# GregoryFaust/yaha

Hardware: AMD Instinct MI355X
Metric: aligned reads/s (whole node), 1 000 bp reads, OQC mode hot path (higher is better)
Workload: dtype int16

## Files before the change

### yaha_amd/csrc/device/abi.hip

```cpp
#include "ctx.h"
#include <memory>

std::atomic<int> gCtxPerDevice[64];
std::mutex gRowsMu[64];
hipEvent_t gRowsEv[64][4];
bool gRowsEvValid[64][4];
unsigned long long gRowsSeq[64];
std::atomic<int> gActiveRuns[64];
const char *const kStageNames[T_N] = {"seed_lookup", "hit_sort", "fragments_regions", "chain", "align_dp", "layout", "align_p1_gapfill", "ext_rows", "ext_trace",
                                      "align_p3_score_split", "ext_rows_device_clock", "ext_rows_packed16"};
thread_local const ygpu_ctx *tlsPfFailed = nullptr;

int runTo(ygpu_ctx *ctx, int stage)
{
    int rc;
    HIPCHK(hipSetDevice(ctx->device));
    if (ctx->stageDone < 1) {
        rc = stageSeed(ctx); if (rc) return rc;
        EV0(T_FRAGS); rc = buildFrags(ctx);
        if (rc == YD_RESORT) { rc = stageSeed(ctx); if (rc) return rc; EV0(T_FRAGS); rc = buildFrags(ctx);
            if (rc == YD_RESORT) { ctx->err = "hit sort: the sorted keys are not in ascending order"; rc = YGPU_EINTERNAL; } }
        if (rc) return rc;
        if (!ctx->nFrags) EV1(T_FRAGS);
        ctx->stageDone = 1;
// ... 209 lines not shown
    if (!ix || !p) return YGPU_EINVAL;
    for (int k = 0; k < n * cpd; k++) { all[k] = new ygpu_ctx; all[k]->device = devices[k / cpd]; }
    std::vector<ygpu_ctx *> out(n); for (int k = 0; k < n; k++) out[k] = all[k * cpd];
    std::vector<int> rcs(n, 0);
    auto notStarted = [&](int rc) {
        for (int k = 0; k < n; k++) {
            if (!rcs[k]) { rcs[k] = YGPU_EINVAL; out[k]->err = "not started: another device of the call failed"; }
            if (rc_each) rc_each[k] = rcs[k];
            for (int j = 1; j < cpd; j++) all[k * cpd + j]->err = out[k]->err;
        }
        return rc;
    };
    const double t0 = nowMs();
    int ndev = 0;
    if (hipGetDeviceCount(&ndev) != hipSuccess || ndev <= 0) { for (int k = 0; k < n; k++) { rcs[k] = YGPU_ENODEV;
        out[k]->err = "no HIP device visible: the hot path needs an MI355X (there is no CPU fallback)"; } return notStarted(YGPU_ENODEV); }
    if (getenv("YGPU_INIT_PHASES")) fprintf(stderr, "[ygpu] init: runtime up (hipGetDeviceCount) %8.1f ms\n", nowMs() - t0);
    {
        bool bad = false;
        for (int k = 0; k < n; k++) if (devices[k] < 0 || devices[k] >= ndev) { rcs[k] = YGPU_ENODEV; out[k]->err = "device index out of range"; bad = true; }
        if (bad) return notStarted(YGPU_ENODEV);
    }
    { int bad = 0; for (int k = 0; k < n; k++) { rcs[k] = checkParams(out[k], ix, p); if (rcs[k]) bad = rcs[k]; } if (bad) return notStarted(bad); }
    ImagePlan plan; plan.build(ix, n > 1 ? (64ull << 20) : (1024ull << 20));
    std::vector<ImageState> states(n); for (auto &st : states) { st.done.reset(new std::atomic<int>[plan.pieces.size() + 1]);
        for (size_t i = 0; i <= plan.pieces.size(); i++) st.done[i] = 0; }
    std::unique_ptr<std::atomic<int>[]> ready(new std::atomic<int>[n]); for (int k = 0; k < n; k++) ready[k] = 0;
    std::vector<int> srcIndex(n, -1); const bool peer = !(getenv("YGPU_PEER_COPY") && atoi(getenv("YGPU_PEER_COPY")) == 0);
    for (int k = 1; k < n && peer; k++) {
        int can = devices[k] == devices[k - 1] ? 1 : 0;
        if (!can && hipDeviceCanAccessPeer(&can, devices[k], devices[k - 1]) != hipSuccess) { can = 0; (void)hipGetLastError(); }
        if (can && devices[k] != devices[k - 1]) { if (hipSetDevice(devices[k]) == hipSuccess) { const hipError_t e = hipDeviceEnablePeerAccess(devices[k - 1], 0);
            if (e != hipSuccess && e != hipErrorPeerAccessAlreadyEnabled) can = 0; } else can = 0; (void)hipGetLastError(); }
        if (can) srcIndex[k] = k - 1;
    }
    if (getenv("YGPU_INIT_PHASES")) { fprintf(stderr, "[ygpu] init: image sources:");
        for (int k = 0; k < n; k++) { if (srcIndex[k] < 0) fprintf(stderr, " device %d <- host;", devices[k]);
        else fprintf(stderr, " device %d <- device %d;", devices[k], devices[srcIndex[k]]); } fprintf(stderr, " %zu pieces\n", plan.pieces.size()); }
    std::vector<std::thread> th;
    for (int k = 1; k < n; k++) th.emplace_back([&, k]() { rcs[k] = initDevice(out[k], devices[k], srcIndex[k], srcIndex[k] >= 0 ? devices[srcIndex[k]] : -1, ix, plan,
        states.data(), k, ready.get(), all + k * cpd + 1, cpd - 1); });
    rcs[0] = initDevice(out[0], devices[0], -1, -1, ix, plan, states.data(), 0, ready.get(), all + 1, cpd - 1);
    for (auto &x : th) x.join();
    int rc = 0; for (int k = 0; k < n; k++) { if (rc_each) rc_each[k] = rcs[k]; if (rcs[k] && !rc) rc = rcs[k];
        if (rcs[k]) for (int j = 1; j < cpd; j++) if (all[k * cpd + j]->err.empty()) all[k * cpd + j]->err = "the device's first context failed: " + out[k]->err; }
    return rc;
}

int ygpu_device_count(void) { int n = 0; if (hipGetDeviceCount(&n) != hipSuccess) { (void)hipGetLastError(); return 0; } return n; }

int ygpu_init(int device, const ygpu_index_view *ix, const ygpu_params *p, ygpu_ctx **out)
{
    if (!out) return YGPU_EINVAL;
    return ygpu_init_multi(&device, 1, 1, ix, p, out, nullptr);
}

int ygpu_clone(const ygpu_ctx *parent, ygpu_ctx **out)
{
    *out = nullptr;
    if (!parent || !parent->stream) return YGPU_EINVAL;
    ygpu_ctx *ctx = new ygpu_ctx; *out = ctx; ctx->device = parent->device;
    int rc = initCommon(ctx, parent->device); if (rc) return rc;
    shareImage(ctx, parent);
    ENSURE(ctx->counters, 4 * CNT_N); ENSURE(ctx->ctr, sizeof(DevCounters)); ENSURE(ctx->errFlag, 64);
    HIPCHK(hipMemsetAsync(ctx->counters.p, 0, 4 * CNT_N, ctx->stream));
    HIPCHK(streamSync(ctx));
    return 0;
}

}
std::vector<DevBuf *> allBuffers(ygpu_ctx *ctx)
{
    DevBuf *all[] = {&ctx->dBases, &ctx->dSO, &ctx->dROA, &ctx->dLow, &ctx->dFwd, &ctx->dRev, &ctx->dFwd4, &ctx->dRev4, &ctx->dReadOff, &ctx->dKmerOff, &ctx->posS, &ctx->posC,
        &ctx->posRsI, &ctx->hitOff, &ctx->expandStart, &ctx->keysA, &ctx->keysB, &ctx->segOff, &ctx->bigB, &ctx->bigE, &ctx->isHead, &ctx->tileState,
                         &ctx->frags, &ctx->regStart, &ctx->multiList, &ctx->smallList, &ctx->bigList, &ctx->regionCount, &ctx->regionBase, &ctx->clumps, &ctx->clumpFrags,
                             &ctx->clumpFrags0, &ctx->order, &ctx->clumpsSorted, &ctx->rootPush, &ctx->rootBase, &ctx->outClumps,
                         &ctx->outClumps2, &ctx->outOps, &ctx->outRoot, &ctx->outPush, &ctx->dstIdx, &ctx->readCount, &ctx->readStart, &ctx->counters, &ctx->ctr, &ctx->errFlag,
                             &ctx->scanState, &ctx->bucketWork, &ctx->scratchAlign,
                         &ctx->segLists, &ctx->subB, &ctx->subE, &ctx->subLists, &ctx->subBigB, &ctx->subBigE, &ctx->sub2B, &ctx->sub2E, &ctx->sub2Lists, &ctx->sub3B, &ctx->sub3E,
                             &ctx->sub3Lists, &ctx->kmerParts, &ctx->scratchChain, &ctx->dpProbs, &ctx->dpRes, &ctx->dpOps, &ctx->rootState, &ctx->stateOps, &ctx->extProbs,
                             &ctx->rowsBound, &ctx->stripOff, &ctx->extRes, &ctx->extTrace, &ctx->chunkCnt, &ctx->memoKeys, &ctx->memoCount, &ctx->probs2, &ctx->rowsBound2,
                             &ctx->stripOff2, &ctx->extRes2, &ctx->extTrace2, &ctx->rowsClock, &ctx->splitScratch, &ctx->fallList, &ctx->keys2a, &ctx->keys2b, &ctx->vals2a,
                             &ctx->vals2b, &ctx->extKeys, &ctx->extVals, &ctx->extKeys2, &ctx->extOrder, &ctx->slowList, &ctx->gapScratch, &ctx->jointCount, &ctx->jointBase,
                             &ctx->joints, &ctx->sortKeys, &ctx->sortVals, &ctx->sortKeys2, &ctx->sortVals2, &ctx->gapOps, &ctx->waveChunks, &ctx->extOps, &ctx->traceCnt,
                         &ctx->oqCs, &ctx->oqCl, &ctx->oqOpsIn, &ctx->oqSeeds, &ctx->oqQlen, &ctx->pf.scanState, &ctx->pf.counters, &ctx->oqProf, &ctx->oqLists, &ctx->oqClsCnt,
                             &ctx->oqThr, &ctx->oqSeqStart, &ctx->oqSeqLen, &ctx->oqNeed, &ctx->oqPoolOff, &ctx->oqKeys, &ctx->oqStack, &ctx->oqNodes, &ctx->oqPrim, &ctx->oqPA,
                             &ctx->oqPfx, &ctx->oqPath, &ctx->oqPool, &ctx->oqPush, &ctx->oqOut, &ctx->oqOutCnt, &ctx->oqOutOps, &ctx->oqPrimCnt, &ctx->oqOutStart,
                             &ctx->oqOpsStart, &ctx->oqFClumps, &ctx->oqFOps, &ctx->jnCnt, &ctx->jnStart, &ctx->jnOut, &ctx->jnStats, &ctx->jnSeqStart, &ctx->jnSeqLen,
                         &ctx->puFwd, &ctx->puReadOff, &ctx->puTileCnt, &ctx->puTileStart, &ctx->puCand, &ctx->puSlots, &ctx->puRows,
                         &ctx->idTable, &ctx->idStats, &ctx->idSeqStart, &ctx->idSeqLen, &ctx->idBinBase, &ctx->idTileCnt, &ctx->idTileStart, &ctx->idOut};
    return std::vector<DevBuf *>(all, all + sizeof all / sizeof all[0]);
}
extern "C" {

void ygpu_destroy(ygpu_ctx *ctx)
{
    if (!ctx) return;
    if (ctx->worker.joinable()) { { std::lock_guard<std::mutex> lk(ctx->aMu); ctx->aQuit = true; } ctx->aCv.notify_all(); ctx->worker.join(); }
    if (ctx->counted) gCtxPerDevice[ctx->device & 63]--;
    if (ctx->stream) {
        hipSetDevice(ctx->device);
        {
            const int dv = ctx->device & 63; std::lock_guard<std::mutex> lk(gRowsMu[dv]);
            (void)hipStreamSynchronize(ctx->stream);
            if (gCtxPerDevice[dv].load() <= 0) for (int k = 0; k < 4; k++) if (gRowsEvValid[dv][k]) { (void)hipEventDestroy(gRowsEv[dv][k]); gRowsEvValid[dv][k] = false; }
        }
        if (ctx->sharedIndex) { ctx->dBases.p = nullptr; ctx->dBases.cap = 0; ctx->dSO.p = nullptr; ctx->dSO.cap = 0; ctx->dROA.p = nullptr; ctx->dROA.cap = 0;
            ctx->dLow.p = nullptr; ctx->dLow.cap = 0; }
        const std::vector<DevBuf *> all = allBuffers(ctx);
        for (auto b : all) b->release();
        for (int t = 0; t < T_N; t++) { hipEventDestroy(ctx->ev[t][0]); hipEventDestroy(ctx->ev[t][1]); }
        if (ctx->evSync) hipEventDestroy(ctx->evSync);
        if (ctx->pinned) hipHostFree(ctx->pinned);
        if (ctx->pf.pinned) hipHostFree(ctx->pf.pinned);
        if (ctx->snapCtr) hipHostFree(ctx->snapCtr);
        if (ctx->pf.evSync) hipEventDestroy(ctx->pf.evSync);
        if (ctx->evSnap) hipEventDestroy(ctx->evSnap);
        for (int i = 0; i < YD_MAX_CHUNK_EV; i++) hipEventDestroy(ctx->evChunk[i]);
        hipEventDestroy(ctx->evTail); hipStreamDestroy(ctx->stream2);
        hipStreamDestroy(ctx->stream);
    }
    delete ctx;
}
int ygpu_memory(ygpu_ctx *ctx, uint64_t *free_bytes, uint64_t *total_bytes, uint64_t *ctx_bytes)
{
    if (!ctx || !ctx->stream) return YGPU_EINVAL;
    HIPCHK(hipSetDevice(ctx->device));
    size_t fb = 0, tb = 0; HIPCHK(hipMemGetInfo(&fb, &tb));
    uint64_t mine = 0; for (DevBuf *b : allBuffers(ctx)) if (b->p && !(ctx->sharedIndex && (b == &ctx->dBases || b == &ctx->dSO || b == &ctx->dROA
        || b == &ctx->dLow))) mine += b->cap;
    if (free_bytes) *free_bytes = fb; if (total_bytes) *total_bytes = tb; if (ctx_bytes) *ctx_bytes = mine;
    return 0;
}
int ygpu_park(ygpu_ctx *ctx)
{
    if (!ctx || !ctx->stream) return YGPU_EINVAL;
    HIPCHK(hipSetDevice(ctx->device)); HIPCHK(streamSync(ctx));
    for (DevBuf *b : allBuffers(ctx)) if (b != &ctx->dBases && b != &ctx->dSO && b != &ctx->dROA && b != &ctx->dLow) b->release();
    if (ctx->counted) { gCtxPerDevice[ctx->device & 63]--; ctx->counted = false; }
    ctx->stageDone = 0; ctx->parked = true; ctx->idUsed = 0;
    return 0;
}
int ygpu_get_arena_profile(ygpu_ctx *ctx, ygpu_arena_profile *out)
{
    if (!ctx || !ctx->stream || !out) return YGPU_EINVAL;
    memset(out, 0, sizeof *out);
    const std::vector<DevBuf *> all = allBuffers(ctx);
    if (all.size() > sizeof out->cap / sizeof out->cap[0]) { ctx->err = "arena profile: more buffers than the profile holds"; return YGPU_EINTERNAL; }
    out->n = (uint32_t)all.size();
    for (size_t k = 0; k < all.size(); k++) { DevBuf *b = all[k];
        out->cap[k] = (b == &ctx->dBases || b == &ctx->dSO || b == &ctx->dROA || b == &ctx->dLow) ? 0ull : (uint64_t)b->cap; }
    out->trace_ratio = ctx->traceRatio; out->ops_ratio = ctx->opsRatio; out->last_clump_slots = ctx->lastClumpSlots; out->last_fall = ctx->lastFall; out->bases = ctx->totalBases;
    return 0;
}
int ygpu_presize(ygpu_ctx *ctx, const ygpu_arena_profile *prof)
{
    if (!ctx || !ctx->stream || !prof) return YGPU_EINVAL;
    if (ctx->parked) { ctx->err = "the context was parked (ygpu_park)"; return YGPU_EINVAL; }
    HIPCHK(hipSetDevice(ctx->device));
    const std::vector<DevBuf *> all = allBuffers(ctx);
    if (prof->n != all.size()) { ctx->err = "arena profile of another build"; return YGPU_EINVAL; }
    for (size_t k = 0; k < all.size(); k++) {
        DevBuf *b = all[k];
        if (b == &ctx->dBases || b == &ctx->dSO || b == &ctx->dROA || b == &ctx->dLow || b == &ctx->counters || b == &ctx->ctr || b == &ctx->errFlag
            || b == &ctx->pf.counters || b == &ctx->idTable || b == &ctx->idStats) continue;
        if (prof->cap[k] > b->cap && b->ensureExact((size_t)prof->cap[k])) { (void)hipGetLastError(); ctx->err = "hipMalloc failed while presizing the arenas"; return YGPU_ENOMEM;
// ... 140 lines not shown
```

### yaha_amd/csrc/device/align_diag.h

```cpp
#pragma once

static void diagJointHist(ygpu_ctx *ctx, uint32_t J)
{
    std::vector<JointRec> hj(J); hipMemcpy(hj.data(), ctx->joints.p, sizeof(JointRec) * (size_t)J, hipMemcpyDeviceToHost);
    unsigned long long nj[4] = {0, 0, 0, 0}, cj[4] = {0, 0, 0, 0}, b3 = 0, b3lim = 0, c3lim = 0, f3 = 0, wh[5] = {0, 0, 0, 0, 0};
    for (auto &j : hj) if (j.kind == JK_DP) {
        const bool banded = (j.flags & 2u) != 0; const int q = j.qGap, r = j.rGap, ld = q > r ? q - r : r - q, W = banded ? 2 * ctx->P.bandWidth + ld + 1 : r + 1;
        const uint32_t cls = gapJointClass(gapJointKey(ctx->P, banded, q, r)); nj[cls]++; cj[cls] += (unsigned long long)q * (unsigned long long)std::min(W, r + 1);
        if (cls == 3) { if (banded) { b3++; if (W <= 32 && q <= YD_GROWS - 1 && r <= YD_GREF) { b3lim++; c3lim += (unsigned long long)q * W; } } else f3++;
            wh[std::min(4, (W - 17) / 8)]++; }
    }
    fprintf(stderr, "[ygpu] DP joints by class (band <= 12 / band <= 16 / other W <= 16 / the rest): %llu %llu %llu %llu; strip cells %llu %llu %llu %llu; "
                    "the rest: banded %llu (W <= 32 within the band kernels' limits: %llu, %llu cells), full %llu; "
                    "W 17-24 / 25-32 / 33-40 / 41-48 / more: %llu %llu %llu %llu %llu\n",
            nj[0], nj[1], nj[2], nj[3], cj[0], cj[1], cj[2], cj[3], b3, b3lim, c3lim, f3, wh[0], wh[1], wh[2], wh[3], wh[4]);
}

static void diagCountDups(ygpu_ctx *ctx, uint32_t nProb)
{
    std::vector<ExtProb> hp(nProb); hipMemcpy(hp.data(), ctx->extProbs.p, sizeof(ExtProb) * (size_t)nProb, hipMemcpyDeviceToHost);
    std::vector<std::array<uint32_t, 4>> keys; keys.reserve(nProb);
    for (auto &e : hp) if (e.flags & XP_VALID) keys.push_back({e.qBase, e.rOff, (uint32_t)e.qOff | ((uint32_t)e.qLen << 16), e.flags & 3u});
    std::sort(keys.begin(), keys.end()); size_t dup = 0, sameStart = 0;
    for (size_t k = 1; k < keys.size(); k++) { dup += keys[k] == keys[k - 1];
        sameStart += keys[k][0] == keys[k - 1][0] && keys[k][1] == keys[k - 1][1] && (keys[k][2] & 0xFFFF) == (keys[k - 1][2] & 0xFFFF) && keys[k][3] == keys[k - 1][3]; }
    fprintf(stderr, "[ygpu] extension problems: %zu valid, %zu exact duplicates (%.2f%%), %zu share (read, strand, direction, rOff, qOff) with their predecessor (%.2f%%)\n",
        keys.size(), dup, 100.0 * dup / std::max<size_t>(1, keys.size()), sameStart, 100.0 * sameStart / std::max<size_t>(1, keys.size()));
}

static void diagTraceLens(ygpu_ctx *ctx, const ExtArgs &E, uint32_t np)
{
    streamSync(ctx);
    std::vector<ExtRes> hr(np); std::vector<uint32_t> ho(np);
    hipMemcpy(hr.data(), E.res, sizeof(ExtRes) * (size_t)np, hipMemcpyDeviceToHost); hipMemcpy(ho.data(), E.order, 4ull * np, hipMemcpyDeviceToHost);
    unsigned long long walkers = 0, sumLen = 0, sumWaveMax = 0, sumRows = 0, hist[8] = {0};
    for (uint32_t w = 0; w < np; w += 64) { uint32_t mx = 0; for (uint32_t k = w; k < std::min(np, w + 64); k++) { const ExtRes &r = hr[ho[k]];
        const uint32_t len = r.score > 0 ? (uint32_t)r.maxi : 0u; walkers += r.score > 0; sumLen += len; sumRows += r.rows; mx = std::max(mx, len); int b = 0;
        while (b < 7 && (len >> (b + 3))) b++; hist[len ? b : 0] += 1; } sumWaveMax += mx; }
    fprintf(stderr, "[ygpu] traceback: %u problems, %llu walk (%.1f%%), mean walk %.1f rows (all) / %.1f (walkers), rows computed mean %.1f; sum over waves of "
        "the longest walk %llu = %.1f x the lanes' mean\n",
            np, walkers, 100.0 * walkers / np, (double)sumLen / np, (double)sumLen / std::max(1ull, walkers), (double)sumRows / np, sumWaveMax,
                (double)sumWaveMax * 64.0 / std::max(1ull, sumLen));
    fprintf(stderr, "[ygpu] walk length histogram (0..7, 8.., 16.., 32.., 64.., 128.., 256.., 512..):"); for (int b = 0; b < 8; b++) fprintf(stderr, " %llu", hist[b]);
        fprintf(stderr, "\n");
}

static void diagTraceDbg(const ExtArgs &E)
{
    unsigned w8[8]; hipMemcpyFromSymbol(w8, HIP_SYMBOL(gTraceDbg), sizeof w8);
    if (!w8[0]) return;
    ExtRes rr; hipMemcpy(&rr, E.res + w8[6], sizeof rr, hipMemcpyDeviceToHost); ExtProb pp; hipMemcpy(&pp, E.probs + w8[6], sizeof pp, hipMemcpyDeviceToHost);
    fprintf(stderr, "[ygpu] k_ext_trace left its strip: dword %d of %u, f0 %u, laneOff %u; problem %u where %08x (wave %u lane %u phase %u) score %d maxi %d maxj "
        "%d rows %u qLen %u flags %u\n", (int)w8[1], w8[2], w8[3], w8[4], w8[6], w8[7], w8[7] >> 10, (w8[7] >> 4) & 63, w8[7] & 15, rr.score, rr.maxi, rr.maxj, rr.rows,
            pp.qLen, pp.flags);
    memset(w8, 0, sizeof w8); hipMemcpyToSymbol(HIP_SYMBOL(gTraceDbg), w8, sizeof w8);
}

static void diagFallWhy(ygpu_ctx *ctx, const unsigned int *fallCount)
{
    uint32_t fc = 0; hipMemcpyAsync(&fc, fallCount, 4, hipMemcpyDeviceToHost, ctx->stream); streamSync(ctx);
    unsigned w8[8]; hipMemcpyFromSymbol(w8, HIP_SYMBOL(gFallWhy), sizeof w8);
    fprintf(stderr, "[ygpu] roots left to the wave kernel %u (other %u, DP not listed %u, second split %u, depth/list %u)\n", fc, w8[0], w8[1], w8[2], w8[3]);
    memset(w8, 0, sizeof w8); hipMemcpyToSymbol(HIP_SYMBOL(gFallWhy), w8, sizeof w8);
}

static void diagListHist(ygpu_ctx *ctx, uint32_t r0, uint32_t r1)
{
    const uint32_t nr2 = r1 - r0; std::vector<ExtRes> hr2(2 * (size_t)nr2); std::vector<RootState> hs(nr2);
    hipMemcpy(hr2.data(), ctx->extRes.as<ExtRes>() + 2 * (size_t)r0, sizeof(ExtRes) * hr2.size(), hipMemcpyDeviceToHost);
        hipMemcpy(hs.data(), ctx->rootState.as<RootState>() + r0, sizeof(RootState) * nr2, hipMemcpyDeviceToHost);
    unsigned long long hx[8] = {0}, hb[8] = {0}, ht[8] = {0}, sumx = 0, sumb = 0; const unsigned edges[7] = {0, 1, 2, 4, 8, 16, 32};
    auto bin = [&](unsigned v) { int k = 0; while (k < 7 && v > edges[k]) k++; return k; };
    for (uint32_t k = 0; k < nr2; k++) {
        const unsigned a = hr2[2 * k].score > 0 ? hr2[2 * k].nOps : 0u, c2 = hr2[2 * k + 1].score > 0 ? hr2[2 * k + 1].nOps : 0u, b = hs[k].len; hx[bin(a)]++;
        hx[bin(c2)]++; hb[bin(b)]++; ht[bin(a + b + c2)]++; sumx += a + c2; sumb += b; }
    fprintf(stderr, "[ygpu] list lengths over %u roots (bins: 0, 1, 2, 3-4, 5-8, 9-16, 17-32, more): extension lists", nr2);
        for (int k = 0; k < 8; k++) fprintf(stderr, " %llu", hx[k]);
    fprintf(stderr, "; phase-1 lists"); for (int k = 0; k < 8; k++) fprintf(stderr, " %llu", hb[k]); fprintf(stderr, "; merged");
        for (int k = 0; k < 8; k++) fprintf(stderr, " %llu", ht[k]);
    fprintf(stderr, "; mean ops per root: extensions %.1f, phase 1 %.1f\n", (double)sumx / nr2, (double)sumb / nr2);
}

static void profReset()
{
#ifdef YD_PROF
    unsigned long long z[16] = {0}; hipMemcpyToSymbol(HIP_SYMBOL(gProf), z, sizeof z); hipMemcpyToSymbol(HIP_SYMBOL(gRowsProf), z, sizeof(unsigned long long) * 8);
    hipMemcpyToSymbol(HIP_SYMBOL(gTraceProf), z, sizeof(unsigned long long) * 8);
#endif
}
static void profPrint(ygpu_ctx *ctx, unsigned waves)
{
#ifdef YD_PROF
    streamSync(ctx); unsigned long long z[16]; hipMemcpyFromSymbol(z, HIP_SYMBOL(gProf), sizeof z);
    const char *nm[10] = {"root_total", "dp_rows", "traceback", "perfect_ext", "score", "emit", "split", "merge", "dp_calls", "roots"};
    fprintf(stderr, "[YD_PROF] waves %u:", waves); for (int i = 0; i < 10; i++) fprintf(stderr, " %s=%llu", nm[i], z[i]); fprintf(stderr, "\n");
    unsigned long long q[8]; hipMemcpyFromSymbol(q, HIP_SYMBOL(gRowsProf), sizeof q);
    if (q[0]) fprintf(stderr,
        "[YD_PROF] k_ext_rows_pk: wave passes %llu; of them writing results %.1f %%, with a new maximum in some lane %.1f %%, handing blocks over %.1f %%; "
// ... 9 lines not shown
```

### yaha_amd/csrc/device/ctx.h

```cpp
#pragma once
#include <hip/hip_runtime.h>
#include <string>
#include <vector>
#include <cstring>
#include <cstdio>
#include <cstdlib>
#include <algorithm>
#include <array>
#include <atomic>
#include <chrono>
#include <thread>
#include <mutex>
#include <condition_variable>
#include <memory>
#include "common.h"
#include "../oqc_core.h"

#define HIPCHK(call) do { hipError_t e_ = (call); \
    if (e_ != hipSuccess) { ctx->err = std::string(#call) + ": " + hipGetErrorString(e_); return YGPU_ENODEV; } } while (0)

#define KL(kern, grid, block, shmem, st, ...) do { hipLaunchKernelGGL(kern, grid, block, shmem, st, __VA_ARGS__); hipError_t e_ = hipGetLastError(); \
    if (e_ != hipSuccess) { ctx->err = std::string("launch of " #kern " failed: ") + hipGetErrorString(e_); return YGPU_ENODEV; } } while (0)

#define YD_MAX_CHUNK_EV 16

struct DevBuf {
    void *p = nullptr;
    size_t cap = 0;
    int ensure(size_t bytes, bool keep = false, hipStream_t st = 0)
    {
        if (bytes <= cap) return 0;
        size_t ncap = bytes + bytes / 4 + 256; void *np = nullptr;
        if (hipMalloc(&np, ncap) != hipSuccess) return -1;
        if (keep && p && cap) { hipMemcpyAsync(np, p, cap, hipMemcpyDeviceToDevice, st); hipStreamSynchronize(st); }
        if (p) hipFree(p);
        p = np; cap = ncap; return 0;
    }
    void release() { if (p) hipFree(p); p = nullptr; cap = 0; }
    int ensureExact(size_t bytes)
    {
        if (bytes <= cap) return 0;
        release();
        void *np = nullptr;
        if (hipMalloc(&np, bytes) != hipSuccess) return -1;
        p = np; cap = bytes; return 0;
    }
    template <class T> T *as() const { return (T *)p; }
};

enum {
    CNT_NMULTI = 0, CNT_MAXN, CNT_CLUMPS, CNT_CFRAGS, CNT_QCHAIN, CNT_QALIGN, CNT_OUTCLUMPS, CNT_OUTOPS, CNT_QDP, CNT_DPOPS, CNT_NBIG, CNT_QBIG,
    CNT_STATEOPS, CNT_EXTOPS, CNT_QEXT, CNT_SLOW, CNT_NDP, CNT_NDP16, CNT_GAPOPS, CNT_PAD_EVEN, CNT_NMULTI2 ,
        CNT_NTINY, CNT_NSMALL, CNT_NMID, CNT_NB12, CNT_NB16,
        CNT_NB24,
    CNT_SEGC,
    CNT_NFRAGS = CNT_SEGC + 16,
    CNT_NREG = CNT_NFRAGS + 3,
    CNT_SCANFAIL = CNT_NREG + 2,
    CNT_N = CNT_NREG + 4
};
enum { T_SEED = 0, T_SORT, T_FRAGS, T_CHAIN, T_ALIGN, T_LAYOUT, T_TOP, T_P1 = T_TOP, T_XROWS, T_XTRACE, T_P3, T_XROWS_DEV, T_XROWS_PK, T_N };

extern std::atomic<int> gCtxPerDevice[64];
extern std::mutex gRowsMu[64];
extern hipEvent_t gRowsEv[64][4];
extern bool gRowsEvValid[64][4];
extern unsigned long long gRowsSeq[64];
extern std::atomic<int> gActiveRuns[64];
extern const char *const kStageNames[T_N];

struct PfSide {
    std::string err;
    hipStream_t stream = nullptr;
    uint32_t *pinned = nullptr;
    hipEvent_t evSync = nullptr;
    DevBuf scanState, counters;
    int device = 0;
};

enum { TRACK_DEPTH = 0, TRACK_EVENTS = 1, TRACK_PILEUP = 2, TRACK_KINDS };
struct TrackImage {
    int device = 0;
    DevBuf data, stats, seqStart, seqLength, binBase;
    uint64_t nBins = 0;
    uint32_t channels = 1, bin = 0, minMapq = 0, minClip = 0;
    std::vector<uint32_t> hSeqStart, hSeqLength;
    ~TrackImage() { (void)hipSetDevice(device); data.release(); stats.release(); seqStart.release(); seqLength.release(); binBase.release(); }
};

struct ygpu_ctx {
    int device = 0;
    hipStream_t stream = nullptr;
    DevParams P{};
    std::string err;
    int nCU = 256;
    DevBuf dBases, dSO, dROA, dLow;
    bool sharedIndex = false;
    uint32_t nReads = 0;
    int maxQ = 0;
    uint64_t totalBases = 0;
    uint32_t nKmers = 0;
    std::vector<uint32_t> hReadOff, hKmerOff;
    DevBuf dFwd, dRev, dFwd4, dRev4, dReadOff, dKmerOff;
    DevBuf bigB, bigE;
    DevBuf posS, posC, posRsI, hitOff, expandStart, keysA, keysB, segOff, isHead, tileState, frags;
    DevBuf segLists, subB, subE, subLists, subBigB, subBigE, sub2B, sub2E, sub2Lists, sub3B, sub3E, sub3Lists, kmerParts;
    DevBuf regStart, multiList, smallList, bigList, regionCount, regionBase;
    DevBuf clumps, clumpFrags, clumpFrags0, order, clumpsSorted, scratchChain;
    DevBuf rootPush, rootBase, outClumps, outClumps2, outOps, outRoot, outPush, dstIdx, readCount, readStart;
    DevBuf scratchAlign, dpProbs, dpRes, dpOps;
    DevBuf rootState, stateOps, extProbs, rowsBound, stripOff, extRes, extTrace, chunkCnt;
    DevBuf memoKeys, memoCount, probs2, rowsBound2, stripOff2, extRes2, extTrace2, splitScratch, fallList;
    DevBuf keys2a, keys2b, vals2a, vals2b, extKeys, extVals, extKeys2, extOrder, slowList;
    DevBuf gapScratch, jointCount, jointBase, joints, sortKeys, sortVals, sortKeys2, sortVals2, gapOps;
    DevBuf waveChunks, extOps, traceCnt, rowsClock;
    DevBuf counters, ctr, errFlag, scanState, bucketWork;
    bool evUsed[16] = {false};
    double traceT = 0;
    hipStream_t stream2 = nullptr;
    hipEvent_t evChunk[YD_MAX_CHUNK_EV], evTail;
    bool counted = false;
    bool parked = false;
    long long traceBudgetBlocks = 0;
    uint32_t lastClumpSlots = 0;
    bool keepAllFrags = false;
    unsigned long long hRowsClock[2] = {0, 0};
    int laneChunks = 0;
    uint32_t segSortMax = 0;
    int splitLanes = 1;
    int rows2PerCU = 0;
    int alignWavesPerCU = 0;
    int laneExt = 1;
    std::vector<unsigned long long> hStripOff;
    int runsDone = 0;
    double traceRatio = 0.0, opsRatio = 0.03;
    int statRanges = 0, statAttempts = 0;
    double statT0 = 0;
    DevBuf oqProf, oqLists, oqClsCnt, oqThr, oqSeqStart, oqSeqLen, oqNeed, oqPoolOff, oqKeys, oqStack, oqNodes, oqPrim, oqPA, oqPfx, oqPath, oqPool;
    DevBuf oqPush, oqOut, oqOutCnt, oqOutOps, oqPrimCnt, oqOutStart, oqOpsStart, oqFClumps, oqFOps;
    bool oqSet = false, oqDone = false;
    yoqc::Params oqP{};
    yoqc::Seqs oqG{};
    uint32_t nFOut = 0, nFOps = 0;
    PfSide pf;
    std::atomic<bool> pfSnap{false};
    hipEvent_t evSnap = nullptr;
    uint32_t snapN = 0, snapC = 0, snapOps = 0, pfN = 0;
    unsigned long long runGen = 0, snapGen = 0, filtGen = 0;
    ygpu_counters pfCounters{};
    DevCounters *snapCtr = nullptr;
    DevCounters snapCtrPlain{};
    unsigned long long snapHits = 0, snapFrags = 0, snapRegions = 0;
    DevBuf oqCs, oqCl, oqOpsIn, oqSeeds, oqQlen;
    std::shared_ptr<TrackImage> track[TRACK_KINDS];
    DevBuf puFwd, puReadOff, puTileCnt, puTileStart, puCand, puSlots, puRows;
    uint64_t puNCand = 0; bool puHaveCand = false;
    DevBuf idTable, idStats, idSeqStart, idSeqLen, idBinBase, idTileCnt, idTileStart, idOut;
    bool idSet = false, idAuto = false;
    uint64_t idCap = 0, snapBases = 0;
    uint32_t idMinMapq = 0, idMinLen = 1, idNSeqs = 0, idUsed = 0;
    DevBuf jnCnt, jnStart, jnOut, jnStats, jnSeqStart, jnSeqLen;
    bool jnSet = false, jnDone = false, jnHaveTotal = false;
    uint32_t jnMinMapq = 0, jnNSeqs = 0, jnReads = 0, jnTotal = 0;
    uint32_t hOutCounts[2] = {0, 0};
    uint32_t nHits = 0, nFrags = 0, nRegions = 0, nMulti = 0, nTiny = 0, nSmall = 0, nMid = 0, nBig = 0, maxN = 0;
    int sortRankUsed = 0;
    bool sortRankForced = false;
    uint32_t nClumpSlots = 0, nClumps = 0, nClumpFrags = 0, nOut = 0, nOutOps = 0;
    int stageDone = 0;
    std::vector<uint32_t> hClumpStart, hOps, hClumpFragStart, hClumpRS, hDpOps;
    std::vector<ygpu_clump> hClumps;
    std::vector<ygpu_fragment> hFrags, hClumpFrags;
    std::vector<ygpu_dp_result> hDpRes;
    ygpu_counters hCounters{};
    std::thread worker;
    std::mutex aMu;
    std::condition_variable aCv;
    const ygpu_read_batch *aBatch = nullptr;
    uint64_t aTicket = 0;
    int aRc = 0;
    bool aOpen = false, aDone = false, aQuit = false, aWaiting = false;
    ygpu_result_batch aOut{};
    long long lastFall = -1;
    unsigned int hFall = 0;
    uint32_t *pinned = nullptr;
    hipEvent_t evSync = nullptr;
    hipEvent_t ev[T_N][2];
    float ms[T_N] = {0};
    float totalMs = 0;
    const char *names[T_N];
    bool rowsPacked = false;
};

static inline DevBatch devBatch(ygpu_ctx *c)
{
    DevBatch b; b.fwd = c->dFwd.as<uint8_t>(); b.rev = c->dRev.as<uint8_t>(); b.readOff = c->dReadOff.as<uint32_t>(); b.nReads = c->nReads; return b;
}
// ... 73 lines not shown
```

### yaha_amd/csrc/device/dp_stage.h

```cpp
#pragma once
#include "split_lanes.h"

__global__ void k_dp_classify(DevParams P, const uint8_t *bases, const uint8_t *fwd, const uint8_t *rev, JointRec *joints, uint32_t n, uint32_t *keys, uint32_t *diagOps)
{
    YD_HIGH_PRIO();
    const uint32_t t = blockIdx.x * blockDim.x + threadIdx.x;
    if (t >= n) return;
    JointRec j = joints[t];
    YD_GLOBAL const uint8_t *q = toGlobal((j.flags & 1u) ? rev : fwd) + j.qBase; YD_GLOBAL const uint8_t *gB = toGlobal(bases);
    auto refAt = [&](uint32_t off) -> uint32_t { const uint32_t b = gB[off >> 1]; return (off & 1u) ? (b & 15u) : (b >> 4); };
    const int qGap = j.qGap, rGap = j.rGap;
    const bool banded = (j.flags & 2u) != 0;
    j.kind = JK_DP; uint32_t key = YD_JKEY_NONE;
    if (qGap == rGap && qGap > 0) {
        int mm = 0, runs = 0, pc = -1;
        for (int k = 0; k < qGap; k++) { const int c = (uint32_t)q[(int)j.nsqo + k] != refAt(j.nsro + (uint32_t)k); mm += c; runs += c != pc; pc = c; }
        if (mm * (P.MS + P.RC) <= P.MS + 2 * (P.GO + P.GE)) { j.kind = JK_DIAG; j.score = P.MS * (qGap - mm) - P.RC * mm; j.nOps = (uint16_t)runs; }
    }
    if (j.kind == JK_DP) key = gapJointKey(P, banded, qGap, rGap);
    joints[t] = j; keys[t] = key; diagOps[t] = j.kind == JK_DIAG ? (uint32_t)j.nOps : 0u;
}

__global__ void k_dp_gather_ext(const ExtProb *probs, const ExtRes *res, const uint32_t *extOps, const uint32_t *outOff, const uint32_t *dst, uint32_t n,
                                ygpu_dp_result *out, uint32_t *outOps)
{
    YD_HIGH_PRIO();
    const uint32_t p = blockIdx.x * blockDim.x + threadIdx.x;
    if (p >= n) return;
    const ExtRes r = res[p]; ygpu_dp_result o; o.score = 0; o.addedQLen = o.addedRLen = 0; o.op_start = outOff[p]; o.n_ops = 0;
    if (r.score > 0) {
        const bool rv = (probs[p].flags & XP_REV) != 0; const uint32_t *src = extOpsPtr(extOps, r); const char codes[4] = {'M', 'R', 'D', 'I'};
        o.score = r.score; o.addedQLen = (uint16_t)r.maxi; o.addedRLen = (uint16_t)(r.maxi + (r.maxj - YD_LBAND)); o.n_ops = r.nOps;
        for (uint32_t k = 0; k < r.nOps; k++) { const uint32_t op = src[rv ? r.nOps - 1u - k : k];
            outOps[o.op_start + k] = ((uint32_t)(uint8_t)codes[opCode(op) & 3] << 16) | (uint32_t)opLen(op); }
    }
    out[dst[p]] = o;
}
__global__ void k_dp_gather_gap(DevParams P, const uint8_t *bases, const uint8_t *fwd, const uint8_t *rev, const JointRec *joints, const uint32_t *gapOps, const uint32_t *outOff,
    const uint32_t *dst,
                                uint32_t n, ygpu_dp_result *out, uint32_t *outOps)
{
    YD_HIGH_PRIO();
    const uint32_t t = blockIdx.x * blockDim.x + threadIdx.x;
    if (t >= n) return;
    const JointRec j = joints[t]; ygpu_dp_result o; o.score = j.score; o.addedQLen = o.addedRLen = 0; o.op_start = outOff[t]; o.n_ops = j.nOps;
    const char codes[4] = {'M', 'R', 'D', 'I'};
    if (j.kind == JK_DIAG) {
        YD_GLOBAL const uint8_t *q = toGlobal((j.flags & 1u) ? rev : fwd) + j.qBase; YD_GLOBAL const uint8_t *gB = toGlobal(bases);
        int pc = -1, pl = 0; uint32_t w = o.op_start;
        for (int k = 0; k < (int)j.qGap; k++) {
            const uint32_t off = j.nsro + (uint32_t)k, b = gB[off >> 1], rc = (off & 1u) ? (b & 15u) : (b >> 4);
            const int c = (uint32_t)q[(int)j.nsqo + k] == rc ? OP_M : OP_R;
            if (c == pc) pl++; else { if (pc >= 0) outOps[w++] = ((uint32_t)(uint8_t)codes[pc] << 16) | (uint32_t)pl; pc = c; pl = 1; }
        }
        if (pc >= 0) outOps[w++] = ((uint32_t)(uint8_t)codes[pc] << 16) | (uint32_t)pl;
    } else for (uint32_t k = 0; k < j.nOps; k++) { const uint32_t op = gapOps[j.opsOff + k];
        outOps[o.op_start + k] = ((uint32_t)(uint8_t)codes[opCode(op) & 3] << 16) | (uint32_t)opLen(op); }
    out[dst[t]] = o;
}
```

### yaha_amd/csrc/device/gap_band_lanes.h

```cpp
#pragma once
#include "phase_lanes.h"

template <int GW>
__global__ void __launch_bounds__(64) k_gap_band(AlignArgs A, PhaseArgs X)
{
    YD_HIGH_PRIO();
    static_assert(GW == 12 || GW == 16, "two instances");
    const int lane = laneId(); const DevParams &P = A.P;
    const int GO = P.GO, GE = P.GE, GOE = P.GO + P.GE, RC = P.RC, MS = P.MS, maxIntron = P.maxIntron, maxGapP = P.maxGap, bw = P.bandWidth;
    uint32_t *sp = (uint32_t *)(X.gapScratch + (size_t)blockIdx.x * 64u * YD_GAP_SCRATCH) + lane;
    YD_GLOBAL uint32_t *T32 = toGlobal(sp); uint32_t *tmp = sp + (size_t)((YD_GROWS + 1) * 32 / 4) * 64;
    YD_GLOBAL const uint8_t *gB = toGlobal(A.bases);
    const uint32_t tBegin = GW == 12 ? 0u : X.nDPb[0], tEnd = GW == 12 ? X.nDPb[0] : X.nDPb[1];
    constexpr int RD = GW / 4;
    __shared__ uint32_t sQ[16 * 64], sR[13 * 64];
    typedef uint32_t yd_u32u __attribute__((aligned(1)));
    for (uint32_t base = tBegin + blockIdx.x * 64u; base < tEnd; base += gridDim.x * 64u) {
        const uint32_t t = base + (uint32_t)lane; const bool live = t < tEnd;
        int nT = 0, score = 0; unsigned cells = 0; uint32_t ji = 0;
        if (live) {
            ji = X.sortedVals[t]; const JointRec j = X.joints[ji];
            const int qGap = j.qGap, rGap = j.rGap;
            int left, right; if (rGap > qGap) { right = bw + (rGap - qGap); left = bw; } else { left = bw + (qGap - rGap); right = bw; }
            const int W = left + right + 1;
            YD_GLOBAL const uint8_t *q = toGlobal((j.flags & 1u) ? A.B.rev : A.B.fwd) + j.qBase + j.nsqo;
            const uint32_t rB0 = ((j.nsro >= (uint32_t)left ? j.nsro - (uint32_t)left : 0u) >> 1) & ~3u;
            {
                const int nQ = (qGap + 3) >> 2, nR = (int)((((j.nsro + (uint32_t)(qGap - left + GW - 1)) >> 1) - rB0) >> 2) + 1;
#pragma unroll
                for (int k = 0; k < 16; k++) if (k < nQ) sQ[k * 64 + lane] = *(YD_GLOBAL const yd_u32u *)(q + 4 * k);
#pragma unroll
                for (int k = 0; k < 13; k++) if (k < nR) sR[k * 64 + lane] = *(YD_GLOBAL const uint32_t *)(gB + rB0 + 4u * (uint32_t)k);
            }
            auto qAt = [&](int idx) -> int { return (int)((sQ[(idx >> 2) * 64 + lane] >> (8 * (idx & 3))) & 0xFFu); };
            auto refAt = [&](int idx) -> uint32_t {
                if (idx < 0 && (uint32_t)(-idx) > j.nsro) return 15u;
                const uint32_t off = j.nsro + (uint32_t)idx, rel = (off >> 1) - rB0; const uint32_t b = (sR[(rel >> 2) * 64 + lane] >> (8u * (rel & 3u))) & 0xFFu;
                return (off & 1u) ? (b & 15u) : (b >> 4);
            };
            int PV[GW], PF[GW], PI[GW];
#pragma unroll
            for (int c = 0; c < GW; c++) { PV[c] = c == left ? 0 : ((c > left && c < W) ? -(GO + (c - left) * GE) : YD_LWORST); PF[c] = c == left ? -GO : YD_LWORST; PI[c] = 0; }
#pragma unroll
            for (int k = 0; k < RD; k++) {
                uint32_t acc = 0;
#pragma unroll
                for (int b = 0; b < 4; b++) { const int c = 4 * k + b; const uint32_t cell = c == left ? TR_U8 : ((c > left && c < W) ? (uint32_t)(OP_D | ((c - left) << 2)) : 0u);
                    acc |= cell << (8 * b); }
                T32[k * 64] = acc;
            }
            unsigned long long win = 0;
#pragma unroll
            for (int c = 0; c < GW; c++) win |= (unsigned long long)refAt(c - left) << (4 * c);
            int qc = qAt(0);
            for (int i = 1; i <= qGap; i++) {
                const int qcNext = qAt(i < qGap ? i : qGap - 1);
                const uint32_t nbNext = refAt(i - left + GW - 1);
                { int sc = left + 1 - i; if (sc < 0) sc = 0; int ec = left + rGap - i; if (ec > W - 1) ec = W - 1; if (ec >= sc) cells += (unsigned)(ec - sc + 1); }
                int PVCol = YD_LWORST, PE = YD_LWORST, PD = 0, dV = PV[0];
                uint32_t acc = 0;
#pragma unroll
                for (int c = 0; c < GW; c++) {
                    const int rc = (int)((win >> (4 * c)) & 15ull);
                    const bool eq = rc == qc;
                    int V = dV + (eq ? MS : -RC); uint32_t cell = eq ? (uint32_t)OP_M : (uint32_t)OP_R;
                    const int CE = PE - GE, NE = PVCol - GOE;
                    const bool cE = CE >= NE && (PD + 1) <= maxIntron;
                    PE = cE ? CE : NE; PD = cE ? PD + 1 : 1;
                    if (PE > V) { V = PE; cell = (uint32_t)OP_D | ((uint32_t)PD << 2); }
                    int upV, upF, upI;
                    if (c + 1 < GW) { upV = PV[c + 1]; upF = PF[c + 1]; upI = PI[c + 1]; } else { upV = YD_LWORST; upF = YD_LWORST; upI = 0; }
                    const int CF = upF - GE, NF = upV - GOE;
                    const bool cF = CF >= NF && (upI + 1) <= maxGapP;
                    const int F = cF ? CF : NF, I = cF ? upI + 1 : 1;
                    if (F > V) { V = F; cell = (uint32_t)OP_I | ((uint32_t)I << 2); }
                    acc |= (cell & 0xFFu) << (8 * (c & 3));
                    if ((c & 3) == 3) { T32[(i * RD + (c >> 2)) * 64] = acc; acc = 0; }
                    const bool in = c < 11 || c < W;
                    PV[c] = in ? V : YD_LWORST; PF[c] = in ? F : YD_LWORST; PI[c] = in ? I : 0;
                    PVCol = V; dV = upV;
                }
                win = (win >> 4) | ((unsigned long long)nbNext << (4 * (GW - 1)));
                qc = qcNext;
            }
            score = PV[0];
#pragma unroll
            for (int c = 1; c < GW; c++) score = c == right ? PV[c] : score;
            int x = right, y = qGap;
            auto cellAt = [&](int yy, int xx) -> unsigned { const int c = yy * GW + xx; return (T32[(c >> 2) * 64] >> (8 * (c & 3))) & 0xFFu; };
            unsigned cell = cellAt(y, x);
            int prev = cell == TR_U8 ? -1 : (int)(cell & 3u), acc2 = 0, n = 0;
            for (int guard = 0; cell != TR_U8 && guard < 4096; guard++) {
                const int code = (int)(cell & 3u); int len = (int)(cell >> 2);
                if (code == OP_D) x -= len; else if (code == OP_I) { x += len; y -= len; } else { y -= 1; len = 1; }
                if (prev != code) { tmp[n * 64] = opMake(prev, acc2); n++; prev = code; acc2 = len; } else acc2 += len;
                if (y < 0 || x < 0 || x >= GW || n >= 190) break;
                cell = cellAt(y, x);
            }
            tmp[n * 64] = opMake(prev, acc2); n++;
            nT = n;
        }
        int incl = nT;
#pragma unroll
        for (int d = 1; d < 64; d <<= 1) { int v = __shfl_up(incl, d, 64); if (lane >= d) incl += v; }
        const int total = __shfl(incl, 63, 64); unsigned ob = 0;
        if (lane == 63 && total) ob = atomicAdd(X.gapOpsCount, (unsigned)total);
        ob = (unsigned)__shfl((int)ob, 63, 64);
        if (live) {
            const unsigned off = ob + (unsigned)(incl - nT);
            if ((unsigned long long)off + (unsigned)nT > (unsigned long long)X.gapOpsCap) atomicCAS(A.errFlag, 0, (int)YERR_OUT);
            else {
                for (int k = 0; k < nT; k++) X.gapOps[off + k] = tmp[(nT - 1 - k) * 64];
                JointRec *jp = X.joints + ji; jp->opsOff = off; jp->nOps = (uint16_t)nT; jp->score = score; jp->cells = cells;
            }
        }
    }
}
```

### yaha_amd/csrc/device/gap_band_pk.h

```cpp
#pragma once
#include "gap_band_lanes.h"
#include "ext_lanes_pk.h"

template <int GW, bool CAPS, class QAt, class RefAt>
__device__ __forceinline__ int gapBandPkRows(const DevParams &P, int qGap, int left, int right, int W, QAt qAt, RefAt refAt, YD_GLOBAL uint32_t *T32)
{
    constexpr int H = GW / 2, RD = GW / 4;
    const int GO = P.GO, GE = P.GE, GOE = GO + GE;
    const uint32_t GEp = pk2(GE), GOEp = pk2(GOE), LWp = pk2(YD_LW16), LWg = pk2(YD_LW16 - GOE), ONEp = 0x00010001u;
    uint32_t NEGKv = pk2(-(P.MS + P.RC)), MSGv = pk2(P.MS + GOE), ONEv = ONEp, C15v = 0x000F000Fu, FOURv = 0x00040004u, OPDv = pk2(OP_D), OPIv = pk2(OP_I);
    asm volatile("" : "+v"(NEGKv), "+v"(MSGv), "+v"(ONEv), "+v"(C15v), "+v"(FOURv), "+v"(OPDv), "+v"(OPIv));
    const uint32_t maxIp = pk2(P.maxIntron < 30000 ? P.maxIntron : 30000), maxGp = pk2(P.maxGap < 30000 ? P.maxGap : 30000);
    auto onChain = [&](int c) { return c > left && c < W; };
    auto v0 = [&](int c) -> int { return c == left ? 0 : (onChain(c) ? -(GO + (c - left) * GE) : YD_LW16); };
    auto f0 = [&](int c) -> int { return c == left ? -GO : YD_LW16; };
    auto e0 = [&](int c) -> int { return onChain(c) ? -(GO + (c - left) * GE) : YD_LW16; };
    auto d0 = [&](int c) -> int { return onChain(c) ? c - left : 0; };
    auto cell0 = [&](int c) -> uint32_t { return c == left ? (uint32_t)TR_U8 : (onChain(c) ? (uint32_t)(OP_D | ((c - left) << 2)) : 0u); };
    auto lo16 = [](int v) -> uint32_t { return (uint32_t)v & 0xFFFFu; };
    uint32_t PVg[H], PF[H], PI[H], rc[H], keep[H];
#pragma unroll
    for (int k = 0; k < H; k++) {
        PVg[k] = lo16(v0(k) - GOE) | (LWg & 0xFFFF0000u); PF[k] = lo16(f0(k)) | (LWp & 0xFFFF0000u); PI[k] = 0u;
        rc[k] = refAt(k - left) | (refAt(k + H - 1 - left) << 16);
// ... 62 lines not shown
            }
#pragma unroll
            for (int d = 0; d < RD; d++) T32[(t * RD + d) * 64] = D[d];
        }
        carryV = PVg[H - 1] & 0xFFFFu; carryE = PE & 0xFFFFu; carryD = PD & 0xFFFFu;
        if (t == qGap && right < H) {
            scoreLo = 0;
#pragma unroll
            for (int k = 0; k < H; k++) if (k == right) scoreLo = (int)(short)(PVg[k] & 0xFFFFu) + GOE;
        }
        if (t <= qGap) {
            const uint32_t nb = refAt(t + GW - 2 - left), was1 = rc[1] >> 16;
#pragma unroll
            for (int k = 0; k + 1 < H; k++) rc[k] = rc[k + 1];
            rc[H - 1] = was1 | (nb << 16);
        }
        qcHi = qcLo;
    }
    int score = scoreLo;
    if (right >= H) {
#pragma unroll
        for (int k = 0; k < H; k++) if (k + H == right) score = (int)(short)(PVg[k] >> 16) + GOE;
    }
    return score;
}

template <int GW>
__global__ void __launch_bounds__(64) k_gap_band_pk(AlignArgs A, PhaseArgs X)
{
    YD_HIGH_PRIO();
    static_assert(GW == 12 || GW == 16 || GW == 24, "three instances");
    constexpr int H = GW / 2;
    const int lane = laneId(); const DevParams &P = A.P;
    const int bw = P.bandWidth;
    uint32_t *sp = (uint32_t *)(X.gapScratch + (size_t)blockIdx.x * 64u * YD_GAP_SCRATCH) + lane;
    YD_GLOBAL uint32_t *T32 = toGlobal(sp); uint32_t *tmp = sp + (size_t)((YD_GROWS + 1) * 32 / 4) * 64;
    YD_GLOBAL const uint8_t *gB = toGlobal(A.bases);
    const uint32_t tBegin = GW == 12 ? 0u : (GW == 16 ? X.nDPb[0] : X.nDP[1]), tEnd = GW == 12 ? X.nDPb[0] : (GW == 16 ? X.nDPb[1] : X.nDP[1] + X.nDPb[2]);
    __shared__ uint32_t sQ[16 * 64], sR[13 * 64];
    typedef uint32_t yd_u32u __attribute__((aligned(1)));
    for (uint32_t base = tBegin + blockIdx.x * 64u; base < tEnd; base += gridDim.x * 64u) {
        const uint32_t t = base + (uint32_t)lane; const bool live = t < tEnd;
        int nT = 0, score = 0; unsigned cells = 0; uint32_t ji = 0;
        JointRec j; j.qGap = 0; j.rGap = 0; j.nsro = 0; j.flags = 0; j.qBase = 0; j.nsqo = 0;
        if (live) { ji = X.sortedVals[t]; j = X.joints[ji]; }

        const bool caps = __ballot(live && ((int)j.qGap > P.maxGap || P.maxIntron < GW)) != 0ull;
        if (live) {
            const int qGap = j.qGap, rGap = j.rGap;
            int left, right; if (rGap > qGap) { right = bw + (rGap - qGap); left = bw; } else { left = bw + (qGap - rGap); right = bw; }
            const int W = left + right + 1;
            YD_GLOBAL const uint8_t *q = toGlobal((j.flags & 1u) ? A.B.rev : A.B.fwd) + j.qBase + j.nsqo;
            const uint32_t rB0 = ((j.nsro >= (uint32_t)left ? j.nsro - (uint32_t)left : 0u) >> 1) & ~3u;
            {
                const int nQ = (qGap + 3) >> 2, nR = (int)((((j.nsro + (uint32_t)(qGap - left + GW - 1)) >> 1) - rB0) >> 2) + 1;
#pragma unroll
                for (int k = 0; k < 16; k++) if (k < nQ) sQ[k * 64 + lane] = *(YD_GLOBAL const yd_u32u *)(q + 4 * k);
#pragma unroll
                for (int k = 0; k < 13; k++) if (k < nR) sR[k * 64 + lane] = *(YD_GLOBAL const uint32_t *)(gB + rB0 + 4u * (uint32_t)k);
            }
            auto qAt = [&](int idx) -> int { return (int)((sQ[(idx >> 2) * 64 + lane] >> (8 * (idx & 3))) & 0xFFu); };
            auto refAt = [&](int idx) -> uint32_t {
                if (idx < 0 && (uint32_t)(-idx) > j.nsro) return 15u;
                const uint32_t off = j.nsro + (uint32_t)idx, rel = (off >> 1) - rB0; const uint32_t b = (sR[(rel >> 2) * 64 + lane] >> (8u * (rel & 3u))) & 0xFFu;
                return (off & 1u) ? (b & 15u) : (b >> 4);
            };
            for (int i = 1; i <= qGap; i++) { int sc = left + 1 - i; if (sc < 0) sc = 0; int ec = left + rGap - i; if (ec > W - 1) ec = W - 1;
                if (ec >= sc) cells += (unsigned)(ec - sc + 1); }
            score = caps ? gapBandPkRows<GW, true>(P, qGap, left, right, W, qAt, refAt, T32) : gapBandPkRows<GW, false>(P, qGap, left, right, W, qAt, refAt, T32);
            int x = right, y = qGap;
            auto cellAt = [&](int yy, int xx) -> unsigned { const int c = (yy + (xx >= H ? 1 : 0)) * GW + xx; return (T32[(c >> 2) * 64] >> (8 * (c & 3))) & 0xFFu; };
            unsigned cell = cellAt(y, x);
            int prev = cell == TR_U8 ? -1 : (int)(cell & 3u), acc2 = 0, n = 0;
            for (int guard = 0; cell != TR_U8 && guard < 4096; guard++) {
                const int code = (int)(cell & 3u); int len = (int)(cell >> 2);
                if (code == OP_D) x -= len; else if (code == OP_I) { x += len; y -= len; } else { y -= 1; len = 1; }
                if (prev != code) { tmp[n * 64] = opMake(prev, acc2); n++; prev = code; acc2 = len; } else acc2 += len;
                if (y < 0 || x < 0 || x >= GW || n >= 190) break;
                cell = cellAt(y, x);
            }
            tmp[n * 64] = opMake(prev, acc2); n++;
            nT = n;
        }
        int incl = nT;
#pragma unroll
        for (int d = 1; d < 64; d <<= 1) { int v = __shfl_up(incl, d, 64); if (lane >= d) incl += v; }
        const int total = __shfl(incl, 63, 64); unsigned ob = 0;
        if (lane == 63 && total) ob = atomicAdd(X.gapOpsCount, (unsigned)total);
        ob = (unsigned)__shfl((int)ob, 63, 64);
        if (live) {
            const unsigned off = ob + (unsigned)(incl - nT);
            if ((unsigned long long)off + (unsigned)nT > (unsigned long long)X.gapOpsCap) atomicCAS(A.errFlag, 0, (int)YERR_OUT);
            else {
                for (int k = 0; k < nT; k++) X.gapOps[off + k] = tmp[(nT - 1 - k) * 64];
                JointRec *jp = X.joints + ji; jp->opsOff = off; jp->nOps = (uint16_t)nT; jp->score = score; jp->cells = cells;
            }
        }
    }
}
```

### yaha_amd/csrc/device/phase_lanes.h

```cpp
#pragma once
#include "ext_lanes.h"

struct RootState { uint32_t sro, listOff; int32_t score; uint16_t sqo, eqo, refLen, len; uint8_t status, pad[3]; uint32_t pad2[2]; };
enum { JK_NONE = 0, JK_D, JK_I, JK_R, JK_DIAG, JK_DP };
struct JointRec {
    uint32_t nsro, qBase; uint16_t nsqo, qGap, rGap; uint8_t kind, flags;
    uint32_t opsOff; uint16_t nOps, pad; int32_t score; uint32_t cells;
};
struct PhaseArgs {
    RootState *state; uint32_t *stateOps; unsigned int *stateOpsCount; uint32_t stateOpsCap;
    ExtProb *probs; unsigned long long *rowsBound;
    const ExtRes *res; const uint32_t *extOps;
    uint32_t *slowList; unsigned int *slowCount;
    int useList;
    uint32_t rootBegin;
    uint32_t *memoKeys; unsigned int *memoCount; ExtProb *probs2; unsigned long long *rowsBound2; unsigned int *nProb2; uint32_t probs2Cap;
    uint32_t *jointCount; const uint32_t *jointBase; JointRec *joints; uint32_t nJoints;
    uint32_t *sortKeys, *sortVals; const uint32_t *sortedVals; unsigned int *nDP, *nDPb; uint32_t band24;
    uint32_t *gapOps; unsigned int *gapOpsCount; uint32_t gapOpsCap;
    uint32_t *extKeys, *extVals;
    uint8_t *gapScratch;
};

__device__ __forceinline__ unsigned waveSumU(unsigned v) { return (unsigned)waveSumI((int)v); }
__device__ __forceinline__ unsigned waveReserve(unsigned long long mask, unsigned int *counter, int lane, unsigned each = 1u)
{
    if (!mask) return 0u;
    const int first = __builtin_ctzll(mask); unsigned base = 0;
    if (lane == first) base = atomicAdd(counter, each * (unsigned)__builtin_popcountll(mask));
    base = (unsigned)__builtin_amdgcn_readlane((int)base, first);
    return base + each * (unsigned)__builtin_popcountll(mask & ((1ull << lane) - 1ull));
}


template <int N> __device__ __forceinline__ void blockCounters(unsigned long long *const (&dst)[N], const unsigned (&val)[N])
{
    __shared__ unsigned sAcc[N];
    if (threadIdx.x < (unsigned)N) sAcc[threadIdx.x] = 0;
    __syncthreads();
    if (laneId() == 0) { for (int k = 0; k < N; k++) if (val[k]) atomicAdd(&sAcc[k], val[k]); }
    __syncthreads();
    if (threadIdx.x < (unsigned)N && sAcc[threadIdx.x]) atomicAdd(dst[threadIdx.x], (unsigned long long)sAcc[threadIdx.x]);
}

template <int N> __device__ __forceinline__ void blockCountersU32(unsigned int *const (&dst)[N], const unsigned (&val)[N])
{
    __shared__ unsigned sAcc32[N];
    if (threadIdx.x < (unsigned)N) sAcc32[threadIdx.x] = 0;
    __syncthreads();
    if (laneId() == 0) { for (int k = 0; k < N; k++) if (val[k]) atomicAdd(&sAcc32[k], val[k]); }
    __syncthreads();
    if (threadIdx.x < (unsigned)N && sAcc32[threadIdx.x]) atomicAdd(dst[threadIdx.x], sAcc32[threadIdx.x]);
}

__device__ __forceinline__ unsigned blockReserve(unsigned int *counter, unsigned waveTotal)
{
    __shared__ unsigned sTot[4], sBase;
    const int wv = (int)(threadIdx.x >> 6);
    if (laneId() == 0) sTot[wv] = waveTotal;
    __syncthreads();
    if (threadIdx.x == 0) { const unsigned t = sTot[0] + sTot[1] + sTot[2] + sTot[3]; sBase = t ? atomicAdd(counter, t) : 0u; }
    __syncthreads();
    unsigned b = sBase; for (int k = 0; k < wv; k++) b += sTot[k];
    return b;
}

#define YD_GROWS 60
#define YD_GREF 64
#define YD_GQW 16
#define YD_GRW 10
#define YD_GAP_SCRATCH 3072
#define TR_U8 0xFFu
struct GapLaneMem { int *pv, *pf; uint8_t *pi; uint32_t *refw, *qw; uint8_t *T; uint32_t *tmp; };
template <int GW>
__device__ __forceinline__ int gapDPLane(const DevParams &P, YD_GLOBAL const uint8_t *gB, YD_GLOBAL const uint8_t *q, bool banded,
                                         uint32_t rOff, int rLen, int qOff, int qLen, const GapLaneMem &M, int &nOps, unsigned &cellsOut)
{
    const int GO = P.GO, GE = P.GE, RC = P.RC, MS = P.MS, maxIntron = P.maxIntron, maxGapP = P.maxGap;
    int left = 0, right = 0;
    if (banded) { const int bw = P.bandWidth; if (rLen > qLen) { right = bw + (rLen - qLen); left = bw; } else { left = bw + (qLen - rLen); right = bw; } }
    const int W = banded ? left + right + 1 : rLen + 1;
    int *PV = M.pv, *PF = M.pf; uint8_t *PI = M.pi; YD_GLOBAL uint32_t *T32 = (YD_GLOBAL uint32_t *)toGlobal(M.T);
#define GPV(j) PV[(j) * 64]
#define GPF(j) PF[(j) * 64]
#define GPI(j) PI[(j) * 64]
    const uint32_t rByte0 = (rOff >> 1) & ~3u; const int rNib0 = (int)(rOff - 2u * rByte0);
    { YD_GLOBAL const uint32_t *g = (YD_GLOBAL const uint32_t *)(gB + rByte0); uint32_t w[YD_GRW];
#pragma unroll
      for (int k = 0; k < YD_GRW; k++) w[k] = g[k];
#pragma unroll
      for (int k = 0; k < YD_GRW; k++) M.refw[k * 64] = w[k]; }
    const size_t qAddr = (size_t)(q + qOff); const int qSkew = (int)(qAddr & 3u);
    { YD_GLOBAL const uint32_t *g = (YD_GLOBAL const uint32_t *)(qAddr - (size_t)qSkew); uint32_t w[YD_GQW];
#pragma unroll
      for (int k = 0; k < YD_GQW; k++) w[k] = g[k];
#pragma unroll
      for (int k = 0; k < YD_GQW; k++) M.qw[k * 64] = w[k]; }
    auto refAt = [&](int t) -> int { const int nb = rNib0 + t; const uint32_t w = M.refw[(nb >> 3) * 64]; return (int)((w >> (8 * ((nb >> 1) & 3) + ((nb & 1) ? 0 : 4))) & 15u); };
    auto qAt = [&](int t) -> int { const int bb = qSkew + t; return (int)((M.qw[(bb >> 2) * 64] >> (8 * (bb & 3))) & 0xFFu); };
    const int startInit = banded ? left + 1 : 1;
    if (banded) { GPF(W) = YD_WORST; GPV(W) = YD_WORST; GPI(W) = 0; }
    {
        uint32_t acc = 0;
        for (int j = 0; j < W; j++) {
            uint32_t cell = 0;
            if (j == startInit - 1) cell = TR_U8; else if (j >= startInit) { const int dc = j - startInit + 1; cell = (uint32_t)(OP_D | (dc << 2)); GPV(j) = -(GO + dc * GE);
                GPF(j) = YD_WORST; GPI(j) = 0; }
            acc |= cell << (8 * (j & 3));
            if ((j & 3) == 3 || j == W - 1) { T32[(j >> 2) * 64] = acc; acc = 0; }
        }
    }
    GPF(startInit - 1) = 0; GPI(startInit - 1) = 0; GPV(startInit - 1) = 0;
    int V = 0, PVCol = YD_WORST, startCol = 1, endCol = W - 1; unsigned cells = 0;
    for (int i = 1; i <= qLen; i++) {
        int PDCol = 0, PECol = YD_WORST, bl = -1;
        if (banded) {
            startCol = left + 1 - i;
            if (startCol <= 0) { startCol = 0; PVCol = YD_WORST; } else { PVCol = -(GO + i * GE); GPV(startCol - 1) = PVCol; bl = startCol - 1; }
            endCol = min(left + rLen - i, W - 1);
        } else { PVCol = -(GO + i * GE); bl = 0; }
        const int qc = qAt(i - 1);
        const int rRow = banded ? i - left - 1 : 0;
        uint32_t acc = bl >= 0 ? (uint32_t)(OP_I | (i << 2)) << (8 * (bl & 3)) : 0u;
        if (bl >= 0 && ((bl & 3) == 3 || startCol > endCol)) { T32[((i * GW + bl) >> 2) * 64] = acc; acc = 0; }
        for (int j = startCol; j <= endCol; j++) {
            const int RM = banded ? j : j - 1, IO = RM + 1; int op;
            V = GPV(RM);
            const int rc = refAt(banded ? rRow + j : j - 1);
            if (qc == rc) { V += MS; op = OP_M; } else { V -= RC; op = OP_R; }
            int len = 0;
            const int CE = PECol - GE, NE = PVCol - (GO + GE);
            if (CE >= NE && (PDCol + 1) <= maxIntron) { PECol = CE; PDCol = PDCol + 1; } else { PECol = NE; PDCol = 1; }
            if (PECol > V) { V = PECol; op = OP_D; len = PDCol; }
            int F, I; const int CF = GPF(IO) - GE, NF = GPV(IO) - (GO + GE), pio = (int)GPI(IO);
            if (CF >= NF && (pio + 1) <= maxGapP) { F = CF; I = pio + 1; } else { F = NF; I = 1; }
            if (F > V) { V = F; op = OP_I; len = I; }
            GPF(j) = F; GPI(j) = (uint8_t)I;
            acc |= (uint32_t)(op | (len << 2)) << (8 * (j & 3));
            if ((j & 3) == 3 || j == endCol) { T32[((i * GW + j) >> 2) * 64] = acc; acc = 0; }
            if (banded) GPV(j) = V; else GPV(j - 1) = PVCol;
            PVCol = V; cells++;
        }
        if (!banded) GPV(endCol) = V;
    }
    cellsOut = cells;
    int x = banded ? right : W - 1, y = qLen;
    auto cellAt = [&](int yy, int xx) -> unsigned { const int c = yy * GW + xx; return (T32[(c >> 2) * 64] >> (8 * (c & 3))) & 0xFFu; };
    unsigned cell = cellAt(y, x);
    int prev = cell == TR_U8 ? -1 : (int)(cell & 3u), acc2 = 0, n = 0;
    for (int guard = 0; cell != TR_U8 && guard < 4096; guard++) {
        const int code = (int)(cell & 3u); int len = (int)(cell >> 2);
        if (banded) { if (code == OP_D) x -= len; else if (code == OP_I) { x += len; y -= len; } else { y -= 1; len = 1; } }
        else        { if (code == OP_D) x -= len; else if (code == OP_I) { y -= len; } else { x -= 1; y -= 1; len = 1; } }
        if (prev != code) { M.tmp[n * 64] = opMake(prev, acc2); n++; prev = code; acc2 = len; } else acc2 += len;
        if (y < 0 || x < 0 || x >= GW || n >= 190) break;
        cell = cellAt(y, x);
    }
    M.tmp[n * 64] = opMake(prev, acc2); n++;
    nOps = n;
#undef GPV
#undef GPF
#undef GPI
    return V;
}

__global__ void k_joint_counts(AlignArgs A, PhaseArgs X)
{
    YD_HIGH_PRIO();
    const uint32_t r = blockIdx.x * blockDim.x + threadIdx.x;
    if (r < A.nRoots) X.jointCount[r] = YD_ROOT_REC(A, r).nFrags - 1u;
    if (r == A.nRoots) X.jointCount[r] = 0u;
}

typedef unsigned long long yd_u64u __attribute__((aligned(1)));
template <int DIR>
__device__ __forceinline__ int matchRun(YD_GLOBAL const uint8_t *q, int qi, YD_GLOBAL const uint8_t *gB, uint32_t ro, int maxLen)
{
    int m = 0;
    while (maxLen - m >= 8) {
        const int qa = DIR > 0 ? qi + m : qi - m - 7; const uint32_t ra = DIR > 0 ? ro + (uint32_t)m : ro - (uint32_t)m - 7u;
        unsigned long long qx = *(YD_GLOBAL const yd_u64u *)(q + qa);
        qx = (qx | (qx >> 4)) & 0x00FF00FF00FF00FFull; qx = (qx | (qx >> 8)) & 0x0000FFFF0000FFFFull;
        const uint32_t qs = (uint32_t)(qx | (qx >> 16));
        unsigned long long rx = *(YD_GLOBAL const yd_u64u *)(gB + (ra >> 1));
        rx = ((rx & 0x0F0F0F0F0F0F0F0Full) << 4) | ((rx >> 4) & 0x0F0F0F0F0F0F0F0Full);
        const uint32_t rs = (uint32_t)(rx >> (4u * (ra & 1u)));
        const uint32_t diff = qs ^ rs;
        if (diff) return m + (DIR > 0 ? (__builtin_ctz(diff) >> 2) : (__builtin_clz(diff) >> 2));
        m += 8;
    }
    for (; m < maxLen; m++) {
        const uint32_t off = DIR > 0 ? ro + (uint32_t)m : ro - (uint32_t)m; const uint32_t b = gB[off >> 1];
        if ((uint32_t)q[DIR > 0 ? qi + m : qi - m] != ((off & 1u) ? (b & 15u) : (b >> 4))) break;
    }
    return m;
}

#define YD_JKEY_NONE 0xFFFu
#define YD_JKEY_BITS 12
__host__ __device__ __forceinline__ uint32_t gapJointClass(uint32_t key) { return key >> 10; }
__host__ __device__ __forceinline__ uint32_t gapJointKey(const DevParams &P, bool banded, int qGap, int rGap)
{
    const int lenDiff = qGap > rGap ? qGap - rGap : rGap - qGap;
    const int W = banded ? 2 * P.bandWidth + lenDiff + 1 : rGap + 1;
    uint32_t cls = W <= 16 ? 2u : 3u;
    const bool lim = banded && P.bandWidth >= 5 && P.maxGap >= 16 && qGap <= YD_GROWS && rGap <= YD_GREF;
    if (lim && W <= 16) cls = W <= 12 ? 0u : 1u;
    uint32_t wf = (uint32_t)(W < 31 ? W : 31);
    if (cls == 3u) wf = (lim && W <= 24) ? (uint32_t)(W - 17) : 8u + (uint32_t)(W - 17 < 23 ? W - 17 : 23);
    return (cls << 10) | (wf << 5) | (uint32_t)((qGap >> 1) < 30 ? (qGap >> 1) : 30);
}
__host__ __device__ __forceinline__ bool gapJointBand24(uint32_t key) { return (key >> 10) == 3u && ((key >> 5) & 31u) < 8u; }

template <int BS = 256>
__device__ __forceinline__ uint32_t wgDeal(uint32_t root, uint32_t cls)
{
    __shared__ uint32_t sHist[65], sOrder[BS];
    const int lane = laneId();
    if (threadIdx.x < 65u) sHist[threadIdx.x] = 0u;
    __syncthreads();
    const uint32_t inCls = atomicAdd(&sHist[cls], 1u);
    __syncthreads();
    if (threadIdx.x < 64u) {
        const uint32_t c = sHist[lane]; uint32_t incl = c;
#pragma unroll
        for (int d = 1; d < 64; d <<= 1) { const uint32_t y = (uint32_t)__shfl_up((int)incl, d, 64); if (lane >= d) incl += y; }
        sHist[lane] = incl - c; if (lane == 63) sHist[64] = incl;
    }
    __syncthreads();
    sOrder[sHist[cls] + inCls] = cls < 64u ? root : 0xFFFFFFFFu;
    __syncthreads();
    return sOrder[threadIdx.x];
}

__global__ void __launch_bounds__(256) k_p1_joints(AlignArgs A, PhaseArgs X)
{
    YD_HIGH_PRIO();
    const uint32_t r = blockIdx.x * blockDim.x + threadIdx.x;
    const bool live = r < A.nRoots; const DevParams &P = A.P;
    unsigned perfect = 0, touched = 0, nDP = 0, nDP16 = 0, nB12 = 0, nB16 = 0, nB24 = 0;
    if (live) {
        const ChainClumpRec rec = YD_ROOT_REC(A, r); const int n = (int)rec.nFrags;
        if (n > 1) {
            const uint32_t read = rec.rs >> 1, r0 = A.B.readOff[read];
            YD_GLOBAL const uint8_t *q = toGlobal((rec.rs & 1u) ? A.B.rev : A.B.fwd) + r0; YD_GLOBAL const uint8_t *gB = toGlobal(A.bases);
            auto refAt = [&](uint32_t off) -> uint32_t { const uint32_t b = gB[off >> 1]; return (off & 1u) ? (b & 15u) : (b >> 4); };
            DevFrag *F = A.clumpFrags + rec.fragOff; const uint32_t jb = X.jointBase[r];
            DevFrag cur = F[0];
            for (int k = 1; k < n; k++) {
                DevFrag nxt = F[k];
                int gap = (int)min(gapI(cur.eqo, nxt.sqo), gapU(cur.sro + (uint32_t)cur.refLen - 1u, nxt.sro));
                { const int c = matchRun<-1>(q, (int)nxt.sqo - 1, gB, nxt.sro - 1u, gap);
                  perfect += c; touched += c + (c < gap);
                  if (c > 0) { nxt.sqo = (uint16_t)(nxt.sqo - c); nxt.sro -= (uint32_t)c; nxt.refLen = (uint16_t)(nxt.refLen + c); } gap -= c; }
                { const uint32_t eRO = cur.sro + (uint32_t)cur.refLen - 1u; const int c = matchRun<1>(q, (int)cur.eqo + 1, gB, eRO + 1u, gap);
                  perfect += c; touched += c + (c < gap);
                  if (c > 0) { cur.eqo = (uint16_t)(cur.eqo + c); cur.refLen = (uint16_t)(cur.refLen + c); } }
                F[k - 1] = cur;
                const uint32_t eRO = cur.sro + (uint32_t)cur.refLen - 1u;
                const int qGap = (int)(gapI(cur.eqo, nxt.sqo) & 0xFFFF), rGap = (int)(gapU(eRO, nxt.sro) & 0xFFFF);
                JointRec j; j.nsro = eRO + 1u; j.qBase = r0; j.nsqo = (uint16_t)((cur.eqo + 1) & 0xFFFF); j.qGap = (uint16_t)qGap; j.rGap = (uint16_t)rGap;
                j.flags = (uint8_t)(rec.rs & 1u); j.opsOff = 0; j.nOps = 0; j.pad = 0; j.score = 0; j.cells = 0; j.kind = JK_NONE;
                uint32_t key = YD_JKEY_NONE;
                if (qGap == 0 && rGap == 0) { }
                else if (qGap == 0) j.kind = JK_D;
                else if (rGap == 0) j.kind = JK_I;
                else if (rGap == 1 && qGap == 1) j.kind = JK_R;
                else {
                    const int lenDiff = qGap > rGap ? qGap - rGap : rGap - qGap;
                    const bool banded = lenDiff + P.bandWidth * 2 + 1 < rGap;
                    j.flags |= banded ? 2u : 0u; j.kind = JK_DP;
                    if (qGap == rGap) {
                        int mm = 0;
                        for (int t = 0; t < qGap; t++) mm += (uint32_t)q[(int)cur.eqo + 1 + t] != refAt(eRO + 1u + (uint32_t)t);
                        if (mm * (P.MS + P.RC) <= P.MS + 2 * (P.GO + P.GE)) { j.kind = JK_DIAG; j.score = P.MS * (qGap - mm) - P.RC * mm; }
                    }
                    if (j.kind == JK_DP) { key = gapJointKey(P, banded, qGap, rGap); const uint32_t cls = gapJointClass(key); nDP++; nDP16 += cls <= 2u; nB12 += cls == 0u;
                        nB16 += cls <= 1u; nB24 += gapJointBand24(key) ? 1u : 0u; }
                }
                X.joints[jb + (uint32_t)(k - 1)] = j; X.sortKeys[jb + (uint32_t)(k - 1)] = key; X.sortVals[jb + (uint32_t)(k - 1)] = jb + (uint32_t)(k - 1);
                cur = nxt;
            }
            F[n - 1] = cur;
        }
    }
    perfect = waveSumU(perfect); touched = waveSumU(touched); nDP = waveSumU(nDP); nDP16 = waveSumU(nDP16); nB12 = waveSumU(nB12); nB16 = waveSumU(nB16); nB24 = waveSumU(nB24);
    { unsigned long long *const dst[2] = {&A.ctr->v[C_PERFECT], &A.ctr->v[C_TOUCHED]}; const unsigned val[2] = {perfect, touched}; blockCounters<2>(dst, val); }
    { unsigned int *const dst[5] = {X.nDP, X.nDP + 1, X.nDPb, X.nDPb + 1, X.nDPb + 2}; const unsigned val[5] = {nDP, nDP16, nB12, nB16, nB24}; blockCountersU32<5>(dst, val); }
}

template <int GW>
__global__ void __launch_bounds__(64) k_gap_lanes(AlignArgs A, PhaseArgs X)
{
    YD_HIGH_PRIO();
    __shared__ int sPV[GW + 1][64], sPF[GW + 1][64];
    __shared__ uint8_t sPI[GW + 1][64]; __shared__ uint32_t sRefW[YD_GRW][64], sQW[YD_GQW][64];
    const int lane = laneId(); const DevParams &P = A.P;
    GapLaneMem GM; GM.pv = &sPV[0][lane]; GM.pf = &sPF[0][lane]; GM.pi = &sPI[0][lane]; GM.refw = &sRefW[0][lane]; GM.qw = &sQW[0][lane];
    { uint32_t *sp = (uint32_t *)(X.gapScratch + (size_t)blockIdx.x * 64u * YD_GAP_SCRATCH) + lane; GM.T = (uint8_t *)sp; GM.tmp = sp + (size_t)((YD_GROWS + 1) * 32 / 4) * 64; }
    YD_GLOBAL const uint8_t *gB = toGlobal(A.bases);
    const uint32_t nAll = X.nDP[0], n16 = X.nDP[1];
    const uint32_t tBegin = GW == 16 ? X.nDPb[1] : n16 + (X.band24 ? X.nDPb[2] : 0u), tEnd = GW == 16 ? n16 : nAll;
    for (uint32_t base = tBegin + blockIdx.x * 64u; base < tEnd; base += gridDim.x * 64u) {
        const uint32_t t = base + (uint32_t)lane; const bool live = t < tEnd;
        int nT = 0, score = 0; unsigned cells = 0; bool tooBig = false; uint32_t ji = 0;
        if (live) {
            ji = X.sortedVals[t]; const JointRec j = X.joints[ji];
            const bool banded = (j.flags & 2u) != 0; const int qGap = j.qGap, rGap = j.rGap;
            const int lenDiff = qGap > rGap ? qGap - rGap : rGap - qGap;
            const int W = banded ? 2 * P.bandWidth + lenDiff + 1 : rGap + 1;
            if (W > GW || qGap > YD_GROWS || rGap > YD_GREF) tooBig = true;
            else {
                YD_GLOBAL const uint8_t *q = toGlobal((j.flags & 1u) ? A.B.rev : A.B.fwd) + j.qBase;
                score = gapDPLane<GW>(P, gB, q, banded, j.nsro, rGap, (int)j.nsqo, qGap, GM, nT, cells);
            }
        }
        { const unsigned long long mm = __ballot(tooBig); const unsigned sl = waveReserve(mm, X.slowCount, lane); if (tooBig) X.slowList[sl] = ji; }
        int incl = nT;
#pragma unroll
        for (int d = 1; d < 64; d <<= 1) { int v = __shfl_up(incl, d, 64); if (lane >= d) incl += v; }
        const int total = __shfl(incl, 63, 64); unsigned ob = 0;
        if (lane == 63 && total) ob = atomicAdd(X.gapOpsCount, (unsigned)total);
        ob = (unsigned)__shfl((int)ob, 63, 64);
        if (live && !tooBig) {
            const unsigned off = ob + (unsigned)(incl - nT);
            if ((unsigned long long)off + (unsigned)nT > (unsigned long long)X.gapOpsCap) atomicCAS(A.errFlag, 0, (int)YERR_OUT);
            else {
                for (int k = 0; k < nT; k++) X.gapOps[off + k] = GM.tmp[(nT - 1 - k) * 64];
                JointRec *jp = X.joints + ji; jp->opsOff = off; jp->nOps = (uint16_t)nT; jp->score = score; jp->cells = cells;
            }
        }
    }
}

__global__ void __launch_bounds__(64) k_gap_wave(AlignArgs A, PhaseArgs X)
{
    YD_HIGH_PRIO();
    const int lane = laneId();
    WaveMem M = carveScratch(A.scratch + (size_t)blockIdx.x * A.scratchPerWave, A.maxQ, A.traceRows, A.listCap, A.genCap);
    __shared__ uint16_t sTrace[YD_LDS_CELLS];
    int err = 0; WaveScratch S; S.ldsTrace = sTrace; S.trace = M.trace; S.traceRows = A.traceRows; S.tmpOps = M.tmpOps; S.tmpCap = 2 * A.maxQ + 512; S.gen = M.gen;
        S.genCap = A.genCap; S.err = &err;
    const unsigned n = uniU(*X.slowCount);
    for (;;) {
        if (__ballot(1) != ~0ull) { atomicCAS(A.errFlag, 0, (int)YERR_EXEC); break; }
        unsigned t = 0; if (lane == 0) t = atomicAdd(A.queueHead, 1u);
        const unsigned i = uniU(t);
        if (i >= n) break;
        const uint32_t ji = uniU(X.slowList[i]); const JointRec j = X.joints[ji];
        const uint8_t *q = ((j.flags & 1u) ? A.B.rev : A.B.fwd) + j.qBase;
        DPOut o = dpWave(A.P, A.bases, q, (j.flags & 2u) ? YGPU_DP_BANDED : YGPU_DP_FULL, j.nsro, (int)j.rGap, (int)j.nsqo, (int)j.qGap, S);
        if (UNI_B(err != 0)) { if (lane == 0) atomicCAS(A.errFlag, 0, err); break; }
        const int nT = uni(o.nOps); unsigned ob = 0;
        if (lane == 0) ob = atomicAdd(X.gapOpsCount, (unsigned)nT); ob = uniU(ob);
        if (UNI_B((unsigned long long)ob + (unsigned)nT > (unsigned long long)X.gapOpsCap)) { if (lane == 0) atomicCAS(A.errFlag, 0, (int)YERR_OUT); break; }
        for (int k = lane; k < nT; k += 64) X.gapOps[ob + k] = dpOp(S, o, false, k);
        if (lane == 0) { JointRec *jp = X.joints + ji; jp->opsOff = ob; jp->nOps = (uint16_t)nT; jp->score = uni(o.score); jp->cells = (uint32_t)uni(o.cells); }
    }
}

__global__ void __launch_bounds__(256) k_p1_assemble(AlignArgs A, PhaseArgs X)
{
    YD_HIGH_PRIO();
    const int lane = laneId(); const uint32_t r = blockIdx.x * blockDim.x + threadIdx.x;
    const bool live = r < A.nRoots; const DevParams &P = A.P;
    ChainClumpRec rec; rec.nFrags = 0; rec.rs = 0; rec.fragOff = 0;
    if (live) rec = YD_ROOT_REC(A, r);
    const int n = (int)rec.nFrags; const uint32_t jb = live ? X.jointBase[r] : 0u;
    unsigned want = 0;
    if (live) { want = (unsigned)n + 1u; for (int k = 0; k + 1 < n; k++) { const JointRec &j = X.joints[jb + (uint32_t)k];
        want += j.kind == JK_DP ? (unsigned)j.nOps : (j.kind == JK_DIAG ? (unsigned)j.qGap : (j.kind != JK_NONE ? 1u : 0u)); } }
    unsigned incl = want;
#pragma unroll
    for (int d = 1; d < 64; d <<= 1) { unsigned t = (unsigned)__shfl_up((int)incl, d, 64); if (lane >= d) incl += t; }
    const unsigned total = (unsigned)__shfl((int)incl, 63, 64);
    const unsigned base = blockReserve(X.stateOpsCount, total);
    const unsigned slot = base + incl - want;
    unsigned perfect = 0, touched = 0, gapCalls = 0, gapRows = 0, gapCells = 0;
    if (live) {
        if ((unsigned long long)slot + want > (unsigned long long)X.stateOpsCap) atomicCAS(A.errFlag, 0, (int)YERR_OUT);
        else {
            const uint32_t read = rec.rs >> 1, r0 = A.B.readOff[read]; const int qlen = (int)(A.B.readOff[read + 1] - r0);
            YD_GLOBAL const uint8_t *q = toGlobal((rec.rs & 1u) ? A.B.rev : A.B.fwd) + r0; YD_GLOBAL const uint8_t *gB = toGlobal(A.bases);
            auto refAt = [&](uint32_t off) -> uint32_t { const uint32_t b = gB[off >> 1]; return (off & 1u) ? (b & 15u) : (b >> 4); };
            const DevFrag *F = A.clumpFrags + rec.fragOff;
            uint32_t *ops = X.stateOps + slot; int nOut = 0, pc = -1, pl = 0, score = 0;
            auto put = [&](int code, int len) { if (pc == code) { pl = (pl + len) & 0xFFFF; return; } if (pc >= 0) { ops[nOut] = opMake(pc, pl); nOut++; } pc = code;
                pl = len & 0xFFFF; };
            const DevFrag firstF = F[0]; DevFrag cur = firstF;
            for (int k = 1; k <= n; k++) {
                { const int ql = fragQLen(cur.sqo, cur.eqo); put(OP_M, ql); score += P.MS * ql; }
                if (k == n) break;
                const JointRec j = X.joints[jb + (uint32_t)(k - 1)]; const int qGap = j.qGap, rGap = j.rGap;
                if (j.kind == JK_D) { put(OP_D, rGap); score -= P.GO + rGap * P.GE; }
                else if (j.kind == JK_I) { put(OP_I, qGap); score -= P.GO + qGap * P.GE; }
                else if (j.kind == JK_R) { put(OP_R, 1); score -= P.RC; }
                else if (j.kind == JK_DIAG) {
                    const int g = qGap;
                    for (int t = 0; t < g; t++) put((uint32_t)q[(int)j.nsqo + t] == refAt(j.nsro + (uint32_t)t) ? OP_M : OP_R, 1);
                    score += j.score; gapCalls++; gapRows += (unsigned)g; touched += (unsigned)g;
                    if (P.bandWidth * 2 + 1 < g) { const int bw = P.bandWidth, W = 2 * bw + 1; for (int i = 1; i <= g; i++) { int sc = bw + 1 - i; if (sc < 0) sc = 0;
                        int ec = bw + g - i; if (ec > W - 1) ec = W - 1; if (ec >= sc) gapCells += (unsigned)(ec - sc + 1); } }
                    else gapCells += (unsigned)(g * g);
                } else if (j.kind == JK_DP) {
                    for (int t = 0; t < (int)j.nOps; t++) { const uint32_t op = X.gapOps[j.opsOff + (uint32_t)t]; put(opCode(op), opLen(op)); }
                    score += j.score; gapCalls++; gapRows += (unsigned)qGap; gapCells += j.cells; touched += (unsigned)rGap;
                }
                cur = F[k];
            }
            uint32_t sro = firstF.sro; int sqo = firstF.sqo, eqo = cur.eqo; int refLen = (int)((1u + (cur.sro + (uint32_t)cur.refLen - 1u) - firstF.sro) & 0xFFFFu);
            int firstAdd = 0;
            int backLen = (int)((uint32_t)sqo < sro ? (uint32_t)sqo : sro), forwLen;
            if (backLen > 0) {
                const int m = matchRun<-1>(q, sqo - 1, gB, sro - 1u, backLen);
                perfect += m; touched += m + (m < backLen);
                if (m > 0) { firstAdd = m; score += m * P.MS; backLen -= m; sqo -= m; sro -= (uint32_t)m; refLen = (refLen + m) & 0xFFFF; }
            }
            {
                const uint32_t eRO = sro + (uint32_t)refLen - 1u;
                const uint32_t qrem = (uint32_t)(((qlen - 1) - eqo) & 0xFFFF), rrem = P.maxROff - eRO;
                forwLen = (int)(qrem < rrem ? qrem : rrem);
                if (forwLen > 0) {
                    const int m = matchRun<1>(q, eqo + 1, gB, eRO + 1u, forwLen);
                    perfect += m; touched += m + (m < forwLen);
                    if (m > 0) { pl = (pl + m) & 0xFFFF; score += m * P.MS; forwLen -= m; eqo += m; refLen = (refLen + m) & 0xFFFF; }
                }
            }
            if (nOut == 0) pl = (pl + firstAdd) & 0xFFFF;
            ops[nOut] = opMake(pc, pl); nOut++;
            if (nOut > 1 && firstAdd) ops[0] = opMake(opCode(ops[0]), (opLen(ops[0]) + firstAdd) & 0xFFFF);
            RootState s; memset(&s, 0, sizeof s);
            s.sro = sro; s.sqo = (uint16_t)sqo; s.eqo = (uint16_t)eqo; s.refLen = (uint16_t)refLen; s.score = score; s.status = (rec.rs & 1u) ? stReversed : 0;
                s.len = (uint16_t)nOut;
            s.listOff = slot;
            X.state[r] = s;
            const uint32_t strand = (rec.rs & 1u) ? XP_STRAND : 0u; const bool vb = backLen >= P.minExtLength, vf = forwLen >= P.minExtLength;
            ExtProb pb; pb.qBase = r0; pb.rOff = sro - 1u; pb.qOff = (uint16_t)((sqo - 1) & 0xFFFF); pb.qLen = (uint16_t)(backLen & 0xFFFF);
                pb.flags = strand | XP_REV | (vb ? XP_VALID : 0u);
            ExtProb pf; pf.qBase = r0; pf.rOff = sro + (uint32_t)refLen; pf.qOff = (uint16_t)((eqo + 1) & 0xFFFF); pf.qLen = (uint16_t)(forwLen & 0xFFFF);
                pf.flags = strand | (vf ? XP_VALID : 0u);
            X.probs[2 * (size_t)r] = pb; X.probs[2 * (size_t)r + 1] = pf;
            X.extKeys[2 * (size_t)r] = vb ? 0xFFFFu - pb.qLen : 0xFFFFu; X.extKeys[2 * (size_t)r + 1] = vf ? 0xFFFFu - pf.qLen : 0xFFFFu;
            X.extVals[2 * (size_t)r] = 2u * r; X.extVals[2 * (size_t)r + 1] = 2u * r + 1u;
            X.rowsBound[2 * (size_t)r] = vb ? (unsigned long long)((pb.qLen + 19u) / 10u) : 0ull;
                X.rowsBound[2 * (size_t)r + 1] = vf ? (unsigned long long)((pf.qLen + 19u) / 10u) : 0ull;
        }
    }
    perfect = waveSumU(perfect); touched = waveSumU(touched); gapCalls = waveSumU(gapCalls); gapRows = waveSumU(gapRows); gapCells = waveSumU(gapCells);
    { unsigned long long *c = A.ctr->v; unsigned long long *const dst[5] = {&c[C_PERFECT], &c[C_TOUCHED], &c[C_GAP_CALLS], &c[C_GAP_ROWS], &c[C_GAP_CELLS]};
      const unsigned val[5] = {perfect, touched, gapCalls, gapRows, gapCells}; blockCounters<5>(dst, val); }
}

__device__ __forceinline__ int opScore(const DevParams &P, int code, int len) { return len * (code == OP_M ? P.MS : (code == OP_R ? -P.RC : -P.GE)) + (code >= OP_D ? -P.GO : 0); }
#define YD_OP_COUNT(code, len, m, r, i, d) \
    do { m += (code) == OP_M ? (len) : 0; r += (code) == OP_R ? (len) : 0; i += (code) == OP_I ? (len) : 0; d += (code) == OP_D ? (len) : 0; } while (0)
typedef uint32_t yd_u32x4u __attribute__((ext_vector_type(4), aligned(4)));
struct MergedOps {
    const uint32_t *a, *b, *c; int na, nb, nc; int jab, jbc;
    mutable const uint32_t *wp = nullptr; mutable uint32_t w0 = 0, w1 = 0, w2 = 0, w3 = 0;
    __device__ __forceinline__ uint32_t fetch(const uint32_t *seg, int idx) const
    {
        const uint32_t *base = seg + (idx & ~3);
        if (base != wp) { const yd_u32x4u v = *(YD_GLOBAL const yd_u32x4u *)toGlobal(base); w0 = v.x; w1 = v.y; w2 = v.z; w3 = v.w; wp = base; }
        const int sl = idx & 3;
        return sl == 0 ? w0 : (sl == 1 ? w1 : (sl == 2 ? w2 : w3));
    }
    __device__ int count() const { return (na - jab) + nb + (nc - jbc); }
    int lenA0 = 0, lenC0 = 0;
    __device__ __forceinline__ void setJunctions()
    {
        jab = (na > 0 && opCode(a[0]) == opCode(b[0])) ? 1 : 0; lenA0 = jab ? opLen(a[0]) : 0;
        jbc = (nc > 0 && opCode(c[0]) == opCode(b[nb - 1])) ? 1 : 0; lenC0 = jbc ? opLen(c[0]) : 0;
    }
    __device__ uint32_t at(int k) const
    {
        const int ka = na - jab;
        if (k < ka) return fetch(a, na - 1 - k);
        k -= ka;
        if (k < nb) {
            uint32_t op = fetch(b, k); int len = opLen(op);
            if (k == 0 && jab) len += lenA0;
            if (k == nb - 1 && jbc) len += lenC0;
            return opMake(opCode(op), len & 0xFFFF);
        }
        return fetch(c, k - nb + jbc);
    }
    __device__ __forceinline__ uint32_t atLean(int k) const
    {
        const int ka = na - jab, kb = ka + nb;
        const bool inA = k < ka, inB = !inA & (k < kb);
        const int idx = inA ? na - 1 - k : (inB ? k - ka : k - kb + jbc);
        const uint32_t op = fetch(inA ? a : (inB ? b : c), idx);
        const int add = ((inB & (k == ka)) ? lenA0 : 0) + ((inB & (k == kb - 1)) ? lenC0 : 0);
        return (op & 0xFFFF0000u) | ((op + (uint32_t)add) & 0xFFFFu);
    }
};
struct PredFrame { int start, len, sqo, eqo, refLen; uint32_t sro; int phase, minItem, maxItem, sQO, eQO; uint32_t sRO, eRO; };
__device__ inline int predictCarefulDPs(const DevParams &P, const MergedOps &L, int n0, int sqo0, int eqo0, uint32_t sro0, int refLen0,
                                        YD_GLOBAL const uint8_t *q, int qlen, YD_GLOBAL const uint8_t *gB, ExtProb *out, uint32_t qBase, uint32_t strand)
{
    PredFrame st[5]; int depth = 0, nOut = 0; const int wS = sqo0, wE = eqo0;
    PredFrame f; f.start = 0; f.len = n0; f.sqo = sqo0; f.eqo = eqo0; f.sro = sro0; f.refLen = refLen0; f.phase = 0;
    for (int guard = 0; guard < 64; guard++) {
        if (f.phase == 0) {
            int matches = 0, mism = 0, ins = 0, del = 0, AGS = 0, maxAGS = -10000, maxItem = -1, minItem = -1, eQO = 0, sQO = 0; uint32_t eRO = 0, sRO = 0;
            for (int k = 0; k < f.len; k++) {
                const uint32_t op = L.at(f.start + k); const int code = opCode(op), len = opLen(op);
                YD_OP_COUNT(code, len, matches, mism, ins, del);
                AGS += opScore(P, code, len); if (AGS < 0) AGS = 0;
                if (AGS > maxAGS) { maxAGS = AGS; maxItem = k; eQO = (f.sqo + matches + mism + ins - 1) & 0xFFFF; eRO = f.sro + (uint32_t)(matches + mism + del) - 1u; }
            }
            AGS = maxAGS; matches = mism = ins = del = 0; int maxMatch = 0;
            for (int k = maxItem; k >= 0; k--) {
                const uint32_t op = L.at(f.start + k); const int code = opCode(op), len = opLen(op);
                YD_OP_COUNT(code, len, matches, mism, ins, del);
                AGS -= opScore(P, code, len); maxMatch = (code == OP_M && len > maxMatch) ? len : maxMatch;
                if (AGS <= 0) { minItem = k; sQO = (eQO - (matches + mism + ins - 1)) & 0xFFFF; sRO = eRO - (uint32_t)(matches + mism + del - 1); break; }
            }
            if (maxMatch < P.wordLen || minItem < 0) f.phase = 4;
            else {
                f.minItem = minItem; f.maxItem = maxItem; f.sQO = sQO; f.eQO = eQO; f.sRO = sRO; f.eRO = eRO; f.phase = 1;
                bool has = false;
                if (minItem != 0) for (int k = 0; k < minItem && !has; k++) { const uint32_t op = L.at(f.start + k); has = opCode(op) == OP_M && opLen(op) >= P.wordLen; }
                if (has) {
                    if (depth >= 5) return nOut;
                    PredFrame c; c.start = f.start; c.len = minItem; c.sqo = f.sqo; c.eqo = (sQO - 1) & 0xFFFF; c.sro = f.sro;
                        c.refLen = (int)((1u + (sRO - 1u) - f.sro) & 0xFFFFu); c.phase = 0;
                    st[depth++] = f; f = c;
                }
            }
            continue;
        }
        if (f.phase == 1) {
            f.phase = 2;
            const int t0 = f.maxItem + 1, tl = f.len - t0; bool has = false;
            if (f.maxItem != f.len - 1) for (int k = 0; k < tl && !has; k++) { const uint32_t op = L.at(f.start + t0 + k); has = opCode(op) == OP_M && opLen(op) >= P.wordLen; }
            if (has) {
                if (depth >= 5) return nOut;
                PredFrame c; c.start = f.start + t0; c.len = tl; c.sqo = (f.eQO + 1) & 0xFFFF; c.eqo = f.eqo; c.sro = f.eRO + 1u;
// ... 221 lines not shown
```

### yaha_amd/csrc/device/stage_align.hip

```cpp
#include "ctx.h"
#include "phase_lanes.h"
#include "gap_band_lanes.h"
#include "gap_band_pk.h"
#include "ext_lanes_pk.h"
#include "split_lanes.h"
#include "dp_stage.h"
#include "align_kernels.h"
#include "layout.h"
#include "align_diag.h"

static bool laneKernels(const ygpu_ctx *ctx) { return ctx->laneExt && ctx->P.bandWidth == 5 && ctx->P.maxGap >= YD_LBAND; }

static bool extRowsPacked(const ygpu_ctx *ctx, bool caps)
{
    const bool force32 = getenv("YGPU_EXT32") != nullptr;
    const DevParams &P = ctx->P;
    return !force32 && !caps && P.MS >= 0 && (long long)P.MS * std::max(1, ctx->maxQ) <= 15000 && P.RC >= 0 && P.GO >= 0 && P.GE >= 0 && P.X >= 0
        && (long long)P.RC + P.X + P.GO + 21ll * P.GE <= 4000;
}

static bool gapBandPacked(const ygpu_ctx *ctx)
{
    const DevParams &P = ctx->P;
    return getenv("YGPU_EXT32") == nullptr && getenv("YGPU_GAP32") == nullptr && P.MS >= 0 && P.RC >= 0 && P.GO >= 0 && P.GE >= 0 && 64ll * std::max(P.MS,
// ... 24 lines not shown
    return E;
}

static int launchGapFills(ygpu_ctx *ctx, const AlignArgs &A, PhaseArgs &X, uint32_t nJoints, unsigned waves)
{
    const unsigned gBlocks16 = (unsigned)std::min<uint64_t>(gridFor(nJoints, 64), (uint64_t)ctx->nCU * 9), gBlocks32 = (unsigned)std::min<uint64_t>(gridFor(nJoints, 64),
        (uint64_t)ctx->nCU * 6);
    ENSURE(ctx->gapScratch, (size_t)YD_GAP_SCRATCH * 64 * std::max(gBlocks16, gBlocks32)); X.gapScratch = ctx->gapScratch.as<uint8_t>();
    const bool pk = gapBandPacked(ctx); X.band24 = (pk && !getenv("YGPU_GAP24_OFF")) ? 1u : 0u;
    if (pk) {
        KL(k_gap_band_pk<12>, dim3(gBlocks16), dim3(64), 0, ctx->stream, A, X); KL(k_gap_band_pk<16>, dim3(gBlocks16), dim3(64), 0, ctx->stream, A, X);
        if (X.band24) KL(k_gap_band_pk<24>, dim3(gBlocks16), dim3(64), 0, ctx->stream, A, X);
    }
    else { KL(k_gap_band<12>, dim3(gBlocks16), dim3(64), 0, ctx->stream, A, X); KL(k_gap_band<16>, dim3(gBlocks16), dim3(64), 0, ctx->stream, A, X); }
    KL(k_gap_lanes<16>, dim3(gBlocks16), dim3(64), 0, ctx->stream, A, X);
    KL(k_gap_lanes<32>, dim3(gBlocks32), dim3(64), 0, ctx->stream, A, X);
    KL(k_gap_wave, dim3(waves), dim3(64), 0, ctx->stream, A, X);
    return 0;
}

static int orderLongestFirst(ygpu_ctx *ctx, const uint32_t *keys, uint32_t n, uint32_t *out)
{
    const uint32_t sub = 0xFFFFu - (uint32_t)std::min(ctx->maxQ, 0xFFFF); int shift = 0; while (((uint32_t)ctx->maxQ >> shift) >= kBucketMax - 1u) shift++;
    return bucketOrder(ctx, keys, nullptr, 0, n, sub, shift, ((uint32_t)ctx->maxQ >> shift) + 2u, out, ctx->stream);
}

static void alignDims(ygpu_ctx *ctx, int &listCap, int &front, int &genCap, int &traceRows)
{
    front = 2 * ctx->maxQ + 8 * ctx->P.bandWidth + 64; listCap = 2 * front + 3 * ctx->maxQ + 1024;
    const long long md = std::min<long long>(ctx->P.maxDesert, 32000), g = std::min<long long>(ctx->P.maxGap, 32000), wMax = md + g + 2 * ctx->P.bandWidth + 3;
    genCap = (int)std::max<long long>(1024, wMax + 1);
    const long long wExt = 4ll * ctx->P.bandWidth + 1;
    traceRows = (int)std::max<long long>((ctx->maxQ + 2) * ((wExt + 63) / 64), ((md + 2) * wMax + 63) / 64 + 1);
}

enum class AlignOutcome { Done, GrowLaneArenas, GrowOutput, TraceGrown, Failed };
struct AlignResult {
    AlignOutcome what; int code; uint32_t ef;
    AlignResult(AlignOutcome w) : what(w), code(0), ef(0) {}
    AlignResult(int rc) : what(rc ? AlignOutcome::Failed : AlignOutcome::Done), code(rc), ef(0) {}
    static AlignResult ofFlag(uint32_t ef) { AlignResult r(ef == 0 ? AlignOutcome::Done : (ef == YERR_OUT ? AlignOutcome::GrowOutput : AlignOutcome::Failed));
        if (r.what == AlignOutcome::Failed) { r.code = YGPU_EINTERNAL; r.ef = ef; } return r; }
};

static const double kChunkBlocks = (double)YD_CHUNK_FLUSHES * 64.0;

struct TracePlan {
    unsigned maxBlocksK = 0, maxWavesK = 0;
    std::vector<uint32_t> cuts; size_t nRanges = 1;
    unsigned long long nChunksArena = 0; uint32_t maxCh = 0, extOpsCap = 0;
};
struct LanePass {
    AlignArgs A; PhaseArgs X; ExtArgs E; ExtKernels K; TracePlan T;
    unsigned waves = 0; bool rowsShare = false; uint32_t NC = 0, nProb = 0, J = 0; uint32_t *cnt = nullptr, *cc = nullptr;
    unsigned long long boundBlocks = 0, usedChunksMax = 0;
    size_t c = 0; uint32_t r0 = 0, r1 = 0, p0 = 0, np = 0;
    AlignArgs Ac; PhaseArgs Xc, Xw; uint32_t cap2 = 0, nSlow = 0, n2 = 0;
};

static int phase1(ygpu_ctx *ctx, LanePass &L, uint32_t stateOpsCap, uint32_t gapOpsPerJoint)
{
    const uint32_t NC = L.NC, nProb = L.nProb; uint32_t *cnt = L.cnt; const AlignArgs &A = L.A; PhaseArgs &X = L.X; int rc;
    ENSURE(ctx->rootState, sizeof(RootState) * (uint64_t)NC); ENSURE(ctx->stateOps, 4ull * stateOpsCap); ENSURE(ctx->extProbs, sizeof(ExtProb) * (uint64_t)nProb);
    ENSURE(ctx->rowsBound, 8ull * (nProb + 1)); ENSURE(ctx->stripOff, 8ull * (nProb + 1)); ENSURE(ctx->extRes, sizeof(ExtRes) * (uint64_t)nProb);
    ENSURE(ctx->slowList, 4ull * (NC + 1));
    HIPCHK(hipMemsetAsync(cnt + CNT_STATEOPS, 0, 16, ctx->stream));
    HIPCHK(hipMemsetAsync(cnt + CNT_QALIGN, 0, 4, ctx->stream));
    HIPCHK(hipMemsetAsync((unsigned long long *)ctx->rowsBound.p + nProb, 0, 8, ctx->stream));
    X.state = ctx->rootState.as<RootState>(); X.stateOps = ctx->stateOps.as<uint32_t>(); X.stateOpsCount = cnt + CNT_STATEOPS; X.stateOpsCap = stateOpsCap;
    X.probs = ctx->extProbs.as<ExtProb>(); X.rowsBound = ctx->rowsBound.as<unsigned long long>(); X.res = ctx->extRes.as<ExtRes>(); X.extOps = nullptr; X.rootBegin = 0;
        X.band24 = 0;
    TRACE("lanes: ensure");
    X.slowList = ctx->slowList.as<uint32_t>(); X.slowCount = cnt + CNT_SLOW; X.useList = 1;
    EV0(T_P1);
    ENSURE(ctx->jointCount, 4ull * (NC + 2)); ENSURE(ctx->jointBase, 4ull * (NC + 2));
    X.jointCount = ctx->jointCount.as<uint32_t>(); X.jointBase = ctx->jointBase.as<uint32_t>();
    KL(k_joint_counts, dim3(gridFor(NC + 1, 256)), dim3(256), 0, ctx->stream, A, X);
    rc = cubScan(ctx, ctx->jointCount.as<uint32_t>(), ctx->jointBase.as<uint32_t>(), NC + 1); if (rc) return rc;
    uint32_t J = 0; rc = fetchU32(ctx, ctx->jointBase.as<uint32_t>() + NC, &J); if (rc) return rc;
    L.J = J;
    const uint32_t gapOpsCap = (uint32_t)std::min<uint64_t>(0x7FFFFFF0ull, (uint64_t)gapOpsPerJoint * J + (1u << 20));
    ENSURE(ctx->joints, sizeof(JointRec) * (uint64_t)(J + 1)); ENSURE(ctx->sortKeys, 4ull * (J + 1)); ENSURE(ctx->sortVals, 4ull * (J + 1)); ENSURE(ctx->sortKeys2, 4ull * (J + 1));
        ENSURE(ctx->sortVals2, 4ull * (J + 1));
    ENSURE(ctx->gapOps, 4ull * gapOpsCap); ENSURE(ctx->slowList, 4ull * (std::max(NC, J) + 1));
    X.slowList = ctx->slowList.as<uint32_t>();
    X.joints = ctx->joints.as<JointRec>(); X.nJoints = J; X.sortKeys = ctx->sortKeys.as<uint32_t>(); X.sortVals = ctx->sortVals.as<uint32_t>();
        X.sortedVals = ctx->sortVals2.as<uint32_t>();
    X.nDP = cnt + CNT_NDP; X.nDPb = cnt + CNT_NB12; X.gapOps = ctx->gapOps.as<uint32_t>(); X.gapOpsCount = cnt + CNT_GAPOPS; X.gapOpsCap = gapOpsCap;
    HIPCHK(hipMemsetAsync(cnt + CNT_NDP, 0, 12, ctx->stream)); HIPCHK(hipMemsetAsync(cnt + CNT_NB12, 0, 12, ctx->stream));
    if (J) {
        KL(k_p1_joints, dim3(gridFor(NC, 256)), dim3(256), 0, ctx->stream, A, X);
        rc = bucketOrder(ctx, X.sortKeys, X.sortVals, 0, J, 0, 0, 1u << YD_JKEY_BITS, ctx->sortVals2.as<uint32_t>(), ctx->stream); if (rc) return rc;
        rc = launchGapFills(ctx, A, X, J, std::min(L.waves, 512u)); if (rc) return rc;
    }
    ENSURE(ctx->extKeys, 4ull * (nProb + 1)); ENSURE(ctx->extVals, 4ull * (nProb + 1)); ENSURE(ctx->extKeys2, 4ull * (nProb + 1)); ENSURE(ctx->extOrder, 4ull * (nProb + 1));
    X.extKeys = ctx->extKeys.as<uint32_t>(); X.extVals = ctx->extVals.as<uint32_t>();
    KL(k_p1_assemble, dim3(gridFor(NC, 256)), dim3(256), 0, ctx->stream, A, X);
    rc = cubScan64(ctx, ctx->rowsBound.as<unsigned long long>(), ctx->stripOff.as<unsigned long long>(), nProb + 1); if (rc) return rc;
    EV1(T_P1);
    TRACE("lanes: p1+scan");
    if (kTrace) { uint32_t v[3] = {0, 0, 0}; fetchU32(ctx, cnt + CNT_SLOW, &v[0]); uint32_t w[3] = {0, 0, 0}; fetchU32(ctx, cnt + CNT_NDP, w, 3); v[1] = w[0]; v[2] = w[2];
        fprintf(stderr, "[ygpu] roots %u, joints %u, DP joints %u (W<=16: %u, wave fallback %u), gap ops %u\n", NC, J, v[1], w[1], v[0], v[2]); }
    if (kTrace && getenv("YGPU_JOINT_HIST")) diagJointHist(ctx, J);
    return 0;
}

static void sizeRowsLaunch(const ygpu_ctx *ctx, const ExtKernels &K, bool rowsShare, TracePlan &T)
{
    int perCU = 2; if (hipOccupancyMaxActiveBlocksPerMultiprocessor(&perCU, K.rows, (int)K.rowsBS, 0) != hipSuccess || perCU < 1) perCU = K.rowsBS == 512u ? 1 : 2;
    if (const char *e = getenv("YGPU_ROWS_PER_CU")) { int v = atoi(e); if (v >= 1 && v < perCU) perCU = v; }
    unsigned maxBlocksK = (unsigned)((uint64_t)ctx->nCU * perCU);
    if (rowsShare && K.rowsBS == 256u) maxBlocksK = std::max(64u, maxBlocksK * 3u / 5u);
    if (const char *e = getenv("YGPU_ROWS_BLOCKS")) { const long v = atol(e); if (v >= 64 && v <= (long)ctx->nCU * perCU) maxBlocksK = (unsigned)v; }
    T.maxBlocksK = maxBlocksK; T.maxWavesK = maxBlocksK * (K.rowsBS / 64u);
}

static int cutRanges(ygpu_ctx *ctx, uint32_t NC, double perRange, bool &haveBounds, std::vector<uint32_t> &cuts)
{
    if (!haveBounds) {
        ctx->hStripOff.resize(2 * (size_t)NC + 1);
        HIPCHK(hipMemcpyAsync(ctx->hStripOff.data(), ctx->stripOff.p, 8ull * (2 * (size_t)NC + 1), hipMemcpyDeviceToHost, ctx->stream)); HIPCHK(streamSync(ctx)); haveBounds = true;
    }
    uint32_t r0 = 0;
    while (r0 < NC) {
        uint32_t lo = r0 + 1, hi = NC;
        while (lo < hi) { uint32_t mid = lo + (hi - lo + 1) / 2; if ((double)(ctx->hStripOff[2 * (size_t)mid] - ctx->hStripOff[2 * (size_t)r0]) <= perRange) lo = mid;
            else hi = mid - 1; }
        cuts.push_back(lo); r0 = lo;
    }
    return 0;
}

static int planTraceArena(ygpu_ctx *ctx, LanePass &L)
{
    TracePlan &T = L.T; const uint32_t NC = L.NC, nProb = L.nProb; const unsigned long long boundBlocks = L.boundBlocks;
    sizeRowsLaunch(ctx, L.K, L.rowsShare, T);
    const unsigned maxWavesK = T.maxWavesK;
    size_t freeB = 0, totB = 0; hipMemGetInfo(&freeB, &totB);
    const int nShare = std::max(1, gCtxPerDevice[ctx->device & 63].load());
    const size_t fairB = (size_t)((double)totB * 0.6 / nShare), availB = (size_t)((double)(freeB + ctx->extTrace.cap) * 0.8);
    unsigned long long budgetChunks = std::max<unsigned long long>(maxWavesK + 64ull, (unsigned long long)std::min(fairB, availB) / (YD_CHUNK_DWORDS * 4ull));
    budgetChunks = std::min<unsigned long long>(budgetChunks, (96ull << 30) / (YD_CHUNK_DWORDS * 4ull));
    if (ctx->traceRatio <= 0.0) {
        const double meanBoundRows = 10.0 * (double)boundBlocks / std::max(1u, nProb);
        ctx->traceRatio = std::min(0.6, std::max(0.02, (165.0 + 0.02 * meanBoundRows) / std::max(1.0, meanBoundRows)));
    }
    const double slackChunks = (double)maxWavesK + (double)ctx->nCU * 8.0 + 64.0;
    const double wantChunks = (double)boundBlocks * ctx->traceRatio / kChunkBlocks + slackChunks;
    unsigned long long nChunksArena = 0; bool haveBounds = false;
    for (;;) {
        T.cuts.assign(1, 0);
        if (wantChunks <= (double)budgetChunks && ctx->traceBudgetBlocks <= 0) { T.cuts.push_back(NC); nChunksArena = (unsigned long long)wantChunks; }
        else {
            double perRange = std::max(1.0, ((double)budgetChunks - slackChunks) * kChunkBlocks / ctx->traceRatio);
            if (ctx->traceBudgetBlocks > 0) perRange = std::min(perRange, (double)ctx->traceBudgetBlocks);
            nChunksArena = (unsigned long long)std::min((double)budgetChunks, perRange * ctx->traceRatio / kChunkBlocks + slackChunks);
            const int rc = cutRanges(ctx, NC, perRange, haveBounds, T.cuts); if (rc) return rc;
        }
        T.nRanges = T.cuts.size() - 1;
        const unsigned long long minChunks = maxWavesK + 64ull;
        nChunksArena = std::min<unsigned long long>(std::max<unsigned long long>(nChunksArena, minChunks), 0xFFFFFFF0ull);
        {
            const unsigned long long capChunks = ctx->extTrace.cap > 256 ? (unsigned long long)((ctx->extTrace.cap - 256) / (YD_CHUNK_DWORDS * 4ull)) : 0ull;
            if (T.nRanges == 1 && capChunks > minChunks && nChunksArena > capChunks && (double)nChunksArena <= 1.3 * (double)capChunks) nChunksArena = capChunks;
        }
        if (ctx->extTrace.ensureExact((size_t)nChunksArena * YD_CHUNK_DWORDS * 4ull + 256) == 0) break;
        (void)hipGetLastError();
        if (nChunksArena <= minChunks) { ctx->err = "hipMalloc failed for the extension trace arena (not even one chunk per wave fits)"; return YGPU_ENOMEM; }
        budgetChunks = std::max<unsigned long long>(minChunks, nChunksArena / 2);
        if (kTrace) fprintf(stderr, "[ygpu] trace arena of %llu chunks refused by the device: retrying with %llu and ranges\n", nChunksArena, budgetChunks);
    }
    ctx->statRanges = (int)T.nRanges;
    T.nChunksArena = std::min<unsigned long long>(0xFFFFFFF0ull, (unsigned long long)((ctx->extTrace.cap - 256) / (YD_CHUNK_DWORDS * 4ull)));
    T.maxCh = (uint32_t)std::min<unsigned long long>(T.nChunksArena, std::max<unsigned long long>(64ull, 4ull * T.nChunksArena / std::max(1u, maxWavesK) + 64ull));
    ENSURE(ctx->waveChunks, 4ull * (size_t)maxWavesK * T.maxCh + 64);
    T.extOpsCap = (uint32_t)std::min<double>(2.0e9, (double)boundBlocks * 10.0 * ctx->opsRatio + 4.0e6);
    ENSURE(ctx->extOps, 4ull * T.extOpsCap + 64);
    ENSURE(ctx->chunkCnt, 32ull * (T.nRanges + 2));
    HIPCHK(hipMemsetAsync(ctx->chunkCnt.p, 0, 32ull * (T.nRanges + 2), ctx->stream));
    ENSURE(ctx->traceCnt, 64); HIPCHK(hipMemsetAsync(ctx->traceCnt.p, 0, 64, ctx->stream));
// ... 112 lines not shown
        if (ctx->traceRatio >= 64.0) { ctx->err = "the extension trace arena overflows even at 64 times the problems' bound"; return YGPU_ENOMEM; }
        ctx->traceRatio = std::min(64.0, ctx->traceRatio * 1.5); return AlignOutcome::TraceGrown;
    }
    if (ef == YERR_OUT && usedOps > L.T.extOpsCap) {
        ctx->opsRatio = std::min(4.0, std::max(ctx->opsRatio * 2.0, 1.3 * (double)usedOps / std::max(1.0, (double)boundBlocks * 10.0))); return AlignOutcome::TraceGrown; }
    if (ef == 0 && boundBlocks) {
        const double usedRatio = ((double)L.usedChunksMax - (double)std::min<unsigned long long>(L.usedChunksMax, L.T.maxWavesK)) * kChunkBlocks * (double)L.T.nRanges
            / (double)boundBlocks;
        ctx->traceRatio = std::max(0.01, usedRatio * 1.3);
        ctx->opsRatio = std::max(0.002, std::max(1.3 * (double)usedOps / ((double)boundBlocks * 10.0), ctx->opsRatio * 0.7));
    }
    TRACE("lanes: ranges done");
    return AlignResult::ofFlag(ef);
}

static AlignResult alignWithLaneExtensions(ygpu_ctx *ctx, const AlignArgs &A, unsigned waves, uint32_t stateOpsCap, uint32_t gapOpsPerJoint)
{
    LanePass L; L.A = A; L.waves = waves; L.NC = ctx->nClumps; L.nProb = 2 * L.NC; L.cnt = ctx->counters.as<uint32_t>(); uint32_t *cnt = L.cnt; int rc;
    rc = phase1(ctx, L, stateOpsCap, gapOpsPerJoint); if (rc) return rc;
    HIPCHK(hipMemcpyAsync(&L.boundBlocks, ctx->stripOff.as<unsigned long long>() + L.nProb, 8, hipMemcpyDeviceToHost, ctx->stream));
    uint32_t ef = 0; rc = fetchU32(ctx, ctx->errFlag.p, &ef); if (rc) return rc;
    if (ef == YERR_OUT) return AlignOutcome::GrowLaneArenas;
    if (ef) return AlignResult::ofFlag(ef);
    L.rowsShare = gActiveRuns[ctx->device & 63].load() >= 2;
    L.K = extKernels(ctx, L.rowsShare); ctx->rowsPacked = L.K.packed;
    rc = planTraceArena(ctx, L); if (rc) return rc;
    const TracePlan &T = L.T; const auto traceKernel = L.K.trace;
    TRACE("lanes: trace arena");
    if (kTrace && getenv("YGPU_COUNT_DUPS")) diagCountDups(ctx, L.nProb);
    if (kTrace) fprintf(stderr, "[ygpu] trace bound %.2f GB, arena %.2f GB (%llu chunks, ratio %.3f), %zu range(s); ext ops cap %u\n", L.boundBlocks * 128.0 / 1e9,
        T.nChunksArena * (YD_CHUNK_DWORDS * 4.0) / 1e9, T.nChunksArena, ctx->traceRatio, T.nRanges, T.extOpsCap);
    ENSURE(ctx->rowsClock, 16); { const unsigned long long init[2] = {~0ull, 0ull}; HIPCHK(hipMemcpyAsync(ctx->rowsClock.p, init, 16, hipMemcpyHostToDevice, ctx->stream)); }
    L.E = extArgsBase(ctx, (uint32_t)T.nChunksArena, T.maxCh, T.extOpsCap); L.E.clock = ctx->rowsClock.as<unsigned long long>(); L.E.ctr = ctx->ctr.as<DevCounters>();
        L.E.dbgMode = getenv("YGPU_TRACE_MODE") ? atoi(getenv("YGPU_TRACE_MODE")) : 0;
    L.X.extOps = ctx->extTrace.as<uint32_t>();
    L.cc = ctx->chunkCnt.as<uint32_t>();
    EV0(T_XROWS);
    for (size_t c = 0; c < T.nRanges; c++) {
        const bool last = c + 1 == T.nRanges;
        L.c = c; L.r0 = T.cuts[c]; L.r1 = T.cuts[c + 1]; L.p0 = 2 * L.r0; L.np = 2 * (L.r1 - L.r0);
        rc = launchRows(ctx, L); if (rc) return rc;
        if (last) EV1(T_XROWS);
        TRACE("lanes: ext_rows");
        if (c == 0) { ctx->evUsed[T_XTRACE] = true; hipEventRecord(ctx->ev[T_XTRACE][0], ctx->stream); }
        if (kTrace && getenv("YGPU_TRACE_LENS")) diagTraceLens(ctx, L.E, L.np);
        rc = orderTraceback(ctx, L); if (rc) return rc;
        KL(traceKernel, dim3(gridFor(L.np, L.K.traceBS)), dim3(L.K.traceBS), 0, ctx->stream, L.E);
        if (last) hipEventRecord(ctx->ev[T_XTRACE][1], ctx->stream);
        TRACE("lanes: ext_trace");
        if (kTrace) diagTraceDbg(L.E);
        rc = scoreRoots(ctx, L); if (rc) return rc;
        if (ctx->splitLanes && L.nSlow) { rc = carefulRound(ctx, L); if (rc) return rc; }
        rc = waveFallback(ctx, L); if (rc) return rc;
        if (last) hipEventRecord(ctx->ev[T_P3][1], ctx->stream);
        TRACE("lanes: p3");
        if (kTrace && getenv("YGPU_LIST_HIST")) diagListHist(ctx, L.r0, L.r1);
    }
    HIPCHK(hipMemcpyAsync(ctx->hRowsClock, ctx->rowsClock.p, 16, hipMemcpyDeviceToHost, ctx->stream));
    unsigned int usedOps = 0; HIPCHK(hipMemcpyAsync(&usedOps, ctx->traceCnt.as<unsigned int>() + 1, 4, hipMemcpyDeviceToHost, ctx->stream));
    { const FetchPiece pc[2] = {{ctx->errFlag.p, &ef, 1}, {cnt + CNT_OUTCLUMPS, ctx->hOutCounts, 2}}; rc = fetchMany(ctx, pc, 2); if (rc) return rc; }
    if (ctx->splitLanes) ctx->lastFall = (long long)ctx->hFall;
    return learnRatios(ctx, L, ef, usedOps);
}

int stageAlign(ygpu_ctx *ctx)
{
    const uint32_t n = ctx->nReads, NC = ctx->nClumps; DevBatch B = devBatch(ctx); int rc;
    uint32_t *cnt = ctx->counters.as<uint32_t>();
    ENSURE(ctx->readCount, 4ull * (n + 1)); ENSURE(ctx->readStart, 4ull * (n + 1));
    HIPCHK(hipMemsetAsync(ctx->readCount.p, 0, 4ull * (n + 1), ctx->stream));
    ctx->nOut = ctx->nOutOps = 0;
    if (NC) {
        TRACE("before align");
        EV0(T_ALIGN);
        int listCap, front, genCap, traceRows; alignDims(ctx, listCap, front, genCap, traceRows);
        const size_t per = alignScratchBytes(ctx->maxQ, traceRows, listCap, genCap);
        size_t freeB = 0, totB = 0; hipMemGetInfo(&freeB, &totB);
        uint64_t maxWaves = std::max<uint64_t>(64, (uint64_t)((freeB / std::max(1, gCtxPerDevice[ctx->device & 63].load()) + ctx->scratchAlign.cap) * 6 / 10) / per);
        const bool useLanes = laneKernels(ctx);
        const unsigned wavesPerCU = ctx->alignWavesPerCU > 0 ? (unsigned)ctx->alignWavesPerCU : (useLanes ? 4u : 12u);
        unsigned waves = (unsigned)std::min<uint64_t>(std::min<uint64_t>(NC, (uint64_t)ctx->nCU * wavesPerCU), maxWaves);
        if (useLanes && per * waves > (3ull << 30)) waves = (unsigned)std::min<uint64_t>(waves, std::max<uint64_t>(64, (3ull << 30) / per));
        ENSURE(ctx->scratchAlign, per * waves);
        ENSURE(ctx->clumpFrags0, 16ull * (ctx->nClumpFrags + 1));
        HIPCHK(hipMemcpyAsync(ctx->clumpFrags0.p, ctx->clumpFrags.p, 16ull * ctx->nClumpFrags, hipMemcpyDeviceToDevice, ctx->stream));
        ENSURE(ctx->rootPush, 4ull * (NC + 1)); ENSURE(ctx->rootBase, 4ull * (NC + 1));
        uint32_t stateOpsCap = (uint32_t)std::min<uint64_t>(0x7FFFFFF0ull, 32ull * NC + 8ull * ctx->nClumpFrags + 65536);
        uint32_t gapOpsPerJoint = 16;
        uint32_t outClumpCap = NC + NC / 2 + 1024; uint32_t outOpsCap = (uint32_t)std::min<uint64_t>(0x7FFFFFF0ull, 32ull * NC + ctx->totalBases / 2 + 65536);
        if (const char *e = getenv("YGPU_ALIGN_CAPS")) { long long s = 0, o = 0; sscanf(e, "%lld:%lld", &s, &o);
            if (s > 0) stateOpsCap = (uint32_t)std::min<long long>(s, 0x7FFFFFF0ll);
            if (o > 0) outClumpCap = outOpsCap = (uint32_t)std::min<long long>(o, 0x7FFFFFF0ll); }
        for (int attempt = 0;; attempt++) {
            ctx->statAttempts = attempt + 1;
            ENSURE(ctx->outClumps, sizeof(ygpu_clump) * (uint64_t)outClumpCap); ENSURE(ctx->outClumps2, sizeof(ygpu_clump) * (uint64_t)outClumpCap);
            ENSURE(ctx->outOps, 4ull * outOpsCap); ENSURE(ctx->outRoot, 4ull * outClumpCap); ENSURE(ctx->outPush, 4ull * outClumpCap); ENSURE(ctx->dstIdx, 4ull * outClumpCap);
            HIPCHK(hipMemsetAsync(cnt + CNT_QALIGN, 0, 12, ctx->stream));
            HIPCHK(hipMemsetAsync(ctx->rootPush.p, 0, 4ull * (NC + 1), ctx->stream));
            HIPCHK(hipMemsetAsync(ctx->errFlag.p, 0, 4, ctx->stream));
            AlignArgs A; A.P = ctx->P; A.bases = ctx->dBases.as<uint8_t>(); A.B = B; A.order = nullptr; A.nRoots = NC;
            A.clumps = ctx->clumpsSorted.as<ChainClumpRec>(); A.clumpFrags = ctx->clumpFrags.as<DevFrag>(); A.queueHead = cnt + CNT_QALIGN;
            A.scratch = ctx->scratchAlign.as<uint8_t>(); A.scratchPerWave = per; A.maxQ = ctx->maxQ; A.listCap = listCap; A.front = front; A.genCap = genCap;
                A.traceRows = traceRows;
            A.outClumps = ctx->outClumps.as<ygpu_clump>(); A.outOps = ctx->outOps.as<uint32_t>(); A.outRoot = ctx->outRoot.as<uint32_t>(); A.outPush = ctx->outPush.as<uint32_t>();
            A.outCounts = cnt + CNT_OUTCLUMPS; A.outClumpCap = outClumpCap; A.outOpsCap = outOpsCap; A.rootPushCount = ctx->rootPush.as<unsigned int>();
            A.ctr = ctx->ctr.as<DevCounters>(); A.errFlag = ctx->errFlag.as<int>();
            profReset();
            AlignResult r = AlignOutcome::Done;
            if (useLanes) r = alignWithLaneExtensions(ctx, A, waves, stateOpsCap, gapOpsPerJoint);
            else KL(k_align, dim3(waves), dim3(64), 0, ctx->stream, A);
            profPrint(ctx, waves);
            if (!useLanes) { uint32_t ef = 0; const FetchPiece pc[2] = {{cnt + CNT_OUTCLUMPS, ctx->hOutCounts, 2}, {ctx->errFlag.p, &ef, 1}}; rc = fetchMany(ctx, pc, 2);
                if (rc) return rc; r = AlignResult::ofFlag(ef); }
            const char *redo = nullptr; bool growCaps = true;
            switch (r.what) {
            case AlignOutcome::Done: ctx->nOut = ctx->hOutCounts[0]; ctx->nOutOps = ctx->hOutCounts[1]; break;
            case AlignOutcome::GrowLaneArenas: redo = "phase-1 arenas (state ops, gap ops)"; break;
            case AlignOutcome::GrowOutput: redo = "output arenas"; break;
            case AlignOutcome::TraceGrown: redo = "trace / extension-op arena"; growCaps = false; break;
            case AlignOutcome::Failed: if (!r.ef) return r.code;
                redo = "output arenas"; break;
            }
            if (!redo) break;
            if (kStats) fprintf(stderr, "[ygpu] ctx %p: align attempt %d repeated (%s); trace ratio %.3f, ops ratio %.4f\n", (void *)ctx, attempt + 1, redo, ctx->traceRatio,
                ctx->opsRatio);
            if (r.what == AlignOutcome::Failed || attempt >= 24)       { char b[96];
                snprintf(b, sizeof b, "align stage failed with device error %u (see dp_wave.h YERR_*)", r.ef ? r.ef : (uint32_t)YERR_OUT); ctx->err = b;
                return r.ef ? r.code : YGPU_EOVERFLOW; }
            if (growCaps) {
                outClumpCap = (uint32_t)std::min<uint64_t>(0x7FFFFFF0ull, 2ull * outClumpCap); outOpsCap = (uint32_t)std::min<uint64_t>(0x7FFFFFF0ull, 2ull * outOpsCap);
                gapOpsPerJoint = std::min<uint32_t>(gapOpsPerJoint * 2u, 1u << 16); stateOpsCap = (uint32_t)std::min<uint64_t>(0x7FFFFFF0ull, 2ull * stateOpsCap);
            }
            HIPCHK(hipMemcpyAsync(ctx->clumpFrags.p, ctx->clumpFrags0.p, 16ull * ctx->nClumpFrags, hipMemcpyDeviceToDevice, ctx->stream));
            HIPCHK(hipMemsetAsync(ctx->ctr.as<DevCounters>()->v + C_SCORED, 0, 8 * (16 - C_SCORED), ctx->stream));
        }
        TRACE("align: fetch");
        EV1(T_ALIGN);
        EV0(T_LAYOUT);
        rc = cubScan(ctx, ctx->rootPush.as<uint32_t>(), ctx->rootBase.as<uint32_t>(), NC + 1); if (rc) return rc;
        if (ctx->nOut) {
            KL(k_out_layout, dim3(gridFor(ctx->nOut, 256)), dim3(256), 0, ctx->stream, ctx->outRoot.as<uint32_t>(), ctx->outPush.as<uint32_t>(), ctx->rootBase.as<uint32_t>(),
                ctx->rootPush.as<unsigned int>(), ctx->nOut, ctx->dstIdx.as<uint32_t>());
            KL(k_out_scatter, dim3(gridFor(ctx->nOut, 256)), dim3(256), 0, ctx->stream, ctx->outClumps.as<ygpu_clump>(), ctx->dstIdx.as<uint32_t>(), ctx->nOut,
                ctx->outClumps2.as<ygpu_clump>());
        }
        KL(k_read_counts, dim3(gridFor(NC, 256)), dim3(256), 0, ctx->stream, ctx->clumpsSorted.as<ChainClumpRec>(), ctx->rootPush.as<unsigned int>(), NC,
            ctx->readCount.as<unsigned int>());
    }
    rc = cubScan(ctx, ctx->readCount.as<uint32_t>(), ctx->readStart.as<uint32_t>(), n + 1); if (rc) return rc;
    if (NC) EV1(T_LAYOUT);
    return 0;
}

static int dpBatchWave(ygpu_ctx *ctx, const ygpu_dp_problem *problems, uint32_t n, const ygpu_dp_result **results, const uint32_t **ops, uint64_t *n_ops)
{
    uint32_t *cnt = ctx->counters.as<uint32_t>();
    int listCap, front, genCap, traceRows; alignDims(ctx, listCap, front, genCap, traceRows); listCap = 64;
    const size_t per = alignScratchBytes(ctx->maxQ, traceRows, listCap, genCap);
    const unsigned waves = (unsigned)std::min<uint64_t>(std::max<uint32_t>(n, 1u), (uint64_t)ctx->nCU * 4);
    uint32_t opsCap = (uint32_t)std::min<uint64_t>(0x7FFFFFF0ull, (uint64_t)n * (2ull * ctx->maxQ + 64));
    ENSURE(ctx->scratchAlign, per * waves); ENSURE(ctx->dpProbs, sizeof(ygpu_dp_problem) * (uint64_t)(n + 1)); ENSURE(ctx->dpRes, sizeof(ygpu_dp_result) * (uint64_t)(n + 1));
        ENSURE(ctx->dpOps, 4ull * opsCap + 64);
    HIPCHK(hipMemcpyAsync(ctx->dpProbs.p, problems, sizeof(ygpu_dp_problem) * (uint64_t)n, hipMemcpyHostToDevice, ctx->stream));
    HIPCHK(hipMemsetAsync(cnt + CNT_QDP, 0, 8, ctx->stream)); HIPCHK(hipMemsetAsync(ctx->errFlag.p, 0, 4, ctx->stream));
    HIPCHK(hipMemsetAsync(ctx->dpRes.p, 0, sizeof(ygpu_dp_result) * (uint64_t)(n + 1), ctx->stream));
    DPBatchArgs A; A.P = ctx->P; A.bases = ctx->dBases.as<uint8_t>(); A.B = devBatch(ctx); A.probs = ctx->dpProbs.as<ygpu_dp_problem>(); A.n = n; A.queueHead = cnt + CNT_QDP;
    A.scratch = ctx->scratchAlign.as<uint8_t>(); A.scratchPerWave = per; A.maxQ = ctx->maxQ; A.listCap = listCap; A.genCap = genCap; A.traceRows = traceRows;
    A.res = ctx->dpRes.as<ygpu_dp_result>(); A.ops = ctx->dpOps.as<uint32_t>(); A.opsCount = cnt + CNT_DPOPS; A.opsCap = opsCap; A.errFlag = ctx->errFlag.as<int>();
    if (n) KL(k_dp_batch, dim3(waves), dim3(64), 0, ctx->stream, A);
    uint32_t no = 0, ef = 0; int rc = fetchU32(ctx, cnt + CNT_DPOPS, &no); if (rc) return rc; rc = fetchU32(ctx, ctx->errFlag.p, &ef); if (rc) return rc;
    if (ef) { char b[64]; snprintf(b, sizeof b, "dp batch failed with device error %u", ef); ctx->err = b; return YGPU_EINTERNAL; }
    ctx->hDpRes.resize(n); ctx->hDpOps.resize(no);
    if (n) HIPCHK(hipMemcpy(ctx->hDpRes.data(), ctx->dpRes.p, sizeof(ygpu_dp_result) * (uint64_t)n, hipMemcpyDeviceToHost));
    if (no) HIPCHK(hipMemcpy(ctx->hDpOps.data(), ctx->dpOps.p, 4ull * no, hipMemcpyDeviceToHost));
    *results = ctx->hDpRes.data(); *ops = ctx->hDpOps.data(); *n_ops = no;
    return 0;
}

static int dpBatchLanes(ygpu_ctx *ctx, const ygpu_dp_problem *problems, uint32_t n, bool second, const ygpu_dp_result **results, const uint32_t **ops, uint64_t *n_ops)
{
    std::vector<ExtProb> xp; std::vector<uint32_t> xdst; std::vector<unsigned long long> xrows; std::vector<JointRec> jp; std::vector<uint32_t> jdst;
    uint64_t gapOpsBound = 64;
    for (uint32_t k = 0; k < n; k++) {
        const ygpu_dp_problem &p = problems[k]; const uint32_t base = ctx->hReadOff[p.read];
        if (p.mode >= YGPU_DP_EXT_FWD) {
            ExtProb e; e.qBase = base; e.rOff = p.rOff; e.qOff = p.qOff; e.qLen = p.qLen;
                e.flags = (p.strand ? XP_STRAND : 0u) | (p.mode == YGPU_DP_EXT_REV ? XP_REV : 0u) | XP_VALID;
            xp.push_back(e); xdst.push_back(k); xrows.push_back((unsigned long long)((p.qLen + 19u) / 10u));
        } else {
            JointRec j; memset(&j, 0, sizeof j); j.nsro = p.rOff; j.qBase = base; j.nsqo = p.qOff; j.qGap = p.qLen; j.rGap = p.rLen; j.kind = JK_DP;
                j.flags = (uint8_t)((p.strand ? 1u : 0u) | (p.mode == YGPU_DP_BANDED ? 2u : 0u));
            jp.push_back(j); jdst.push_back(k); gapOpsBound += (uint64_t)p.qLen + p.rLen + 2;
        }
    }
    const uint32_t nX = (uint32_t)xp.size(), nJ = (uint32_t)jp.size(); int rc;
    uint32_t *cnt = ctx->counters.as<uint32_t>(); DevBatch B = devBatch(ctx);
    HIPCHK(hipMemsetAsync(ctx->errFlag.p, 0, 4, ctx->stream));
    std::vector<ExtRes> hres(nX); std::vector<JointRec> hj(nJ); std::vector<uint32_t> xOff(nX + 1, 0), jOff(nJ + 1, 0);
    if (nX) {
        ENSURE(ctx->extProbs, sizeof(ExtProb) * (uint64_t)nX); ENSURE(ctx->extRes, sizeof(ExtRes) * (uint64_t)nX); ENSURE(ctx->chunkCnt, 64);
        HIPCHK(hipMemcpyAsync(ctx->extProbs.p, xp.data(), sizeof(ExtProb) * (uint64_t)nX, hipMemcpyHostToDevice, ctx->stream));
        HIPCHK(hipMemsetAsync(ctx->chunkCnt.p, 0, 64, ctx->stream)); HIPCHK(hipMemsetAsync(ctx->extRes.p, 0, sizeof(ExtRes) * (uint64_t)nX, ctx->stream));
        unsigned long long blocks = 0, opsBound = 64; for (uint32_t k = 0; k < nX; k++) { blocks += xrows[k]; opsBound += 2ull * xp[k].qLen + 4; }
        const ExtKernels K = extKernels(ctx, false);
        const auto rowsKernel = second ? K.rows2 : K.rows, traceKernel = K.trace; const unsigned bs = second ? K.rows2BS : K.rowsBS;
        int perCU = 2; if (hipOccupancyMaxActiveBlocksPerMultiprocessor(&perCU, K.rows, (int)K.rowsBS, 0) != hipSuccess || perCU < 1) perCU = 2;
        const unsigned blocksK = (unsigned)std::min<uint64_t>(((uint64_t)nX + bs - 1) / bs, (uint64_t)ctx->nCU * (second ? 1 : perCU)), wavesK = blocksK * (bs / 64u);
        for (unsigned long long mult = 2;; mult *= 8) {
        const unsigned long long nCh = mult * blocks / (YD_CHUNK_FLUSHES * 64ull) + 2ull * wavesK + 64ull;
        if (nCh * (YD_CHUNK_DWORDS * 4ull) > (64ull << 30) || opsBound > 0x7FFFFFF0ull) { ctx->err = "too many extension rows in one ygpu_dp_batch call"; return YGPU_EINVAL; }
        const uint32_t maxCh = (uint32_t)nCh;
        ENSURE(ctx->extTrace, nCh * (YD_CHUNK_DWORDS * 4ull) + 256); ENSURE(ctx->waveChunks, 4ull * (size_t)wavesK * maxCh + 64); ENSURE(ctx->extOps, 4ull * opsBound + 64);
            ENSURE(ctx->traceCnt, 64);
        HIPCHK(hipMemsetAsync(ctx->traceCnt.p, 0, 64, ctx->stream));
        ExtArgs E = extArgsBase(ctx, (uint32_t)nCh, maxCh, (uint32_t)opsBound); E.probs = ctx->extProbs.as<ExtProb>(); E.nProb = nX; E.res = ctx->extRes.as<ExtRes>();
            E.queue = ctx->chunkCnt.as<unsigned int>();
        KL(rowsKernel, dim3(blocksK), dim3(bs), 0, ctx->stream, E);
        KL(traceKernel, dim3(gridFor(nX, K.traceBS)), dim3(K.traceBS), 0, ctx->stream, E);
        uint32_t ef2 = 0; rc = fetchU32(ctx, ctx->errFlag.p, &ef2); if (rc) return rc;
        if (ef2 != YERR_TRACEMEM) break;
        if (mult >= 1024) { ctx->err = "extension trace arena overflows"; return YGPU_ENOMEM; }
        HIPCHK(hipMemsetAsync(ctx->errFlag.p, 0, 4, ctx->stream)); HIPCHK(hipMemsetAsync(ctx->chunkCnt.p, 0, 64, ctx->stream));
            HIPCHK(hipMemsetAsync(ctx->extRes.p, 0, sizeof(ExtRes) * (uint64_t)nX, ctx->stream));
        }
        HIPCHK(hipMemcpyAsync(hres.data(), ctx->extRes.p, sizeof(ExtRes) * (uint64_t)nX, hipMemcpyDeviceToHost, ctx->stream)); HIPCHK(streamSync(ctx));
        for (uint32_t k = 0; k < nX; k++) xOff[k + 1] = xOff[k] + (hres[k].score > 0 ? hres[k].nOps : 0u);
    }
    if (nJ) {
        const uint32_t gapOpsCap = (uint32_t)std::min<uint64_t>(0x7FFFFFF0ull, gapOpsBound);
        ENSURE(ctx->joints, sizeof(JointRec) * (uint64_t)(nJ + 1)); ENSURE(ctx->sortKeys, 4ull * (nJ + 1)); ENSURE(ctx->sortVals, 4ull * (nJ + 1));
            ENSURE(ctx->sortVals2, 4ull * (nJ + 1));
        ENSURE(ctx->gapOps, 4ull * gapOpsCap); ENSURE(ctx->slowList, 4ull * (nJ + 1));
        HIPCHK(hipMemcpyAsync(ctx->joints.p, jp.data(), sizeof(JointRec) * (uint64_t)nJ, hipMemcpyHostToDevice, ctx->stream));
        KL(k_dp_classify, dim3(gridFor(nJ, 256)), dim3(256), 0, ctx->stream, ctx->P, ctx->dBases.as<uint8_t>(), ctx->dFwd.as<uint8_t>(), ctx->dRev.as<uint8_t>(),
            ctx->joints.as<JointRec>(), nJ, ctx->sortKeys.as<uint32_t>(), ctx->sortVals.as<uint32_t>());
        std::vector<uint32_t> keys(nJ), idx(nJ);
        rc = fetchU32(ctx, ctx->sortKeys.p, keys.data(), nJ); if (rc) return rc;
        for (uint32_t k = 0; k < nJ; k++) idx[k] = k;
        std::stable_sort(idx.begin(), idx.end(), [&](uint32_t a, uint32_t b) { return keys[a] < keys[b]; });
        uint32_t nd[3] = {0, 0, 0}, nb[3] = {0, 0, 0}; for (uint32_t k = 0; k < nJ; k++) if (keys[k] != YD_JKEY_NONE) { const uint32_t cls = gapJointClass(keys[k]); nd[0]++;
            nd[1] += cls <= 2u; nb[0] += cls == 0u; nb[1] += cls <= 1u; nb[2] += gapJointBand24(keys[k]) ? 1u : 0u; }
        HIPCHK(hipMemcpyAsync(cnt + CNT_NB12, nb, 12, hipMemcpyHostToDevice, ctx->stream));
        HIPCHK(hipMemcpyAsync(ctx->sortVals2.p, idx.data(), 4ull * nJ, hipMemcpyHostToDevice, ctx->stream));
        HIPCHK(hipMemcpyAsync(cnt + CNT_NDP, nd, 12, hipMemcpyHostToDevice, ctx->stream));
        HIPCHK(hipMemsetAsync(cnt + CNT_SLOW, 0, 4, ctx->stream)); HIPCHK(hipMemsetAsync(cnt + CNT_QALIGN, 0, 4, ctx->stream));
        int listCap, front, genCap, traceRows; alignDims(ctx, listCap, front, genCap, traceRows); listCap = 64;
        const size_t per = alignScratchBytes(ctx->maxQ, traceRows, listCap, genCap); const unsigned waves = 512;
        ENSURE(ctx->scratchAlign, per * waves);
        AlignArgs A; memset(&A, 0, sizeof A); A.P = ctx->P; A.bases = ctx->dBases.as<uint8_t>(); A.B = B; A.queueHead = cnt + CNT_QALIGN;
            A.scratch = ctx->scratchAlign.as<uint8_t>(); A.scratchPerWave = per;
        A.maxQ = ctx->maxQ; A.listCap = listCap; A.front = front; A.genCap = genCap; A.traceRows = traceRows; A.ctr = ctx->ctr.as<DevCounters>();
            A.errFlag = ctx->errFlag.as<int>();
        PhaseArgs X; memset(&X, 0, sizeof X); X.joints = ctx->joints.as<JointRec>(); X.nJoints = nJ; X.sortedVals = ctx->sortVals2.as<uint32_t>(); X.nDP = cnt + CNT_NDP;
            X.nDPb = cnt + CNT_NB12;
        X.gapOps = ctx->gapOps.as<uint32_t>(); X.gapOpsCount = cnt + CNT_GAPOPS; X.gapOpsCap = gapOpsCap; X.slowList = ctx->slowList.as<uint32_t>(); X.slowCount = cnt + CNT_SLOW;
        rc = launchGapFills(ctx, A, X, nJ, waves); if (rc) return rc;
        HIPCHK(hipMemcpyAsync(hj.data(), ctx->joints.p, sizeof(JointRec) * (uint64_t)nJ, hipMemcpyDeviceToHost, ctx->stream)); HIPCHK(streamSync(ctx));
        for (uint32_t k = 0; k < nJ; k++) jOff[k + 1] = jOff[k] + hj[k].nOps;
    }
    uint32_t ef = 0; rc = fetchU32(ctx, ctx->errFlag.p, &ef); if (rc) return rc;
    if (ef) { char b[64]; snprintf(b, sizeof b, "dp batch (lane kernels) failed with device error %u", ef); ctx->err = b; return YGPU_EINTERNAL; }
    const uint32_t totX = xOff[nX], tot = totX + jOff[nJ];
    for (auto &v : jOff) v += totX;
    ENSURE(ctx->dpRes, sizeof(ygpu_dp_result) * (uint64_t)(n + 1)); ENSURE(ctx->dpOps, 4ull * tot + 64); ENSURE(ctx->dpProbs, 8ull * (n + 2));
    uint32_t *dOff = ctx->dpProbs.as<uint32_t>(), *dDst = dOff + (n + 2);
    if (nX) {
        HIPCHK(hipMemcpyAsync(dOff, xOff.data(), 4ull * nX, hipMemcpyHostToDevice, ctx->stream));
            HIPCHK(hipMemcpyAsync(dDst, xdst.data(), 4ull * nX, hipMemcpyHostToDevice, ctx->stream));
        KL(k_dp_gather_ext, dim3(gridFor(nX, 256)), dim3(256), 0, ctx->stream, ctx->extProbs.as<ExtProb>(), ctx->extRes.as<ExtRes>(), ctx->extTrace.as<uint32_t>(), dOff, dDst, nX,
           ctx->dpRes.as<ygpu_dp_result>(), ctx->dpOps.as<uint32_t>());
        HIPCHK(streamSync(ctx));
    }
    if (nJ) {
        HIPCHK(hipMemcpyAsync(dOff, jOff.data(), 4ull * nJ, hipMemcpyHostToDevice, ctx->stream));
            HIPCHK(hipMemcpyAsync(dDst, jdst.data(), 4ull * nJ, hipMemcpyHostToDevice, ctx->stream));
        KL(k_dp_gather_gap, dim3(gridFor(nJ, 256)), dim3(256), 0, ctx->stream, ctx->P, ctx->dBases.as<uint8_t>(), ctx->dFwd.as<uint8_t>(), ctx->dRev.as<uint8_t>(),
            ctx->joints.as<JointRec>(), ctx->gapOps.as<uint32_t>(), dOff, dDst, nJ,
           ctx->dpRes.as<ygpu_dp_result>(), ctx->dpOps.as<uint32_t>());
        HIPCHK(streamSync(ctx));
    }
    ctx->hDpRes.resize(n); ctx->hDpOps.resize(tot);
    if (n) HIPCHK(hipMemcpy(ctx->hDpRes.data(), ctx->dpRes.p, sizeof(ygpu_dp_result) * (uint64_t)n, hipMemcpyDeviceToHost));
    if (tot) HIPCHK(hipMemcpy(ctx->hDpOps.data(), ctx->dpOps.p, 4ull * tot, hipMemcpyDeviceToHost));
    *results = ctx->hDpRes.data(); *ops = ctx->hDpOps.data(); *n_ops = tot;
    return 0;
}

extern "C" {
int ygpu_dp_batch_ex(ygpu_ctx *ctx, const ygpu_dp_problem *problems, uint32_t n, int kernels, const ygpu_dp_result **results, const uint32_t **ops, uint64_t *n_ops)
{
    if (!ctx || !ctx->stream || !ctx->nReads || kernels < YGPU_DP_KERNELS_AUTO || kernels > YGPU_DP_KERNELS_LANES_CAREFUL) return YGPU_EINVAL;
    HIPCHK(hipSetDevice(ctx->device));
    for (uint32_t k = 0; k < n; k++) if (problems[k].read >= ctx->nReads || problems[k].mode > 3) { ctx->err = "bad DP problem"; return YGPU_EINVAL; }
    const bool useLanes = laneKernels(ctx);
    if (kernels == YGPU_DP_KERNELS_WAVE || (kernels == YGPU_DP_KERNELS_AUTO && !useLanes)) return dpBatchWave(ctx, problems, n, results, ops, n_ops);
    if (!useLanes) { ctx->err = "the lane kernels need -BW 5 and -G >= 10"; return YGPU_EINVAL; }
    return dpBatchLanes(ctx, problems, n, kernels == YGPU_DP_KERNELS_LANES_CAREFUL, results, ops, n_ops);
}
int ygpu_trace_volume(ygpu_ctx *ctx, uint64_t out[6])
{
    if (!ctx || !ctx->stream || !out || ctx->stageDone < 3) return YGPU_EINVAL;
    HIPCHK(hipSetDevice(ctx->device));
    for (int k = 0; k < 6; k++) out[k] = 0;
    const uint32_t nProb = 2u * ctx->nClumps;
    if (!laneKernels(ctx) || !nProb || ctx->extRes.cap < sizeof(ExtRes) * (uint64_t)nProb) return 0;
    ENSURE(ctx->traceCnt, 64);
    unsigned long long *d = (unsigned long long *)((char *)ctx->traceCnt.p + 32);
    HIPCHK(hipMemsetAsync(d, 0, 32, ctx->stream));
    KL(k_trace_volume, dim3(gridFor(nProb, 256)), dim3(256), 0, ctx->stream, ctx->extRes.as<ExtRes>(), nProb, d);
    unsigned long long h[4] = {0, 0, 0, 0};
    HIPCHK(hipMemcpyAsync(h, d, 32, hipMemcpyDeviceToHost, ctx->stream)); HIPCHK(streamSync(ctx));
    out[0] = h[0]; out[1] = h[1]; out[2] = h[2]; out[3] = h[3];
    out[4] = ctx->rowsPacked ? 16 : 12;
    out[5] = ctx->extTrace.cap;
    return 0;
// ... 5 lines not shown
```

Before: 427,700.

## Finish DP-free roots in one pass and inline short gap op lists

Replaces the joints kernel with a roots kernel that finishes roots needing no DP gap fill in one pass. Roots that do need it go on a pending list that the assemble kernel handles after the gap fills. Pure-diagonal joints store a mismatch bitmask, and gap-fill results with at most 14 ops are packed into the joint record instead of the global gapOps arena. The per-run clumpFrags backup copy is also skipped on the lanes path. The aim is to cut per-root launches, global atomics and memory traffic, at the cost of more complex packing logic and reuse of joint fields.

```diff
diff --git a/yaha_amd/csrc/device/abi.hip b/yaha_amd/csrc/device/abi.hip
--- a/yaha_amd/csrc/device/abi.hip
+++ b/yaha_amd/csrc/device/abi.hip
@@ -315,6 +315,7 @@
                              &ctx->rowsBound, &ctx->stripOff, &ctx->extRes, &ctx->extTrace, &ctx->chunkCnt, &ctx->memoKeys, &ctx->memoCount, &ctx->probs2, &ctx->rowsBound2,
                              &ctx->stripOff2, &ctx->extRes2, &ctx->extTrace2, &ctx->rowsClock, &ctx->splitScratch, &ctx->fallList, &ctx->keys2a, &ctx->keys2b, &ctx->vals2a,
                              &ctx->vals2b, &ctx->extKeys, &ctx->extVals, &ctx->extKeys2, &ctx->extOrder, &ctx->slowList, &ctx->gapScratch, &ctx->jointCount, &ctx->jointBase,
+                             &ctx->pendList,
                              &ctx->joints, &ctx->sortKeys, &ctx->sortVals, &ctx->sortKeys2, &ctx->sortVals2, &ctx->gapOps, &ctx->waveChunks, &ctx->extOps, &ctx->traceCnt,
                          &ctx->oqCs, &ctx->oqCl, &ctx->oqOpsIn, &ctx->oqSeeds, &ctx->oqQlen, &ctx->pf.scanState, &ctx->pf.counters, &ctx->oqProf, &ctx->oqLists, &ctx->oqClsCnt,
                              &ctx->oqThr, &ctx->oqSeqStart, &ctx->oqSeqLen, &ctx->oqNeed, &ctx->oqPoolOff, &ctx->oqKeys, &ctx->oqStack, &ctx->oqNodes, &ctx->oqPrim, &ctx->oqPA,
diff --git a/yaha_amd/csrc/device/align_diag.h b/yaha_amd/csrc/device/align_diag.h
--- a/yaha_amd/csrc/device/align_diag.h
+++ b/yaha_amd/csrc/device/align_diag.h
@@ -14,6 +14,19 @@
                     "the rest: banded %llu (W <= 32 within the band kernels' limits: %llu, %llu cells), full %llu; "
                     "W 17-24 / 25-32 / 33-40 / 41-48 / more: %llu %llu %llu %llu %llu\n",
             nj[0], nj[1], nj[2], nj[3], cj[0], cj[1], cj[2], cj[3], b3, b3lim, c3lim, f3, wh[0], wh[1], wh[2], wh[3], wh[4]);
+    const uint32_t NC = ctx->nClumps; std::vector<uint32_t> jb((size_t)NC + 1); hipMemcpy(jb.data(), ctx->jointBase.p, 4ull * (NC + 1), hipMemcpyDeviceToHost);
+    unsigned long long fr[6] = {0}, noDP = 0, noDPmulti = 0, oh[17] = {0}, dh[7] = {0}, nDiag = 0, nDPj = 0; const unsigned de[6] = {4, 8, 16, 32, 64, 128};
+    for (uint32_t r = 0; r < NC; r++) {
+        const uint32_t nj2 = jb[r + 1] - jb[r]; fr[std::min(5u, nj2)]++; bool dp = false;
+        for (uint32_t k = jb[r]; k < jb[r + 1] && k < J; k++) dp |= hj[k].kind == JK_DP;
+        noDP += !dp; noDPmulti += !dp && nj2 > 0;
+    }
+    for (auto &j : hj) { if (j.kind == JK_DP) { nDPj++; oh[j.nOps <= 15 ? j.nOps : 16]++; }
+        if (j.kind == JK_DIAG) { nDiag++; int b = 0; while (b < 6 && j.qGap > de[b]) b++; dh[b]++; } }
+    fprintf(stderr, "[ygpu] roots %u by fragments (1, 2, 3, 4, 5, more): %llu %llu %llu %llu %llu %llu; without a DP joint %llu (%.1f%%; %llu of them with joints)\n", NC,
+            fr[0], fr[1], fr[2], fr[3], fr[4], fr[5], noDP, 100.0 * noDP / std::max(1u, NC), noDPmulti);
+    fprintf(stderr, "[ygpu] DP joints %llu by ops (0 .. 15, more):", nDPj); for (int k = 0; k < 17; k++) fprintf(stderr, " %llu", oh[k]);
+    fprintf(stderr, "; pure diagonals %llu by length (<= 4, 8, 16, 32, 64, 128, more):", nDiag); for (int k = 0; k < 7; k++) fprintf(stderr, " %llu", dh[k]); fprintf(stderr, "\n");
 }
 
 static void diagCountDups(ygpu_ctx *ctx, uint32_t nProb)
diff --git a/yaha_amd/csrc/device/ctx.h b/yaha_amd/csrc/device/ctx.h
--- a/yaha_amd/csrc/device/ctx.h
+++ b/yaha_amd/csrc/device/ctx.h
@@ -50,7 +50,8 @@
 
 enum {
     CNT_NMULTI = 0, CNT_MAXN, CNT_CLUMPS, CNT_CFRAGS, CNT_QCHAIN, CNT_QALIGN, CNT_OUTCLUMPS, CNT_OUTOPS, CNT_QDP, CNT_DPOPS, CNT_NBIG, CNT_QBIG,
-    CNT_STATEOPS, CNT_EXTOPS, CNT_QEXT, CNT_SLOW, CNT_NDP, CNT_NDP16, CNT_GAPOPS, CNT_PAD_EVEN, CNT_NMULTI2 ,
+    CNT_STATEOPS, CNT_EXTOPS, CNT_QEXT, CNT_SLOW, CNT_NDP, CNT_NDP16, CNT_GAPOPS, CNT_NPEND,
+    CNT_NMULTI2 ,
         CNT_NTINY, CNT_NSMALL, CNT_NMID, CNT_NB12, CNT_NB16,
         CNT_NB24,
     CNT_SEGC,
@@ -112,7 +113,7 @@
     DevBuf rootState, stateOps, extProbs, rowsBound, stripOff, extRes, extTrace, chunkCnt;
     DevBuf memoKeys, memoCount, probs2, rowsBound2, stripOff2, extRes2, extTrace2, splitScratch, fallList;
     DevBuf keys2a, keys2b, vals2a, vals2b, extKeys, extVals, extKeys2, extOrder, slowList;
-    DevBuf gapScratch, jointCount, jointBase, joints, sortKeys, sortVals, sortKeys2, sortVals2, gapOps;
+    DevBuf gapScratch, jointCount, jointBase, joints, sortKeys, sortVals, sortKeys2, sortVals2, gapOps, pendList;
     DevBuf waveChunks, extOps, traceCnt, rowsClock;
     DevBuf counters, ctr, errFlag, scanState, bucketWork;
     bool evUsed[16] = {false};
diff --git a/yaha_amd/csrc/device/dp_stage.h b/yaha_amd/csrc/device/dp_stage.h
--- a/yaha_amd/csrc/device/dp_stage.h
+++ b/yaha_amd/csrc/device/dp_stage.h
@@ -54,7 +54,7 @@
             if (c == pc) pl++; else { if (pc >= 0) outOps[w++] = ((uint32_t)(uint8_t)codes[pc] << 16) | (uint32_t)pl; pc = c; pl = 1; }
         }
         if (pc >= 0) outOps[w++] = ((uint32_t)(uint8_t)codes[pc] << 16) | (uint32_t)pl;
-    } else for (uint32_t k = 0; k < j.nOps; k++) { const uint32_t op = gapOps[j.opsOff + k];
+    } else for (uint32_t k = 0; k < j.nOps; k++) { const uint32_t op = (j.flags & JF_INLINE) ? jointInlineOp(j, (int)k) : gapOps[j.opsOff + k];
         outOps[o.op_start + k] = ((uint32_t)(uint8_t)codes[opCode(op) & 3] << 16) | (uint32_t)opLen(op); }
     out[dst[t]] = o;
 }
diff --git a/yaha_amd/csrc/device/gap_band_lanes.h b/yaha_amd/csrc/device/gap_band_lanes.h
--- a/yaha_amd/csrc/device/gap_band_lanes.h
+++ b/yaha_amd/csrc/device/gap_band_lanes.h
@@ -100,19 +100,6 @@
             tmp[n * 64] = opMake(prev, acc2); n++;
             nT = n;
         }
-        int incl = nT;
-#pragma unroll
-        for (int d = 1; d < 64; d <<= 1) { int v = __shfl_up(incl, d, 64); if (lane >= d) incl += v; }
-        const int total = __shfl(incl, 63, 64); unsigned ob = 0;
-        if (lane == 63 && total) ob = atomicAdd(X.gapOpsCount, (unsigned)total);
-        ob = (unsigned)__shfl((int)ob, 63, 64);
-        if (live) {
-            const unsigned off = ob + (unsigned)(incl - nT);
-            if ((unsigned long long)off + (unsigned)nT > (unsigned long long)X.gapOpsCap) atomicCAS(A.errFlag, 0, (int)YERR_OUT);
-            else {
-                for (int k = 0; k < nT; k++) X.gapOps[off + k] = tmp[(nT - 1 - k) * 64];
-                JointRec *jp = X.joints + ji; jp->opsOff = off; jp->nOps = (uint16_t)nT; jp->score = score; jp->cells = cells;
-            }
-        }
+        gapListOut(A, X, lane, live, ji, tmp, nT, score, cells);
     }
 }
diff --git a/yaha_amd/csrc/device/gap_band_pk.h b/yaha_amd/csrc/device/gap_band_pk.h
--- a/yaha_amd/csrc/device/gap_band_pk.h
+++ b/yaha_amd/csrc/device/gap_band_pk.h
@@ -168,19 +168,6 @@
             tmp[n * 64] = opMake(prev, acc2); n++;
             nT = n;
         }
-        int incl = nT;
-#pragma unroll
-        for (int d = 1; d < 64; d <<= 1) { int v = __shfl_up(incl, d, 64); if (lane >= d) incl += v; }
-        const int total = __shfl(incl, 63, 64); unsigned ob = 0;
-        if (lane == 63 && total) ob = atomicAdd(X.gapOpsCount, (unsigned)total);
-        ob = (unsigned)__shfl((int)ob, 63, 64);
-        if (live) {
-            const unsigned off = ob + (unsigned)(incl - nT);
-            if ((unsigned long long)off + (unsigned)nT > (unsigned long long)X.gapOpsCap) atomicCAS(A.errFlag, 0, (int)YERR_OUT);
-            else {
-                for (int k = 0; k < nT; k++) X.gapOps[off + k] = tmp[(nT - 1 - k) * 64];
-                JointRec *jp = X.joints + ji; jp->opsOff = off; jp->nOps = (uint16_t)nT; jp->score = score; jp->cells = cells;
-            }
-        }
+        gapListOut(A, X, lane, live, ji, tmp, nT, score, cells);
     }
 }
diff --git a/yaha_amd/csrc/device/phase_lanes.h b/yaha_amd/csrc/device/phase_lanes.h
--- a/yaha_amd/csrc/device/phase_lanes.h
+++ b/yaha_amd/csrc/device/phase_lanes.h
@@ -20,6 +20,7 @@
     uint32_t *gapOps; unsigned int *gapOpsCount; uint32_t gapOpsCap;
     uint32_t *extKeys, *extVals;
     uint8_t *gapScratch;
+    uint32_t *pendList; unsigned int *pendCount;
 };
 
 __device__ __forceinline__ unsigned waveSumU(unsigned v) { return (unsigned)waveSumI((int)v); }
@@ -173,6 +174,7 @@
 }
 
 typedef unsigned long long yd_u64u __attribute__((aligned(1)));
+typedef uint32_t yd_u32x4u __attribute__((ext_vector_type(4), aligned(4)));
 template <int DIR>
 __device__ __forceinline__ int matchRun(YD_GLOBAL const uint8_t *q, int qi, YD_GLOBAL const uint8_t *gB, uint32_t ro, int maxLen)
 {
@@ -233,59 +235,225 @@
     return sOrder[threadIdx.x];
 }
 
-__global__ void __launch_bounds__(256) k_p1_joints(AlignArgs A, PhaseArgs X)
+__device__ __forceinline__ unsigned long long diagMask(YD_GLOBAL const uint8_t *q, int qi, YD_GLOBAL const uint8_t *gB, uint32_t ro, int g)
+{
+    unsigned long long mask = 0; int t = 0;
+    for (; g - t >= 8; t += 8) {
+        unsigned long long qx = *(YD_GLOBAL const yd_u64u *)(q + qi + t);
+        qx = (qx | (qx >> 4)) & 0x00FF00FF00FF00FFull; qx = (qx | (qx >> 8)) & 0x0000FFFF0000FFFFull;
+        const uint32_t qs = (uint32_t)(qx | (qx >> 16)); const uint32_t ra = ro + (uint32_t)t;
+        unsigned long long rx = *(YD_GLOBAL const yd_u64u *)(gB + (ra >> 1));
+        rx = ((rx & 0x0F0F0F0F0F0F0F0Full) << 4) | ((rx >> 4) & 0x0F0F0F0F0F0F0F0Full);
+        uint32_t d = qs ^ (uint32_t)(rx >> (4u * (ra & 1u)));
+        d |= d >> 1; d |= d >> 2; d &= 0x11111111u;
+        d = (d | (d >> 3)) & 0x03030303u; d = (d | (d >> 6)) & 0x000F000Fu; d = (d | (d >> 12)) & 0xFFu;
+        mask |= (unsigned long long)d << t;
+    }
+    for (; t < g; t++) { const uint32_t off = ro + (uint32_t)t, b = gB[off >> 1];
+        if ((uint32_t)q[qi + t] != ((off & 1u) ? (b & 15u) : (b >> 4))) mask |= 1ull << t; }
+    return mask;
+}
+
+struct RootPend { uint32_t sro, jb; uint16_t sqo, eqo, refLen, lastM, firstAdd, forwAdd; uint32_t n; uint8_t status, pad[3]; uint32_t pad2; };
+static_assert(sizeof(RootPend) == sizeof(RootState), "RootPend lives in the RootState slot");
+#define JF_DIAG_LONG 4u
+#define JF_INLINE 8u
+#define YD_JINL 14
+__host__ __device__ __forceinline__ uint32_t jointInlineOp(const JointRec &j, int k)
+{
+    const uint32_t b = k < 8 ? (uint32_t)((((unsigned long long)j.qBase << 32) | j.nsro) >> (8 * k)) : (k < 10 ? (uint32_t)j.nsqo >> (8 * (k - 8)) : j.opsOff >> (8 * (k - 10)));
+    return ((b & 3u) << 16) | (((b >> 2) & 63u) + 1u);
+}
+__device__ __forceinline__ void gapListOut(const AlignArgs &A, const PhaseArgs &X, int lane, bool have, uint32_t ji, const uint32_t *tmp, int nT, int score, unsigned cells)
+{
+    bool inl = have && nT <= YD_JINL; unsigned long long lo = 0; uint32_t mid = 0, hi = 0;
+    if (inl) for (int k = 0; k < nT; k++) {
+        const uint32_t op = tmp[(nT - 1 - k) * 64]; const uint32_t code = op >> 16; const int len = opLen(op);
+        if (code > 3u || len < 1 || len > 64) { inl = false; break; }
+        const uint32_t b = code | ((uint32_t)(len - 1) << 2);
+        if (k < 8) lo |= (unsigned long long)b << (8 * k); else if (k < 10) mid |= b << (8 * (k - 8)); else hi |= b << (8 * (k - 10));
+    }
+    const int nA = (have && !inl) ? nT : 0;
+    int incl = nA;
+#pragma unroll
+    for (int d = 1; d < 64; d <<= 1) { int v = __shfl_up(incl, d, 64); if (lane >= d) incl += v; }
+    const int total = __shfl(incl, 63, 64); unsigned ob = 0;
+    if (lane == 63 && total) ob = atomicAdd(X.gapOpsCount, (unsigned)total);
+    ob = (unsigned)__shfl((int)ob, 63, 64);
+    if (!have) return;
+    JointRec *jp = X.joints + ji;
+    if (inl) {
+        jp->nsro = (uint32_t)lo; jp->qBase = (uint32_t)(lo >> 32); jp->nsqo = (uint16_t)mid; jp->opsOff = hi; jp->flags |= (uint8_t)JF_INLINE;
+        jp->nOps = (uint16_t)nT; jp->score = score; jp->cells = cells;
+        return;
+    }
+    const unsigned off = ob + (unsigned)(incl - nA);
+    if ((unsigned long long)off + (unsigned)nT > (unsigned long long)X.gapOpsCap) { atomicCAS(A.errFlag, 0, (int)YERR_OUT); return; }
+    for (int k = 0; k < nT; k++) X.gapOps[off + k] = tmp[(nT - 1 - k) * 64];
+    jp->opsOff = off; jp->nOps = (uint16_t)nT; jp->score = score; jp->cells = cells;
+}
+
+template <bool WITH_DP>
+__device__ __forceinline__ int emitRootList(const AlignArgs &A, const PhaseArgs &X, uint32_t jb, int n, int firstAdd, int forwAdd, int lastM, uint32_t *ops, int &scoreOut,
+                                            unsigned &gapCells)
+{
+    const DevParams &P = A.P;
+    int nOut = 0, pc = OP_M, pl = firstAdd & 0xFFFF, score = (firstAdd + forwAdd) * P.MS;
+    auto put = [&](int code, int len) { if (pc == code) { pl = (pl + len) & 0xFFFF; return; } ops[nOut] = opMake(pc, pl); nOut++; pc = code; pl = len & 0xFFFF; };
+    for (int k = 0; k + 1 < n; k++) {
+        const JointRec j = X.joints[jb + (uint32_t)k]; const int qGap = j.qGap, rGap = j.rGap;
+        { const int ql = (int)j.pad; put(OP_M, ql); score += P.MS * ql; }
+        if (j.kind == JK_D) { put(OP_D, rGap); score -= P.GO + rGap * P.GE; }
+        else if (j.kind == JK_I) { put(OP_I, qGap); score -= P.GO + qGap * P.GE; }
+        else if (j.kind == JK_R) { put(OP_R, 1); score -= P.RC; }
+        else if (j.kind == JK_DIAG) {
+            const int g = qGap;
+            if (j.flags & JF_DIAG_LONG) {
+                YD_GLOBAL const uint8_t *q = toGlobal((j.flags & 1u) ? A.B.rev : A.B.fwd) + j.qBase; YD_GLOBAL const uint8_t *gB = toGlobal(A.bases);
+                for (int t = 0; t < g; t++) { const uint32_t off = j.nsro + (uint32_t)t, b = gB[off >> 1];
+                    put((uint32_t)q[(int)j.nsqo + t] == ((off & 1u) ? (b & 15u) : (b >> 4)) ? OP_M : OP_R, 1); }
+            } else {
+                const unsigned long long m = (unsigned long long)j.opsOff | ((unsigned long long)j.cells << 32);
+                for (int t = 0; t < g; ) {
+                    const bool mis = ((m >> t) & 1ull) != 0; const unsigned long long x = (mis ? ~m : m) >> t;
+                    int run = x ? __builtin_ctzll(x) : 64; if (run > g - t) run = g - t;
+                    put(mis ? OP_R : OP_M, run); t += run;
+                }
+            }
+            score += j.score;
+        } else if (WITH_DP && j.kind == JK_DP) {
+            const uint32_t *seg = X.gapOps + j.opsOff; uint32_t w0 = 0, w1 = 0, w2 = 0, w3 = 0;
+            if (j.flags & JF_INLINE) for (int t = 0; t < (int)j.nOps; t++) { const uint32_t op = jointInlineOp(j, t); put(opCode(op), opLen(op)); }
+            else for (int t = 0; t < (int)j.nOps; t++) {
+                if ((t & 3) == 0) { const yd_u32x4u v = *(YD_GLOBAL const yd_u32x4u *)toGlobal(seg + t); w0 = v.x; w1 = v.y; w2 = v.z; w3 = v.w; }
+                const int sl = t & 3; const uint32_t op = sl == 0 ? w0 : (sl == 1 ? w1 : (sl == 2 ? w2 : w3));
+                put(opCode(op), opLen(op));
+            }
+            score += j.score; gapCells += j.cells;
+        }
+    }
+    put(OP_M, lastM); score += P.MS * lastM;
+    pl = (pl + forwAdd) & 0xFFFF;
+    ops[nOut] = opMake(pc, pl); nOut++;
+    scoreOut = score;
+    return nOut;
+}
+
+__global__ void __launch_bounds__(256) k_p1_roots(AlignArgs A, PhaseArgs X)
 {
     YD_HIGH_PRIO();
-    const uint32_t r = blockIdx.x * blockDim.x + threadIdx.x;
+    const int lane = laneId(); const uint32_t r = blockIdx.x * blockDim.x + threadIdx.x;
     const bool live = r < A.nRoots; const DevParams &P = A.P;
-    unsigned perfect = 0, touched = 0, nDP = 0, nDP16 = 0, nB12 = 0, nB16 = 0, nB24 = 0;
+    unsigned perfect = 0, touched = 0, gapCalls = 0, gapRows = 0, gapCells = 0, nDP = 0, nDP16 = 0, nB12 = 0, nB16 = 0, nB24 = 0;
+    unsigned want = 0; bool pend = false; uint32_t jb = 0, sro = 0; int n = 0, firstAdd = 0, forwAdd = 0, lastM = 0, sqo = 0, eqo = 0, refLen = 0; uint8_t status = 0;
     if (live) {
-        const ChainClumpRec rec = YD_ROOT_REC(A, r); const int n = (int)rec.nFrags;
-        if (n > 1) {
-            const uint32_t read = rec.rs >> 1, r0 = A.B.readOff[read];
-            YD_GLOBAL const uint8_t *q = toGlobal((rec.rs & 1u) ? A.B.rev : A.B.fwd) + r0; YD_GLOBAL const uint8_t *gB = toGlobal(A.bases);
-            auto refAt = [&](uint32_t off) -> uint32_t { const uint32_t b = gB[off >> 1]; return (off & 1u) ? (b & 15u) : (b >> 4); };
-            DevFrag *F = A.clumpFrags + rec.fragOff; const uint32_t jb = X.jointBase[r];
-            DevFrag cur = F[0];
-            for (int k = 1; k < n; k++) {
-                DevFrag nxt = F[k];
-                int gap = (int)min(gapI(cur.eqo, nxt.sqo), gapU(cur.sro + (uint32_t)cur.refLen - 1u, nxt.sro));
-                { const int c = matchRun<-1>(q, (int)nxt.sqo - 1, gB, nxt.sro - 1u, gap);
-                  perfect += c; touched += c + (c < gap);
-                  if (c > 0) { nxt.sqo = (uint16_t)(nxt.sqo - c); nxt.sro -= (uint32_t)c; nxt.refLen = (uint16_t)(nxt.refLen + c); } gap -= c; }
-                { const uint32_t eRO = cur.sro + (uint32_t)cur.refLen - 1u; const int c = matchRun<1>(q, (int)cur.eqo + 1, gB, eRO + 1u, gap);
-                  perfect += c; touched += c + (c < gap);
-                  if (c > 0) { cur.eqo = (uint16_t)(cur.eqo + c); cur.refLen = (uint16_t)(cur.refLen + c); } }
-                F[k - 1] = cur;
-                const uint32_t eRO = cur.sro + (uint32_t)cur.refLen - 1u;
-                const int qGap = (int)(gapI(cur.eqo, nxt.sqo) & 0xFFFF), rGap = (int)(gapU(eRO, nxt.sro) & 0xFFFF);
-                JointRec j; j.nsro = eRO + 1u; j.qBase = r0; j.nsqo = (uint16_t)((cur.eqo + 1) & 0xFFFF); j.qGap = (uint16_t)qGap; j.rGap = (uint16_t)rGap;
-                j.flags = (uint8_t)(rec.rs & 1u); j.opsOff = 0; j.nOps = 0; j.pad = 0; j.score = 0; j.cells = 0; j.kind = JK_NONE;
-                uint32_t key = YD_JKEY_NONE;
-                if (qGap == 0 && rGap == 0) { }
-                else if (qGap == 0) j.kind = JK_D;
-                else if (rGap == 0) j.kind = JK_I;
-                else if (rGap == 1 && qGap == 1) j.kind = JK_R;
-                else {
-                    const int lenDiff = qGap > rGap ? qGap - rGap : rGap - qGap;
-                    const bool banded = lenDiff + P.bandWidth * 2 + 1 < rGap;
-                    j.flags |= banded ? 2u : 0u; j.kind = JK_DP;
-                    if (qGap == rGap) {
-                        int mm = 0;
-                        for (int t = 0; t < qGap; t++) mm += (uint32_t)q[(int)cur.eqo + 1 + t] != refAt(eRO + 1u + (uint32_t)t);
-                        if (mm * (P.MS + P.RC) <= P.MS + 2 * (P.GO + P.GE)) { j.kind = JK_DIAG; j.score = P.MS * (qGap - mm) - P.RC * mm; }
+        const ChainClumpRec rec = YD_ROOT_REC(A, r); n = (int)rec.nFrags;
+        const uint32_t read = rec.rs >> 1, r0 = A.B.readOff[read]; const int qlen = (int)(A.B.readOff[read + 1] - r0);
+        YD_GLOBAL const uint8_t *q = toGlobal((rec.rs & 1u) ? A.B.rev : A.B.fwd) + r0; YD_GLOBAL const uint8_t *gB = toGlobal(A.bases);
+        const DevFrag *F = A.clumpFrags + rec.fragOff; jb = X.jointBase[r];
+        const DevFrag firstF = F[0]; DevFrag cur = firstF;
+        want = (unsigned)n + 1u;
+        for (int k = 1; k < n; k++) {
+            DevFrag nxt = F[k];
+            int gap = (int)min(gapI(cur.eqo, nxt.sqo), gapU(cur.sro + (uint32_t)cur.refLen - 1u, nxt.sro));
+            { const int c = matchRun<-1>(q, (int)nxt.sqo - 1, gB, nxt.sro - 1u, gap);
+              perfect += c; touched += c + (c < gap);
+              if (c > 0) { nxt.sqo = (uint16_t)(nxt.sqo - c); nxt.sro -= (uint32_t)c; nxt.refLen = (uint16_t)(nxt.refLen + c); } gap -= c; }
+            { const uint32_t eRO = cur.sro + (uint32_t)cur.refLen - 1u; const int c = matchRun<1>(q, (int)cur.eqo + 1, gB, eRO + 1u, gap);
+              perfect += c; touched += c + (c < gap);
+              if (c > 0) { cur.eqo = (uint16_t)(cur.eqo + c); cur.refLen = (uint16_t)(cur.refLen + c); } }
+            const uint32_t eRO = cur.sro + (uint32_t)cur.refLen - 1u;
+            const int qGap = (int)(gapI(cur.eqo, nxt.sqo) & 0xFFFF), rGap = (int)(gapU(eRO, nxt.sro) & 0xFFFF);
+            JointRec j; j.nsro = eRO + 1u; j.qBase = r0; j.nsqo = (uint16_t)((cur.eqo + 1) & 0xFFFF); j.qGap = (uint16_t)qGap; j.rGap = (uint16_t)rGap;
+            j.flags = (uint8_t)(rec.rs & 1u); j.opsOff = 0; j.nOps = 0; j.pad = (uint16_t)fragQLen(cur.sqo, cur.eqo); j.score = 0; j.cells = 0; j.kind = JK_NONE;
+            uint32_t key = YD_JKEY_NONE;
+            if (qGap == 0 && rGap == 0) { }
+            else if (qGap == 0) { j.kind = JK_D; want++; }
+            else if (rGap == 0) { j.kind = JK_I; want++; }
+            else if (rGap == 1 && qGap == 1) { j.kind = JK_R; want++; }
+            else {
+                const int lenDiff = qGap > rGap ? qGap - rGap : rGap - qGap;
+                const bool banded = lenDiff + P.bandWidth * 2 + 1 < rGap;
+                j.flags |= banded ? 2u : 0u; j.kind = JK_DP;
+                if (qGap == rGap) {
+                    const int g = qGap; int mm = 0; unsigned long long mask = 0;
+                    if (g <= 64) { mask = diagMask(q, (int)cur.eqo + 1, gB, eRO + 1u, g); mm = __builtin_popcountll(mask); }
+                    else for (int t = 0; t < g; t++) { const uint32_t off = eRO + 1u + (uint32_t)t, b = gB[off >> 1];
+                        mm += (uint32_t)q[(int)cur.eqo + 1 + t] != ((off & 1u) ? (b & 15u) : (b >> 4)); }
+                    if (mm * (P.MS + P.RC) <= P.MS + 2 * (P.GO + P.GE)) {
+                        j.kind = JK_DIAG; j.score = P.MS * (g - mm) - P.RC * mm;
+                        if (g <= 64) { j.opsOff = (uint32_t)mask; j.cells = (uint32_t)(mask >> 32); } else j.flags |= JF_DIAG_LONG;
+                        want += (unsigned)g; gapCalls++; gapRows += (unsigned)g; touched += (unsigned)g;
+                        if (P.bandWidth * 2 + 1 < g) { const int bw = P.bandWidth, W = 2 * bw + 1; for (int i = 1; i <= g; i++) { int sc = bw + 1 - i; if (sc < 0) sc = 0;
+                            int ec = bw + g - i; if (ec > W - 1) ec = W - 1; if (ec >= sc) gapCells += (unsigned)(ec - sc + 1); } }
+                        else gapCells += (unsigned)(g * g);
                     }
-                    if (j.kind == JK_DP) { key = gapJointKey(P, banded, qGap, rGap); const uint32_t cls = gapJointClass(key); nDP++; nDP16 += cls <= 2u; nB12 += cls == 0u;
-                        nB16 += cls <= 1u; nB24 += gapJointBand24(key) ? 1u : 0u; }
                 }
-                X.joints[jb + (uint32_t)(k - 1)] = j; X.sortKeys[jb + (uint32_t)(k - 1)] = key; X.sortVals[jb + (uint32_t)(k - 1)] = jb + (uint32_t)(k - 1);
-                cur = nxt;
-            }
-            F[n - 1] = cur;
-        }
-    }
-    perfect = waveSumU(perfect); touched = waveSumU(touched); nDP = waveSumU(nDP); nDP16 = waveSumU(nDP16); nB12 = waveSumU(nB12); nB16 = waveSumU(nB16); nB24 = waveSumU(nB24);
-    { unsigned long long *const dst[2] = {&A.ctr->v[C_PERFECT], &A.ctr->v[C_TOUCHED]}; const unsigned val[2] = {perfect, touched}; blockCounters<2>(dst, val); }
+                if (j.kind == JK_DP) { key = gapJointKey(P, banded, qGap, rGap); const uint32_t cls = gapJointClass(key); nDP++; nDP16 += cls <= 2u; nB12 += cls == 0u;
+                    nB16 += cls <= 1u; nB24 += gapJointBand24(key) ? 1u : 0u;
+                    pend = true; gapCalls++; gapRows += (unsigned)qGap; touched += (unsigned)rGap; }
+            }
+            X.joints[jb + (uint32_t)(k - 1)] = j; X.sortKeys[jb + (uint32_t)(k - 1)] = key; X.sortVals[jb + (uint32_t)(k - 1)] = jb + (uint32_t)(k - 1);
+            cur = nxt;
+        }
+        lastM = fragQLen(cur.sqo, cur.eqo);
+        sro = firstF.sro; sqo = firstF.sqo; eqo = cur.eqo; refLen = (int)((1u + (cur.sro + (uint32_t)cur.refLen - 1u) - firstF.sro) & 0xFFFFu);
+        int backLen = (int)((uint32_t)sqo < sro ? (uint32_t)sqo : sro), forwLen;
+        if (backLen > 0) {
+            const int m = matchRun<-1>(q, sqo - 1, gB, sro - 1u, backLen);
+            perfect += m; touched += m + (m < backLen);
+            if (m > 0) { firstAdd = m; backLen -= m; sqo -= m; sro -= (uint32_t)m; refLen = (refLen + m) & 0xFFFF; }
+        }
+        {
+            const uint32_t eRO = sro + (uint32_t)refLen - 1u;
+            const uint32_t qrem = (uint32_t)(((qlen - 1) - eqo) & 0xFFFF), rrem = P.maxROff - eRO;
+            forwLen = (int)(qrem < rrem ? qrem : rrem);
+            if (forwLen > 0) {
+                const int m = matchRun<1>(q, eqo + 1, gB, eRO + 1u, forwLen);
+                perfect += m; touched += m + (m < forwLen);
+                if (m > 0) { forwAdd = m; forwLen -= m; eqo += m; refLen = (refLen + m) & 0xFFFF; }
+            }
+        }
+        status = (rec.rs & 1u) ? stReversed : 0;
+        const uint32_t strand = (rec.rs & 1u) ? XP_STRAND : 0u; const bool vb = backLen >= P.minExtLength, vf = forwLen >= P.minExtLength;
+        ExtProb pb; pb.qBase = r0; pb.rOff = sro - 1u; pb.qOff = (uint16_t)((sqo - 1) & 0xFFFF); pb.qLen = (uint16_t)(backLen & 0xFFFF);
+            pb.flags = strand | XP_REV | (vb ? XP_VALID : 0u);
+        ExtProb pf; pf.qBase = r0; pf.rOff = sro + (uint32_t)refLen; pf.qOff = (uint16_t)((eqo + 1) & 0xFFFF); pf.qLen = (uint16_t)(forwLen & 0xFFFF);
+            pf.flags = strand | (vf ? XP_VALID : 0u);
+        X.probs[2 * (size_t)r] = pb; X.probs[2 * (size_t)r + 1] = pf;
+        X.extKeys[2 * (size_t)r] = vb ? 0xFFFFu - pb.qLen : 0xFFFFu; X.extKeys[2 * (size_t)r + 1] = vf ? 0xFFFFu - pf.qLen : 0xFFFFu;
+        X.extVals[2 * (size_t)r] = 2u * r; X.extVals[2 * (size_t)r + 1] = 2u * r + 1u;
+        X.rowsBound[2 * (size_t)r] = vb ? (unsigned long long)((pb.qLen + 19u) / 10u) : 0ull;
+            X.rowsBound[2 * (size_t)r + 1] = vf ? (unsigned long long)((pf.qLen + 19u) / 10u) : 0ull;
+        if (pend) {
+            RootPend s; memset(&s, 0, sizeof s);
+            s.sro = sro; s.jb = jb; s.sqo = (uint16_t)sqo; s.eqo = (uint16_t)eqo; s.refLen = (uint16_t)refLen; s.lastM = (uint16_t)lastM; s.firstAdd = (uint16_t)firstAdd;
+                s.forwAdd = (uint16_t)forwAdd; s.n = (uint32_t)n; s.status = status;
+            *(RootPend *)(X.state + r) = s;
+        }
+    }
+    { const unsigned long long pm = __ballot(pend); const unsigned pi = waveReserve(pm, X.pendCount, lane); if (pend) X.pendList[pi] = r; }
+    const bool fin = live && !pend; if (!fin) want = 0;
+    unsigned incl = want;
+#pragma unroll
+    for (int d = 1; d < 64; d <<= 1) { unsigned t = (unsigned)__shfl_up((int)incl, d, 64); if (lane >= d) incl += t; }
+    const unsigned total = (unsigned)__shfl((int)incl, 63, 64);
+    const unsigned base = blockReserve(X.stateOpsCount, total);
+    const unsigned slot = base + incl - want;
+    if (fin) {
+        if ((unsigned long long)slot + want > (unsigned long long)X.stateOpsCap) atomicCAS(A.errFlag, 0, (int)YERR_OUT);
+        else {
+            int score = 0; unsigned dpCells = 0;
+            const int nOut = emitRootList<false>(A, X, jb, n, firstAdd, forwAdd, lastM, X.stateOps + slot, score, dpCells);
+            RootState s; memset(&s, 0, sizeof s);
+            s.sro = sro; s.sqo = (uint16_t)sqo; s.eqo = (uint16_t)eqo; s.refLen = (uint16_t)refLen; s.score = score; s.status = status; s.len = (uint16_t)nOut; s.listOff = slot;
+            X.state[r] = s;
+        }
+    }
+    perfect = waveSumU(perfect); touched = waveSumU(touched); gapCalls = waveSumU(gapCalls); gapRows = waveSumU(gapRows); gapCells = waveSumU(gapCells);
+    nDP = waveSumU(nDP); nDP16 = waveSumU(nDP16); nB12 = waveSumU(nB12); nB16 = waveSumU(nB16); nB24 = waveSumU(nB24);
+    { unsigned long long *c = A.ctr->v; unsigned long long *const dst[5] = {&c[C_PERFECT], &c[C_TOUCHED], &c[C_GAP_CALLS], &c[C_GAP_ROWS], &c[C_GAP_CELLS]};
+      const unsigned val[5] = {perfect, touched, gapCalls, gapRows, gapCells}; blockCounters<5>(dst, val); }
     { unsigned int *const dst[5] = {X.nDP, X.nDP + 1, X.nDPb, X.nDPb + 1, X.nDPb + 2}; const unsigned val[5] = {nDP, nDP16, nB12, nB16, nB24}; blockCountersU32<5>(dst, val); }
 }
 
@@ -316,20 +484,7 @@
             }
         }
         { const unsigned long long mm = __ballot(tooBig); const unsigned sl = waveReserve(mm, X.slowCount, lane); if (tooBig) X.slowList[sl] = ji; }
-        int incl = nT;
-#pragma unroll
-        for (int d = 1; d < 64; d <<= 1) { int v = __shfl_up(incl, d, 64); if (lane >= d) incl += v; }
-        const int total = __shfl(incl, 63, 64); unsigned ob = 0;
-        if (lane == 63 && total) ob = atomicAdd(X.gapOpsCount, (unsigned)total);
-        ob = (unsigned)__shfl((int)ob, 63, 64);
-        if (live && !tooBig) {
-            const unsigned off = ob + (unsigned)(incl - nT);
-            if ((unsigned long long)off + (unsigned)nT > (unsigned long long)X.gapOpsCap) atomicCAS(A.errFlag, 0, (int)YERR_OUT);
-            else {
-                for (int k = 0; k < nT; k++) X.gapOps[off + k] = GM.tmp[(nT - 1 - k) * 64];
-                JointRec *jp = X.joints + ji; jp->opsOff = off; jp->nOps = (uint16_t)nT; jp->score = score; jp->cells = cells;
-            }
-        }
+        gapListOut(A, X, lane, live && !tooBig, ji, GM.tmp, nT, score, cells);
     }
 }
 
@@ -362,99 +517,40 @@
 __global__ void __launch_bounds__(256) k_p1_assemble(AlignArgs A, PhaseArgs X)
 {
     YD_HIGH_PRIO();
-    const int lane = laneId(); const uint32_t r = blockIdx.x * blockDim.x + threadIdx.x;
-    const bool live = r < A.nRoots; const DevParams &P = A.P;
-    ChainClumpRec rec; rec.nFrags = 0; rec.rs = 0; rec.fragOff = 0;
-    if (live) rec = YD_ROOT_REC(A, r);
-    const int n = (int)rec.nFrags; const uint32_t jb = live ? X.jointBase[r] : 0u;
+    const int lane = laneId(); const uint32_t t = blockIdx.x * blockDim.x + threadIdx.x;
+    const uint32_t nPend = *X.pendCount;
+    if (blockIdx.x * blockDim.x >= nPend) return;
+    const bool live = t < nPend;
+    uint32_t r = 0; RootPend S; memset(&S, 0, sizeof S);
+    if (live) { r = X.pendList[t]; S = *(const RootPend *)(X.state + r); }
+    const int n = (int)S.n; const uint32_t jb = S.jb;
     unsigned want = 0;
     if (live) { want = (unsigned)n + 1u; for (int k = 0; k + 1 < n; k++) { const JointRec &j = X.joints[jb + (uint32_t)k];
         want += j.kind == JK_DP ? (unsigned)j.nOps : (j.kind == JK_DIAG ? (unsigned)j.qGap : (j.kind != JK_NONE ? 1u : 0u)); } }
     unsigned incl = want;
 #pragma unroll
-    for (int d = 1; d < 64; d <<= 1) { unsigned t = (unsigned)__shfl_up((int)incl, d, 64); if (lane >= d) incl += t; }
+    for (int d = 1; d < 64; d <<= 1) { unsigned v = (unsigned)__shfl_up((int)incl, d, 64); if (lane >= d) incl += v; }
     const unsigned total = (unsigned)__shfl((int)incl, 63, 64);
     const unsigned base = blockReserve(X.stateOpsCount, total);
     const unsigned slot = base + incl - want;
-    unsigned perfect = 0, touched = 0, gapCalls = 0, gapRows = 0, gapCells = 0;
+    unsigned gapCells = 0;
     if (live) {
         if ((unsigned long long)slot + want > (unsigned long long)X.stateOpsCap) atomicCAS(A.errFlag, 0, (int)YERR_OUT);
         else {
-            const uint32_t read = rec.rs >> 1, r0 = A.B.readOff[read]; const int qlen = (int)(A.B.readOff[read + 1] - r0);
-            YD_GLOBAL const uint8_t *q = toGlobal((rec.rs & 1u) ? A.B.rev : A.B.fwd) + r0; YD_GLOBAL const uint8_t *gB = toGlobal(A.bases);
-            auto refAt = [&](uint32_t off) -> uint32_t { const uint32_t b = gB[off >> 1]; return (off & 1u) ? (b & 15u) : (b >> 4); };
-            const DevFrag *F = A.clumpFrags + rec.fragOff;
-            uint32_t *ops = X.stateOps + slot; int nOut = 0, pc = -1, pl = 0, score = 0;
-            auto put = [&](int code, int len) { if (pc == code) { pl = (pl + len) & 0xFFFF; return; } if (pc >= 0) { ops[nOut] = opMake(pc, pl); nOut++; } pc = code;
-                pl = len & 0xFFFF; };
-            const DevFrag firstF = F[0]; DevFrag cur = firstF;
-            for (int k = 1; k <= n; k++) {
-                { const int ql = fragQLen(cur.sqo, cur.eqo); put(OP_M, ql); score += P.MS * ql; }
-                if (k == n) break;
-                const JointRec j = X.joints[jb + (uint32_t)(k - 1)]; const int qGap = j.qGap, rGap = j.rGap;
-                if (j.kind == JK_D) { put(OP_D, rGap); score -= P.GO + rGap * P.GE; }
-                else if (j.kind == JK_I) { put(OP_I, qGap); score -= P.GO + qGap * P.GE; }
-                else if (j.kind == JK_R) { put(OP_R, 1); score -= P.RC; }
-                else if (j.kind == JK_DIAG) {
-                    const int g = qGap;
-                    for (int t = 0; t < g; t++) put((uint32_t)q[(int)j.nsqo + t] == refAt(j.nsro + (uint32_t)t) ? OP_M : OP_R, 1);
-                    score += j.score; gapCalls++; gapRows += (unsigned)g; touched += (unsigned)g;
-                    if (P.bandWidth * 2 + 1 < g) { const int bw = P.bandWidth, W = 2 * bw + 1; for (int i = 1; i <= g; i++) { int sc = bw + 1 - i; if (sc < 0) sc = 0;
-                        int ec = bw + g - i; if (ec > W - 1) ec = W - 1; if (ec >= sc) gapCells += (unsigned)(ec - sc + 1); } }
-                    else gapCells += (unsigned)(g * g);
-                } else if (j.kind == JK_DP) {
-                    for (int t = 0; t < (int)j.nOps; t++) { const uint32_t op = X.gapOps[j.opsOff + (uint32_t)t]; put(opCode(op), opLen(op)); }
-                    score += j.score; gapCalls++; gapRows += (unsigned)qGap; gapCells += j.cells; touched += (unsigned)rGap;
-                }
-                cur = F[k];
-            }
-            uint32_t sro = firstF.sro; int sqo = firstF.sqo, eqo = cur.eqo; int refLen = (int)((1u + (cur.sro + (uint32_t)cur.refLen - 1u) - firstF.sro) & 0xFFFFu);
-            int firstAdd = 0;
-            int backLen = (int)((uint32_t)sqo < sro ? (uint32_t)sqo : sro), forwLen;
-            if (backLen > 0) {
-                const int m = matchRun<-1>(q, sqo - 1, gB, sro - 1u, backLen);
-                perfect += m; touched += m + (m < backLen);
-                if (m > 0) { firstAdd = m; score += m * P.MS; backLen -= m; sqo -= m; sro -= (uint32_t)m; refLen = (refLen + m) & 0xFFFF; }
-            }
-            {
-                const uint32_t eRO = sro + (uint32_t)refLen - 1u;
-                const uint32_t qrem = (uint32_t)(((qlen - 1) - eqo) & 0xFFFF), rrem = P.maxROff - eRO;
-                forwLen = (int)(qrem < rrem ? qrem : rrem);
-                if (forwLen > 0) {
-                    const int m = matchRun<1>(q, eqo + 1, gB, eRO + 1u, forwLen);
-                    perfect += m; touched += m + (m < forwLen);
-                    if (m > 0) { pl = (pl + m) & 0xFFFF; score += m * P.MS; forwLen -= m; eqo += m; refLen = (refLen + m) & 0xFFFF; }
-                }
-            }
-            if (nOut == 0) pl = (pl + firstAdd) & 0xFFFF;
-            ops[nOut] = opMake(pc, pl); nOut++;
-            if (nOut > 1 && firstAdd) ops[0] = opMake(opCode(ops[0]), (opLen(ops[0]) + firstAdd) & 0xFFFF);
+            int score = 0;
+            const int nOut = emitRootList<true>(A, X, jb, n, (int)S.firstAdd, (int)S.forwAdd, (int)S.lastM, X.stateOps + slot, score, gapCells);
             RootState s; memset(&s, 0, sizeof s);
-            s.sro = sro; s.sqo = (uint16_t)sqo; s.eqo = (uint16_t)eqo; s.refLen = (uint16_t)refLen; s.score = score; s.status = (rec.rs & 1u) ? stReversed : 0;
-                s.len = (uint16_t)nOut;
-            s.listOff = slot;
+            s.sro = S.sro; s.sqo = S.sqo; s.eqo = S.eqo; s.refLen = S.refLen; s.score = score; s.status = S.status; s.len = (uint16_t)nOut; s.listOff = slot;
             X.state[r] = s;
-            const uint32_t strand = (rec.rs & 1u) ? XP_STRAND : 0u; const bool vb = backLen >= P.minExtLength, vf = forwLen >= P.minExtLength;
-            ExtProb pb; pb.qBase = r0; pb.rOff = sro - 1u; pb.qOff = (uint16_t)((sqo - 1) & 0xFFFF); pb.qLen = (uint16_t)(backLen & 0xFFFF);
-                pb.flags = strand | XP_REV | (vb ? XP_VALID : 0u);
-            ExtProb pf; pf.qBase = r0; pf.rOff = sro + (uint32_t)refLen; pf.qOff = (uint16_t)((eqo + 1) & 0xFFFF); pf.qLen = (uint16_t)(forwLen & 0xFFFF);
-                pf.flags = strand | (vf ? XP_VALID : 0u);
-            X.probs[2 * (size_t)r] = pb; X.probs[2 * (size_t)r + 1] = pf;
-            X.extKeys[2 * (size_t)r] = vb ? 0xFFFFu - pb.qLen : 0xFFFFu; X.extKeys[2 * (size_t)r + 1] = vf ? 0xFFFFu - pf.qLen : 0xFFFFu;
-            X.extVals[2 * (size_t)r] = 2u * r; X.extVals[2 * (size_t)r + 1] = 2u * r + 1u;
-            X.rowsBound[2 * (size_t)r] = vb ? (unsigned long long)((pb.qLen + 19u) / 10u) : 0ull;
-                X.rowsBound[2 * (size_t)r + 1] = vf ? (unsigned long long)((pf.qLen + 19u) / 10u) : 0ull;
-        }
-    }
-    perfect = waveSumU(perfect); touched = waveSumU(touched); gapCalls = waveSumU(gapCalls); gapRows = waveSumU(gapRows); gapCells = waveSumU(gapCells);
-    { unsigned long long *c = A.ctr->v; unsigned long long *const dst[5] = {&c[C_PERFECT], &c[C_TOUCHED], &c[C_GAP_CALLS], &c[C_GAP_ROWS], &c[C_GAP_CELLS]};
-      const unsigned val[5] = {perfect, touched, gapCalls, gapRows, gapCells}; blockCounters<5>(dst, val); }
+        }
+    }
+    gapCells = waveSumU(gapCells);
+    { unsigned long long *const dst[1] = {&A.ctr->v[C_GAP_CELLS]}; const unsigned val[1] = {gapCells}; blockCounters<1>(dst, val); }
 }
 
 __device__ __forceinline__ int opScore(const DevParams &P, int code, int len) { return len * (code == OP_M ? P.MS : (code == OP_R ? -P.RC : -P.GE)) + (code >= OP_D ? -P.GO : 0); }
 #define YD_OP_COUNT(code, len, m, r, i, d) \
     do { m += (code) == OP_M ? (len) : 0; r += (code) == OP_R ? (len) : 0; i += (code) == OP_I ? (len) : 0; d += (code) == OP_D ? (len) : 0; } while (0)
-typedef uint32_t yd_u32x4u __attribute__((ext_vector_type(4), aligned(4)));
 struct MergedOps {
     const uint32_t *a, *b, *c; int na, nb, nc; int jab, jbc;
     mutable const uint32_t *wp = nullptr; mutable uint32_t w0 = 0, w1 = 0, w2 = 0, w3 = 0;
diff --git a/yaha_amd/csrc/device/stage_align.hip b/yaha_amd/csrc/device/stage_align.hip
--- a/yaha_amd/csrc/device/stage_align.hip
+++ b/yaha_amd/csrc/device/stage_align.hip
@@ -130,20 +130,21 @@
     const uint32_t gapOpsCap = (uint32_t)std::min<uint64_t>(0x7FFFFFF0ull, (uint64_t)gapOpsPerJoint * J + (1u << 20));
     ENSURE(ctx->joints, sizeof(JointRec) * (uint64_t)(J + 1)); ENSURE(ctx->sortKeys, 4ull * (J + 1)); ENSURE(ctx->sortVals, 4ull * (J + 1)); ENSURE(ctx->sortKeys2, 4ull * (J + 1));
         ENSURE(ctx->sortVals2, 4ull * (J + 1));
-    ENSURE(ctx->gapOps, 4ull * gapOpsCap); ENSURE(ctx->slowList, 4ull * (std::max(NC, J) + 1));
+    ENSURE(ctx->gapOps, 4ull * gapOpsCap + 16); ENSURE(ctx->slowList, 4ull * (std::max(NC, J) + 1));
     X.slowList = ctx->slowList.as<uint32_t>();
     X.joints = ctx->joints.as<JointRec>(); X.nJoints = J; X.sortKeys = ctx->sortKeys.as<uint32_t>(); X.sortVals = ctx->sortVals.as<uint32_t>();
         X.sortedVals = ctx->sortVals2.as<uint32_t>();
     X.nDP = cnt + CNT_NDP; X.nDPb = cnt + CNT_NB12; X.gapOps = ctx->gapOps.as<uint32_t>(); X.gapOpsCount = cnt + CNT_GAPOPS; X.gapOpsCap = gapOpsCap;
-    HIPCHK(hipMemsetAsync(cnt + CNT_NDP, 0, 12, ctx->stream)); HIPCHK(hipMemsetAsync(cnt + CNT_NB12, 0, 12, ctx->stream));
+    HIPCHK(hipMemsetAsync(cnt + CNT_NDP, 0, 16, ctx->stream)); HIPCHK(hipMemsetAsync(cnt + CNT_NB12, 0, 12, ctx->stream));
+    ENSURE(ctx->extKeys, 4ull * (nProb + 1)); ENSURE(ctx->extVals, 4ull * (nProb + 1)); ENSURE(ctx->extKeys2, 4ull * (nProb + 1)); ENSURE(ctx->extOrder, 4ull * (nProb + 1));
+    X.extKeys = ctx->extKeys.as<uint32_t>(); X.extVals = ctx->extVals.as<uint32_t>();
+    ENSURE(ctx->pendList, 4ull * (NC + 1)); X.pendList = ctx->pendList.as<uint32_t>(); X.pendCount = cnt + CNT_NPEND;
+    KL(k_p1_roots, dim3(gridFor(NC, 256)), dim3(256), 0, ctx->stream, A, X);
     if (J) {
-        KL(k_p1_joints, dim3(gridFor(NC, 256)), dim3(256), 0, ctx->stream, A, X);
         rc = bucketOrder(ctx, X.sortKeys, X.sortVals, 0, J, 0, 0, 1u << YD_JKEY_BITS, ctx->sortVals2.as<uint32_t>(), ctx->stream); if (rc) return rc;
         rc = launchGapFills(ctx, A, X, J, std::min(L.waves, 512u)); if (rc) return rc;
-    }
-    ENSURE(ctx->extKeys, 4ull * (nProb + 1)); ENSURE(ctx->extVals, 4ull * (nProb + 1)); ENSURE(ctx->extKeys2, 4ull * (nProb + 1)); ENSURE(ctx->extOrder, 4ull * (nProb + 1));
-    X.extKeys = ctx->extKeys.as<uint32_t>(); X.extVals = ctx->extVals.as<uint32_t>();
-    KL(k_p1_assemble, dim3(gridFor(NC, 256)), dim3(256), 0, ctx->stream, A, X);
+        KL(k_p1_assemble, dim3(gridFor(std::min(NC, J), 256)), dim3(256), 0, ctx->stream, A, X);
+    }
     rc = cubScan64(ctx, ctx->rowsBound.as<unsigned long long>(), ctx->stripOff.as<unsigned long long>(), nProb + 1); if (rc) return rc;
     EV1(T_P1);
     TRACE("lanes: p1+scan");
@@ -422,8 +423,8 @@
         unsigned waves = (unsigned)std::min<uint64_t>(std::min<uint64_t>(NC, (uint64_t)ctx->nCU * wavesPerCU), maxWaves);
         if (useLanes && per * waves > (3ull << 30)) waves = (unsigned)std::min<uint64_t>(waves, std::max<uint64_t>(64, (3ull << 30) / per));
         ENSURE(ctx->scratchAlign, per * waves);
-        ENSURE(ctx->clumpFrags0, 16ull * (ctx->nClumpFrags + 1));
-        HIPCHK(hipMemcpyAsync(ctx->clumpFrags0.p, ctx->clumpFrags.p, 16ull * ctx->nClumpFrags, hipMemcpyDeviceToDevice, ctx->stream));
+        if (!useLanes) { ENSURE(ctx->clumpFrags0, 16ull * (ctx->nClumpFrags + 1));
+            HIPCHK(hipMemcpyAsync(ctx->clumpFrags0.p, ctx->clumpFrags.p, 16ull * ctx->nClumpFrags, hipMemcpyDeviceToDevice, ctx->stream)); }
         ENSURE(ctx->rootPush, 4ull * (NC + 1)); ENSURE(ctx->rootBase, 4ull * (NC + 1));
         uint32_t stateOpsCap = (uint32_t)std::min<uint64_t>(0x7FFFFFF0ull, 32ull * NC + 8ull * ctx->nClumpFrags + 65536);
         uint32_t gapOpsPerJoint = 16;
@@ -471,7 +472,7 @@
                 outClumpCap = (uint32_t)std::min<uint64_t>(0x7FFFFFF0ull, 2ull * outClumpCap); outOpsCap = (uint32_t)std::min<uint64_t>(0x7FFFFFF0ull, 2ull * outOpsCap);
                 gapOpsPerJoint = std::min<uint32_t>(gapOpsPerJoint * 2u, 1u << 16); stateOpsCap = (uint32_t)std::min<uint64_t>(0x7FFFFFF0ull, 2ull * stateOpsCap);
             }
-            HIPCHK(hipMemcpyAsync(ctx->clumpFrags.p, ctx->clumpFrags0.p, 16ull * ctx->nClumpFrags, hipMemcpyDeviceToDevice, ctx->stream));
+            if (!useLanes) HIPCHK(hipMemcpyAsync(ctx->clumpFrags.p, ctx->clumpFrags0.p, 16ull * ctx->nClumpFrags, hipMemcpyDeviceToDevice, ctx->stream));
             HIPCHK(hipMemsetAsync(ctx->ctr.as<DevCounters>()->v + C_SCORED, 0, 8 * (16 - C_SCORED), ctx->stream));
         }
         TRACE("align: fetch");
@@ -570,7 +571,7 @@
         const uint32_t gapOpsCap = (uint32_t)std::min<uint64_t>(0x7FFFFFF0ull, gapOpsBound);
         ENSURE(ctx->joints, sizeof(JointRec) * (uint64_t)(nJ + 1)); ENSURE(ctx->sortKeys, 4ull * (nJ + 1)); ENSURE(ctx->sortVals, 4ull * (nJ + 1));
             ENSURE(ctx->sortVals2, 4ull * (nJ + 1));
-        ENSURE(ctx->gapOps, 4ull * gapOpsCap); ENSURE(ctx->slowList, 4ull * (nJ + 1));
+        ENSURE(ctx->gapOps, 4ull * gapOpsCap + 16); ENSURE(ctx->slowList, 4ull * (nJ + 1));
         HIPCHK(hipMemcpyAsync(ctx->joints.p, jp.data(), sizeof(JointRec) * (uint64_t)nJ, hipMemcpyHostToDevice, ctx->stream));
         KL(k_dp_classify, dim3(gridFor(nJ, 256)), dim3(256), 0, ctx->stream, ctx->P, ctx->dBases.as<uint8_t>(), ctx->dFwd.as<uint8_t>(), ctx->dRev.as<uint8_t>(),
             ctx->joints.as<JointRec>(), nJ, ctx->sortKeys.as<uint32_t>(), ctx->sortVals.as<uint32_t>());
```

New measurement: 442,600 (median of 6 runs). 3.5% higher.
